# manasakani/DeviceKMC

Hardware: AMD Instinct MI355X
Metric: KMC steps/sec (higher is better)
Workload: dtype f64

## Files before the change

### devicekmc_amd/csrc/common.h

```cpp
#pragma once
#include <hip/hip_runtime.h>
#include <stdint.h>
#include <stdio.h>
#include <string.h>
#include <math.h>
#include "../../include/devicekmc_hip.h"
#include "../../include/devicekmc_hip_debug.h"

enum { DEFECT = 0, OXYGEN_DEFECT = 1, VACANCY = 2, O_EL = 3, Hf_EL = 4, Ni_EL = 5, Ti_EL = 6, Pt_EL = 7, N_EL = 8, NULL_ELEMENT = 9 };
enum { EV_GEN = 0, EV_REC = 1, EV_VDIFF = 2, EV_IDIFF = 3, EV_NULL = 4 };

#define DKMC_KB 8.617333262e-5
#define DKMC_Q 1.60217663e-19
#define DKMC_HBAR 1.054571817e-34
#define DKMC_MAX_LAYERS 5
#define WAVE 64

struct MetalSet { int n; const int *e; };

__device__ __forceinline__ bool is_metal(int el, const MetalSet &ms)
{
    bool r = false;
    for (int t = 0; t < ms.n; ++t) r |= (ms.e[t] == el);
    return r;
// ... 87 lines not shown
template <int NT>
__device__ __forceinline__ double block_sum_all(double v, double *red)
{
    const int lane = threadIdx.x & 63, w = threadIdx.x >> 6;
    v = wave_sum(v);
    __syncthreads();
    if (lane == 0) red[w] = v;
    __syncthreads();
    double s = 0.0;
#pragma unroll
    for (int i = 0; i < NT / 64; ++i) s += red[i];
    return s;
}

__host__ __device__ __forceinline__ unsigned long long dbl_key(double v)
{
    const unsigned long long b = __builtin_bit_cast(unsigned long long, v);
    return (b >> 63) ? ~b : (b | 0x8000000000000000ull);
}
__host__ __device__ __forceinline__ double key_dbl(unsigned long long k)
{
    return __builtin_bit_cast(double, (k >> 63) ? (k & 0x7fffffffffffffffull) : ~k);
}
__device__ __forceinline__ int ld_agent(const int *p) { return __hip_atomic_load(p, __ATOMIC_RELAXED, __HIP_MEMORY_SCOPE_AGENT); }
__device__ __forceinline__ void st_agent(int *p, int v) { __hip_atomic_store(p, v, __ATOMIC_RELAXED, __HIP_MEMORY_SCOPE_AGENT); }
__device__ __forceinline__ int seed_bits(int i, int N, int n_left, int n_right) { return (i < n_left ? 1 : 0) | (i >= N - n_right ? 2 : 0); }
inline void clamp_seeds(int N, int &n_left, int &n_right)
{
    n_left = n_left < 0 ? 0 : (n_left > N ? N : n_left);
    n_right = n_right < 0 ? 0 : (n_right > N ? N : n_right);
}

struct KBlocked {
    int m, R, nb, total, maxwin, maxints;
    long long winsum;
    int *perm;
    int *pcol;
    int4 *blk;
    int form = 1;
    int maxseg = 0;
    long long segsum = 0;
    int4 *seg = nullptr;
    int word_bytes = 4;
};
constexpr int X_POLY_DEFAULT = 8;
struct Engine {
    hipStream_t stream = nullptr;
    int device = 0;
    double cg_tol = 1e-6;
    int current_warm_start = 1;
    int profiling = 0;
    int cb_edge_domain = 0;
    long long tcache_budget = -1;
    double pair_cut = 6.5;
    int pair_form = 0;
    int k_blocked = 1;
    int k_blocked_large = 0;
    int k_window_word_bytes = 4;
    int x_aux = 2;
    int x_slab = 1;
    int k_slab = 1;
    int x_poly = X_POLY_DEFAULT;
    int x_poly_auto = 1;
    int x_poly_rows[2] = {0, 0};
    int x_poly_form = 2;
    int x_poly1_degree = 0;
    int x_poly_form_used = 0, x_poly_products = 0;
    int x_slab_poly = 0;
    int x_aux_warm = 0;
    int x_items_kc = 0;
    int x_apply_form = 0;
    int x_tile_f32 = 1;
    double x_tile_drop = 0.0;
    int x_tile_drop_unit = 0;
    int x_tile_drop_auto = 1;
    long long x_tile_drop_gate = 0;
    double x_tile_drop_used = 0.0;
    int xtl_census_form = 1;
    int x_static_tiles = 2;
    int x_static_gate = 0;
    int x_static_nM = -1;
    int x_static_verify = 0;
    int x_tile_f32_fail_once = 0;
    int x_nmul_form = 1;
    int x_nmul_lane_bytes = 16;
    int x_nmul_window = 2;
    int x_nmul_window_cap = 76 * 1024;
    int x_nmul_window_block = 320;
    int x_block = 16;
    int x_format = 1;
    int current_map = 0;
    int x_iter_hint = 0;
    int event_temperature = 0;
    int event_census = 0;
    int event_census_valid = 0;
    double event_census_info[16] = {0};
    dkmc_stats stats{};
    char err[512] = {0};
    int err_code = 0;
    double E_gen[DKMC_MAX_LAYERS] = {0}, E_rec[DKMC_MAX_LAYERS] = {0}, E_Vdiff[DKMC_MAX_LAYERS] = {0}, E_Odiff[DKMC_MAX_LAYERS] = {0};
    int num_layers = 0;
    static const int NBUF = 184;
    void *buf[NBUF] = {nullptr};
    size_t bufsz[NBUF] = {0};
};

constexpr int X_STATIC_GATE = 32768;
static inline int x_static_rule(int ns, int gate_override) { return ns >= (gate_override > 0 ? gate_override : X_STATIC_GATE) ? 1 : 0; }
Engine &eng();
int dkmc_fail(int code, const char *what, const char *file, int line);
void *scratch(int slot, size_t bytes);
void *scratch_try(int slot, size_t bytes);
static inline int grid_blocks(long long work, int per_block, int cap)
{
    long long b = (work + per_block - 1) / per_block;
    if (b < 1) b = 1;
    if (b > cap) b = cap;
    return (int)b;
}
inline MetalSet load_metals(const int *d_metals, int num_metals) { MetalSet ms; ms.n = num_metals; ms.e = d_metals; return ms; }

#define HIPCHK(x) do { hipError_t e__ = (x); if (e__ != hipSuccess) return dkmc_fail((int)e__, hipGetErrorString(e__), __FILE__, __LINE__); } while (0)
#define KCHK() do { hipError_t e__ = hipGetLastError(); if (e__ != hipSuccess) return dkmc_fail((int)e__, hipGetErrorString(e__), __FILE__, __LINE__); } while (0)

enum {
    S_CG_S = 0, S_CG_R, S_CG_P, S_CG_T, S_CG_PART, S_CG_CTRL, S_CG_RUNS, S_CG_REM, S_CG_NRUNS, S_CG_PS, S_CG_SEGOFF, S_CG_SEGS, S_CG_SEGPART, S_CG_XCHG, S_CG_PARTS,
    S_K_DATA, S_K_RHS,
    S_PW_LIST, S_PW_CNT, S_PW_CELLS, S_PW_PERM, S_PW_LIST2,
    S_EV_PROB, S_EV_ROWSUM, S_EV_G2, S_EV_G3, S_EV_CTRL, S_EV_UNI, S_EV_LOG,
    S_SCAN_TMP, S_SCAN_TMP2, S_SCAN_OFF64, S_SCAN_INTILE,
    S_AT_FLAG, S_AT_SITE, S_AT_OFSITE, S_AT_NEIGH,
    S_X_ROWPTR, S_X_COL, S_X_DATA, S_X_DATA2, S_X_CNT, S_X_SLIST, S_X_SCB, S_X_SFLAG, S_X_RHS, S_X_SRANK,
    S_P_IMACRO, S_HEAT, S_HEAT_A, S_HEAT_B, S_HEAT_Y,
    S_MISC0, S_MISC1, S_MISC2, S_MISC3,
    S_XT_DPOS, S_XT_SNODE_D, S_XT_SNODE_I, S_XT_CMASK, S_XT_ISTILE, S_XT_NSUBC, S_XT_TOFF, S_XT_SOFF, S_XT_TILES, S_XT_NITEMW, S_XT_WRANGE,
    S_XT_ITEMS, S_XT_SPLIT, S_XT_TVAL, S_XT_TVAL32, S_XT_ROWPART, S_XT_COLPART, S_XT_CNT, S_XT_Q,
    S_XT_T_NITEMW, S_XT_T_ITEMS, S_XT_T_SPLIT, S_XT_T_COLPART, S_XT_T_MISC,
    S_XTB_PANELS, S_XTB_QS, S_XTB_ROWPART, S_XTB_COLPART, S_XTB_GRAM, S_XTB_SMALL, S_XTB_XI,
    S_XTB_SLAB_BOX, S_XTB_SLAB_TAB, S_XTB_SLAB_OWNER, S_XTB_SLAB_LISTS, S_XTB_SLAB_SDST, S_XTB_SLAB_FLAG, S_XTB_SLAB_RLISTS, S_XTB_SLAB_GX, S_XTB_SLAB_S1, S_XTB_SLAB_S3, S_XTB_SLAB_R3,
    S_XTB_EMU_Y, S_XTB_EMU_CTRL, S_XTB_YPANEL, S_XTB_PRE_V, S_XTB_PRE_W1, S_XTB_PRE_W2, S_XTB_PRE_Z, S_XTB_PRE_U,
    S_XTB_NPACK_CNT, S_XTB_NPACK_OFF, S_XTB_NPACK_COL, S_XTB_NPACK_W,
    S_XTL_CELLS, S_XTL_TFLAG, S_XTL_TVAL32, S_XTL_TILES, S_XTL_WRANGE, S_XTL_NITEMW, S_XTL_ITEMS, S_XTL_SPLIT,
    S_KS_TAB, S_KS_OWNER, S_KS_LISTS, S_KS_FLAG, S_KS_BOX, S_KS_RLISTS, S_KS_XA, S_KS_XB, S_KS_SEND, S_KS_RECV, S_KS_YBUF, S_KS_EMU,
    S_XTB_TEST_RP, S_XTB_TEST_CI, S_XTB_TEST_VAL, S_XTB_TEST_SC, S_XTB_TEST_NSR, S_XTB_TEST_LIST, S_XTB_TEST_IN, S_XTB_TEST_ADD, S_XTB_TEST_OUT,
    S_XTB_TEST_W1, S_XTB_TEST_W2, S_XTB_TEST_QS, S_XTB_TEST_CTRL, S_XTB_TEST_NPCNT, S_XTB_TEST_NPOFF, S_XTB_TEST_NPCOL, S_XTB_TEST_NPW,
    S_P_CMAP,
    S_XTB_ALG_PANELS, S_XTB_ALG_INTS, S_XTB_ALG_GRAM, S_XTB_ALG_QS, S_XTB_ALG_CTRL,
    S_CL_PARENT, S_CL_SUMS, S_CL_POS, S_CL_TABLE, S_CL_CTRL,
    S_EV_NBAD, S_EV_CENSUS_PART, S_EV_CENSUS_INFO,
    S_GAP_SITE, S_GAP_CTRL, S_GAP_CELLS, S_GAP_SORTED, S_GAP_NODES, S_GAP_EDGES,
    S_PT_HOP, S_PT_PRED, S_PT_ROWS, S_PT_CTRL,
    S_TR_HASH, S_TR_COMP, S_TR_SITE, S_TR_ROWS, S_TR_CTRL,
    S_CUT_SITE, S_CUT_TABLE, S_CUT_ROWS, S_CUT_CTRL,
    S_FL_SITE, S_FL_ROWS, S_FL_CTRL,
    S_NSLOTS
};
static_assert(S_NSLOTS <= Engine::NBUF, "scratch slots");

int comm_attached();
int comm_nranks();
int comm_rank();
int comm_allgather_f64(double *buf, size_t count);
int comm_alltoallv_f64(const double *sendbuf, double *recvbuf, const long long *cnt);
int comm_allreduce_sum_f64(double *buf, size_t count);
int comm_agree(int local_rc, const char *what);
int comm_agree_count();
int comm_peer_ready(size_t count);
double *comm_peer_slots(int parity);
void comm_peer_drop();
int comm_peer_exchange(int parity, size_t count, int *ctrl_done, int *ctrl_aborted, int *ctrl_timeout, int stamp);
int comm_bcast0_f64(double *buf, size_t count);

int ev_census_enqueue(int N, int nn, const int *neigh, const int *element, const double *temperature, const double *ev_prob, double **d_info16);

int dkmc_exclusive_scan_i32(const int *d_in, int *d_out, int n, int *d_total);
int dkmc_exclusive_scan_i32_i64(const int *d_in, long long *d_out, int n, long long *d_total);
```

### devicekmc_amd/csrc/engine.hip

```cpp
#include "common.h"
#include <stdlib.h>

int events_upload_layers();
void xstate_reset(const void *key);

static Engine g_engine;
Engine &eng() { return g_engine; }

int dkmc_fail(int code, const char *what, const char *file, int line)
{
    Engine &e = eng();
    snprintf(e.err, sizeof(e.err), "%s (%s:%d)", what, file, line);
    e.err_code = code ? code : -1;
    fprintf(stderr, "devicekmc_hip: %s\n", e.err);
    return e.err_code;
}

void *scratch(int slot, size_t bytes)
{
    Engine &e = eng();
    if (bytes == 0) bytes = 16;
    if (e.bufsz[slot] < bytes) {
        if (e.buf[slot]) { (void)hipStreamSynchronize(e.stream); (void)hipFree(e.buf[slot]); }
        size_t want = bytes + bytes / 8 + 256;
        hipError_t rc = hipMalloc(&e.buf[slot], want);
        if (rc != hipSuccess) {
            char msg[160]; snprintf(msg, sizeof(msg), "hipMalloc(%zu bytes) failed in scratch(slot %d): %s", want, slot, hipGetErrorString(rc));
            dkmc_fail(2, msg, __FILE__, __LINE__); e.buf[slot] = nullptr; e.bufsz[slot] = 0; return nullptr;
        }
        e.bufsz[slot] = want;
    }
    return e.buf[slot];
}

void *scratch_try(int slot, size_t bytes)
{
    Engine &e = eng();
    if (bytes == 0) bytes = 16;
    if (e.bufsz[slot] < bytes) {
        if (e.buf[slot]) { (void)hipStreamSynchronize(e.stream); (void)hipFree(e.buf[slot]); }
        e.buf[slot] = nullptr; e.bufsz[slot] = 0;
        const size_t want = bytes + bytes / 8 + 256;
        if (hipMalloc(&e.buf[slot], want) != hipSuccess) { (void)hipGetLastError(); e.buf[slot] = nullptr; return nullptr; }
        e.bufsz[slot] = want;
    }
    return e.buf[slot];
}

extern "C" {

const char *dkmc_last_error(void) { return eng().err; }
void dkmc_clear_error(void) { eng().err[0] = 0; eng().err_code = 0; }
const dkmc_stats *dkmc_get_stats(void) { return &eng().stats; }
void dkmc_set_cg_tolerance(double tol) { eng().cg_tol = tol; }
void dkmc_set_current_warm_start(int mode) { eng().current_warm_start = mode; }
int dkmc_get_current_warm_start(void) { return eng().current_warm_start; }
void dkmc_set_profiling(int on) { eng().profiling = on; }
void dkmc_set_x_format(int tiled) { eng().x_format = tiled ? 1 : 0; }
int dkmc_get_x_format(void) { return eng().x_format; }
void dkmc_set_current_map(int on) { eng().current_map = on ? 1 : 0; }
int dkmc_get_current_map(void) { return eng().current_map; }
void dkmc_set_tcache_budget(long long bytes) { eng().tcache_budget = bytes; }
void dkmc_set_pair_cutoff(double x_cut) { eng().pair_cut = x_cut > 0.0 ? x_cut : 0.0; }
void dkmc_set_pair_form(int form) { eng().pair_form = form == 1 ? 1 : 0; }
int dkmc_get_pair_form(void) { return eng().pair_form; }
void dkmc_set_k_slab(int on) { eng().k_slab = on ? 1 : 0; }
int dkmc_get_k_slab(void) { return eng().k_slab; }
void dkmc_set_x_aux_warm(int on) { eng().x_aux_warm = on ? 1 : 0; }
int dkmc_get_x_aux_warm(void) { return eng().x_aux_warm; }
void dkmc_set_x_items(int kc) { eng().x_items_kc = kc > 0 ? (kc < 256 ? kc : 256) : 0; }
void dkmc_set_x_poly(int degree) { eng().x_poly = degree < 0 ? 0 : (degree > 16 ? 16 : degree); eng().x_poly_auto = 0; }
int dkmc_get_x_poly(void) { return eng().x_poly; }
void dkmc_set_x_poly_auto(int on) { Engine &e = eng(); e.x_poly_auto = on ? 1 : 0; if (on && e.x_poly <= 0) e.x_poly = X_POLY_DEFAULT; }
int dkmc_get_x_poly_auto(void) { return eng().x_poly_auto; }
void dkmc_set_x_poly_form(int form) { eng().x_poly_form = form == 1 ? 1 : (form == 2 ? 2 : 0); }
int dkmc_get_x_poly_form(void) { return eng().x_poly_form; }
int dkmc_get_x_poly_form_used(void) { return eng().x_poly_form_used; }
int dkmc_get_x_poly_products(void) { return eng().x_poly_products; }
void dkmc_debug_set_x_poly1_degree(int n) { eng().x_poly1_degree = n < 0 ? 0 : (n > 20 ? 20 : n); }
void dkmc_set_x_poly_auto_rows(int n0, int n1) { Engine &e = eng(); e.x_poly_rows[0] = n0 > 0 ? n0 : 0; e.x_poly_rows[1] = n1 > e.x_poly_rows[0] ? n1 : e.x_poly_rows[0]; }
void dkmc_set_x_apply_form(int form) { eng().x_apply_form = form == 1 ? 1 : 0; }
int dkmc_get_x_apply_form(void) { return eng().x_apply_form; }
void dkmc_set_x_tile_f32(int mode) { eng().x_tile_f32 = mode == 0 ? 0 : 1; }
int dkmc_get_x_tile_f32(void) { return eng().x_tile_f32; }
void dkmc_set_x_tile_drop(double theta) { eng().x_tile_drop = theta > 0.0 ? (theta > 1e-4 ? 1e-4 : theta) : 0.0; }
double dkmc_get_x_tile_drop(void) { return eng().x_tile_drop; }
void dkmc_set_x_tile_drop_unit(int unit) { eng().x_tile_drop_unit = unit == 1 ? 1 : 0; }
int dkmc_get_x_tile_drop_unit(void) { return eng().x_tile_drop_unit; }
void dkmc_set_x_tile_drop_auto(int on) { eng().x_tile_drop_auto = on ? 1 : 0; }
int dkmc_get_x_tile_drop_auto(void) { return eng().x_tile_drop_auto; }
void dkmc_set_x_tile_drop_auto_subblocks(long long gate) { eng().x_tile_drop_gate = gate > 0 ? gate : 0; }
double dkmc_get_x_tile_drop_used(void) { return eng().x_tile_drop_used; }
void dkmc_debug_fail_true_residual_once(void) { eng().x_tile_f32_fail_once = 1; }
void dkmc_set_x_static_tiles(int mode) { eng().x_static_tiles = (mode == 0 || mode == 1) ? mode : 2; }
int dkmc_get_x_static_tiles(void) { return eng().x_static_tiles; }
int dkmc_debug_x_static_verify(int on) { const int was = eng().x_static_verify; eng().x_static_verify = on ? 1 : 0; return was; }
void dkmc_debug_set_x_static_gate(int members) { eng().x_static_gate = members > 0 ? members : 0; }
int dkmc_x_static_rule(int members) { return x_static_rule(members, eng().x_static_gate); }
int dkmc_x_static_strips(int n_metals) { return n_metals > 0 ? n_metals / 256 : 0; }
void dkmc_set_x_nmul_form(int form) { eng().x_nmul_form = form == 0 ? 0 : 1; }
int dkmc_get_x_nmul_form(void) { return eng().x_nmul_form; }
void dkmc_set_x_nmul_lane_bytes(int bytes) { eng().x_nmul_lane_bytes = bytes == 8 ? 8 : 16; }
int dkmc_get_x_nmul_lane_bytes(void) { return eng().x_nmul_lane_bytes; }
void dkmc_set_x_nmul_window(int mode) { eng().x_nmul_window = (mode == 0 || mode == 1) ? mode : 2; }
int dkmc_get_x_nmul_window(void) { return eng().x_nmul_window; }
void dkmc_debug_set_x_nmul_window(int cap_bytes, int block_rows)
{
    Engine &e = eng();
    e.x_nmul_window_cap = cap_bytes < 0 ? 76 * 1024 : (cap_bytes > 76 * 1024 ? 76 * 1024 : cap_bytes);
    e.x_nmul_window_block = (block_rows >= 16 && block_rows <= 1024 && block_rows % 16 == 0) ? block_rows : 320;
}
void dkmc_set_x_slab(int on) { eng().x_slab = on ? 1 : 0; }
int dkmc_get_x_slab(void) { return eng().x_slab; }
void dkmc_set_x_slab_poly(int on) { eng().x_slab_poly = on ? 1 : 0; }
int dkmc_get_x_slab_poly(void) { return eng().x_slab_poly; }
void dkmc_set_x_block(int s) { eng().x_block = s < 1 ? 1 : (s > 16 ? 16 : s); }
int dkmc_get_x_block(void) { return eng().x_block; }
void dkmc_set_x_aux(int mode) { eng().x_aux = mode < 0 ? 0 : (mode > 3 ? 2 : mode); }
int dkmc_get_x_aux(void) { return eng().x_aux; }
void dkmc_set_k_blocked(int on) { eng().k_blocked = on ? 1 : 0; }
int dkmc_get_k_blocked(void) { return eng().k_blocked; }
void dkmc_set_k_blocked_large(int on) { eng().k_blocked_large = on ? 1 : 0; }
int dkmc_get_k_blocked_large(void) { return eng().k_blocked_large; }
void dkmc_set_k_window_word_bytes(int bytes) { eng().k_window_word_bytes = bytes == 2 ? 2 : 4; }
int dkmc_get_k_window_word_bytes(void) { return eng().k_window_word_bytes; }
void dkmc_set_cb_edge_domain(int atoms_only) { eng().cb_edge_domain = atoms_only ? 1 : 0; }

int dkmc_get_gpu_info(char *gpu_string, int capacity, int dev)
{
    hipDeviceProp_t prop;
    HIPCHK(hipSetDevice(dev));
    HIPCHK(hipGetDeviceProperties(&prop, dev));
    snprintf(gpu_string, capacity, "%s", prop.name);
    return 0;
}

int dkmc_set_gpu(int dev) { HIPCHK(hipSetDevice(dev)); eng().device = dev; return 0; }
int dkmc_set_stream(void *s) { eng().stream = (hipStream_t)s; return 0; }
int dkmc_synchronize(void) { HIPCHK(hipStreamSynchronize(eng().stream)); return 0; }

int dkmc_copy_to_const_memory(const double *E_gen, const double *E_rec, const double *E_Vdiff, const double *E_Odiff, int nl)
{
    Engine &e = eng();
    if (nl > DKMC_MAX_LAYERS) return dkmc_fail(3, "more than 5 layers (MAX_NUM_LAYERS, kmc_events.cu:7)", __FILE__, __LINE__);
    e.num_layers = nl;
    for (int i = 0; i < nl; ++i) { e.E_gen[i] = E_gen[i]; e.E_rec[i] = E_rec[i]; e.E_Vdiff[i] = E_Vdiff[i]; e.E_Odiff[i] = E_Odiff[i]; }
    return events_upload_layers();
}

#define ALLOC(field, n, T) HIPCHK(hipMalloc((void **)&buf->field, (size_t)(n) * sizeof(T)))
int dkmc_gpubuf_create(dkmc_gpubuf *buf, int N, int N_atom, int nn, int nmt,
                       const int *h_layer, const double *hx, const double *hy, const double *hz,
                       const int *h_neigh, const int *h_metals, double freq, double sigma, double k, const double *h_lattice)
{
    memset(buf, 0, sizeof(*buf));
    buf->N_ = N; buf->N_atom_ = N_atom; buf->nn_ = nn; buf->num_metal_types_ = nmt;
    ALLOC(site_layer, N, int); ALLOC(site_element, N, int); ALLOC(metal_types, nmt > 0 ? nmt : 1, int);
    ALLOC(site_x, N, double); ALLOC(site_y, N, double); ALLOC(site_z, N, double);
    ALLOC(site_power, N, double); ALLOC(site_CB_edge, N, double);
    ALLOC(site_potential_boundary, N, double); ALLOC(site_potential_charge, N, double);
    ALLOC(site_temperature, N, double); ALLOC(site_charge, N, int);
    ALLOC(neigh_idx, (size_t)N * nn, int);
    ALLOC(T_bg, 1, double); ALLOC(sigma, 1, double); ALLOC(k, 1, double); ALLOC(lattice, 3, double); ALLOC(freq, 1, double);
    ALLOC(atom_element, N, int); ALLOC(atom_x, N, double); ALLOC(atom_y, N, double); ALLOC(atom_z, N, double);
    ALLOC(atom_power, N, double); ALLOC(atom_CB_edge, N, double); ALLOC(atom_charge, N, int);
    ALLOC(atom_virtual_potentials, N_atom + 2, double);
    HIPCHK(hipMemset(buf->atom_virtual_potentials, 0, (size_t)(N_atom + 2) * sizeof(double)));
    HIPCHK(hipMemset(buf->site_power, 0, (size_t)N * sizeof(double)));
    HIPCHK(hipMemcpy(buf->site_layer, h_layer, (size_t)N * sizeof(int), hipMemcpyHostToDevice));
    HIPCHK(hipMemcpy(buf->site_x, hx, (size_t)N * sizeof(double), hipMemcpyHostToDevice));
    HIPCHK(hipMemcpy(buf->site_y, hy, (size_t)N * sizeof(double), hipMemcpyHostToDevice));
    HIPCHK(hipMemcpy(buf->site_z, hz, (size_t)N * sizeof(double), hipMemcpyHostToDevice));
    if (nmt > 0) HIPCHK(hipMemcpy(buf->metal_types, h_metals, (size_t)nmt * sizeof(int), hipMemcpyHostToDevice));
    HIPCHK(hipMemcpy(buf->sigma, &sigma, sizeof(double), hipMemcpyHostToDevice));
    HIPCHK(hipMemcpy(buf->k, &k, sizeof(double), hipMemcpyHostToDevice));
    HIPCHK(hipMemcpy(buf->freq, &freq, sizeof(double), hipMemcpyHostToDevice));
// ... 75 lines not shown
```

### devicekmc_amd/csrc/xt.hip

```cpp
#include "xtiles.h"
#include <hip/hip_ext.h>
int tc_prepare_tiled(const XParams &P, dkmc_gpubuf *buf, int ns, const SEntry *S, const int *aflag, const int *srank, const int *atom_site,
                     int c_lo, int c_hi, int sharded, TCacheView *out);
#include <vector>
#include <algorithm>
#include <stdlib.h>
#include <string.h>

__device__ __forceinline__ double xt_tvalue(const XParams &P, double prefac, const TCacheView &TC,
                                            double x1, double y1, double z1, double cb1, int f1, int slot1, int slotA1, int mr1,
                                            double x2, double y2, double z2, double cb2, int f2, int slot2, int slotA2, int mr2,
                                            bool have_pre = false, double pre = 0.0)
{
    const double d = site_dist(x1, y1, z1, x2, y2, z2, P.laty, P.latz, P.pbc);
    if (d < P.nn_dist) return 0.0;
    const int kind = tunnel_kind<AF_MP_VAL>(f1, f2, cb1, cb2, P.tol);
    if (!kind) return 0.0;
    if (kind == 1 && TC.enabled) {
        const bool v1 = f1 & AF_V;
        double cv;
        if (have_pre && !v1) { if (pre == pre) return -pre; }
        else if (tc_lookup(TC, v1 ? slot1 : slot2, v1 ? slotA1 : slotA2, v1 ? mr2 : mr1, cv)) return -cv;
    }
    return -wkb_T(kind, 1e-10 * d, fabs(cb1 - cb2), prefac, P.V0);
}

__global__ void k_xt_snodes(int ns, int ns_pad, const SEntry *__restrict__ S, const double *__restrict__ ax, const double *__restrict__ ay,
                            const double *__restrict__ az, double *sx, double *sy, double *sz, double *scb, int *sflag, int *srow)
{
    const int s = blockIdx.x * blockDim.x + threadIdx.x;
    if (s >= ns_pad) return;
    if (s < ns) {
        const SEntry e = S[s];
        sx[s] = ax[e.idx]; sy[s] = ay[e.idx]; sz[s] = az[e.idx]; scb[s] = e.cb; sflag[s] = e.flag; srow[s] = e.idx + 2;
    } else { sx[s] = 0; sy[s] = 0; sz[s] = 0; scb[s] = 0; sflag[s] = 0; srow[s] = -1; }
}
__global__ void k_xt_snode_slots(int ns, int ns_pad, const SEntry *__restrict__ S, const int *__restrict__ atom_site, TCacheView TC,
                                 int *sslot, int *sslotA, int *smr)
{
    const int s = blockIdx.x * blockDim.x + threadIdx.x;
    if (s >= ns_pad) return;
    int sl = -1, sa = -1, mr = -1;
    if (s < ns && TC.enabled) {
        const SEntry e = S[s];
        if (e.flag & AF_V) { const int site = atom_site[e.idx]; sl = TC.slot_of_site[site]; if (TC.nL) sa = TC.slotA_of_site[site]; }
        mr = TC.mrank_atom[e.idx];
    }
    sslot[s] = sl; sslotA[s] = sa; smr[s] = mr;
}

__global__ __launch_bounds__(XT_NT) void k_xt_census(XParams P, int ns, int nK, int nW, SNodes S, unsigned *__restrict__ cmask,
                                                     const int *__restrict__ keep_flags, long long n_keep_cells)
{
    const int lane = threadIdx.x & 63;
    const long long ci = (long long)blockIdx.x * (XT_NT / 64) + (threadIdx.x >> 6);
    if (ci >= (long long)nK * nW) return;
    if (keep_flags && ci < n_keep_cells && keep_flags[0] == 0) return;
    const int w = (int)(ci / nK), k = (int)(ci % nK);
    unsigned m = 0;
    if (XT_C * w + XT_C - 1 > XT_R * k) {
        double cx[4], cy[4], cz[4], ccb[4]; int cf[4], csc[4];
#pragma unroll
        for (int j = 0; j < 4; ++j) {
            const int sc = XT_C * w + lane + 64 * j;
            csc[j] = sc; cx[j] = S.x[sc]; cy[j] = S.y[sc]; cz[j] = S.z[sc]; ccb[j] = S.cb[sc]; cf[j] = S.flag[sc];
        }
        for (int r = 0; r < XT_R; ++r) {
            const int s = XT_R * k + r;
            if (s >= ns) break;
            const double rx = S.x[s], ry = S.y[s], rz = S.z[s], rcb = S.cb[s]; const int rf = S.flag[s];
#pragma unroll
            for (int j = 0; j < 4; ++j) {
                const bool pred = csc[j] > s && tunnel_kind<AF_MP_VAL>(rf, cf[j], rcb, ccb[j], P.tol) != 0 &&
                                  !(site_dist(rx, ry, rz, cx[j], cy[j], cz[j], P.laty, P.latz, P.pbc) < P.nn_dist);
                const unsigned long long bal = __ballot(pred);
                if (bal & 0xffffffffull) m |= 1u << (2 * j);
                if (bal >> 32) m |= 1u << (2 * j + 1);
            }
            if (m == 0xffu) break;
        }
    }
    if (lane == 0) cmask[ci] = m;
}
__global__ void k_xt_cell_counts(long long ncell, const unsigned *__restrict__ cmask, int *__restrict__ is_tile, int *__restrict__ nsub)
{
    const long long i = (long long)blockIdx.x * blockDim.x + threadIdx.x;
    if (i < ncell) { const unsigned m = cmask[i]; is_tile[i] = m != 0; nsub[i] = __popc(m); }
}
__global__ void k_xt_tile_list(int nK, long long ncell, const unsigned *__restrict__ cmask, const int *__restrict__ toff, const int *__restrict__ soff,
                               XTile *__restrict__ tiles)
{
    const long long i = (long long)blockIdx.x * blockDim.x + threadIdx.x;
    if (i < ncell && cmask[i]) { XTile t; t.k = (int)(i % nK); t.w = (int)(i / nK); t.mask = cmask[i]; t.soff = soff[i]; tiles[toff[i]] = t; }
}
__global__ void k_xt_wrange(int nK, int nW, const unsigned *__restrict__ cmask, int2 *__restrict__ wrange)
{
    const int i = blockIdx.x * blockDim.x + threadIdx.x;
    if (i < nK) {
        int b = nW, e = 0;
        for (int w = 0; w < nW; ++w) if (cmask[(long long)w * nK + i]) { b = min(b, w); e = w + 1; }
        wrange[i] = make_int2(b, e);
    }
}
#define XT_MAXRANKS 64
#define XT_TAPER 2048
struct XSplit { int n; int taper; int tb[XT_MAXRANKS + 1]; int item_lo[XT_MAXRANKS + 1]; int max_items_per_strip; int nitems;
                int soff[XT_MAXRANKS + 1], w_first[XT_MAXRANKS + 1], w_last[XT_MAXRANKS + 1]; };
__global__ void k_xt_split(int ntiles, long long nsub_total, const XTile *__restrict__ tiles, int n, XSplit *sp)
{
    const int r = threadIdx.x;
    if (r > n) return;
    int t = 0;
    if (r == n) t = ntiles;
    else if (r > 0) {
        const long long want = nsub_total * r / n;
        int lo = 0, hi = ntiles;
        while (lo < hi) { const int mid = (lo + hi) >> 1; if ((long long)tiles[mid].soff < want) lo = mid + 1; else hi = mid; }
        t = lo;
    }
    sp->tb[r] = t;
    if (r == 0) { sp->n = n; sp->max_items_per_strip = 0; sp->taper = (ntiles / n >= 8 * XT_TAPER) ? XT_TAPER : 0; }
}
__device__ __forceinline__ int xt_run_len(int t, int t1, int kc, const XSplit *sp)
{
    int r = 0;
    while (r + 1 < sp->n && t >= sp->tb[r + 1]) ++r;
    const int end = sp->tb[r + 1], d = end - 1 - t;
    const int sh = sp->taper ? d / sp->taper : 5;
    int len = sh >= 5 ? kc : min(kc, 1 << sh);
    return max(1, min(len, min(end, t1) - t));
}
template <int MODE>
__global__ void k_xt_items(int nK, int nW, int kc, int ntiles, const int *__restrict__ toff, const int *__restrict__ ioff, const XTile *__restrict__ tiles,
                           XSplit *sp, int *__restrict__ nitem_w, XItem *__restrict__ items, int rec_shift)
{
    const int w = blockIdx.x * blockDim.x + threadIdx.x;
    if (w == 0 && !MODE) nitem_w[2 * (nW + 2)] = rec_shift;
    if (w >= nW) return;
    const int t0 = toff[(long long)w * nK], t1 = (w + 1 < nW) ? toff[(long long)(w + 1) * nK] : ntiles;
    int o = MODE ? ioff[w] : 0, c = 0;
    const int m = (1 << rec_shift) - 1;
    for (int t = t0; t < t1;) {
        const int len = xt_run_len(t, t1, kc, sp);
        if (MODE) { const XTile f = tiles[t]; XItem it; it.t0 = t; it.t1 = t + len; it.w = w; it.c = rec_shift ? 1 : 0; it.k0 = f.k; it.mask0 = f.mask; it.soff0 = f.soff; it.pad = (o + c) >> rec_shift; items[o + c] = it; }
        t += len; ++c;
        bool cut = t >= t1;
        if (!cut) for (int r = 1; r < sp->n; ++r) cut |= sp->tb[r] == t;
        if (cut) {
            const int cpad = (c + m) & ~m;
            for (; c < cpad; ++c)
                if (MODE) { XItem it; it.t0 = t - 1; it.t1 = t - 1; it.w = w; it.c = 1; it.k0 = 0; it.mask0 = 0; it.soff0 = 0; it.pad = (o + c) >> rec_shift; items[o + c] = it; }
        }
    }
    if (!MODE) { nitem_w[w] = c; atomicMax(&sp->max_items_per_strip, c); }
}
__global__ void k_xt_rank_items(const int *__restrict__ nitems_dev, int ntiles, long long nsub_total, const XItem *__restrict__ items,
                                const XTile *__restrict__ tiles, XSplit *sp)
{
    const int r = threadIdx.x;
    const int nitems = *nitems_dev;
    if (r == 0) sp->nitems = nitems;
    if (r > sp->n) return;
    const int tb = sp->tb[r];
    int lo = 0, hi = nitems;
    while (lo < hi) { const int mid = (lo + hi) >> 1; if (items[mid].t0 < tb) lo = mid + 1; else hi = mid; }
    if (r == sp->n) lo = nitems;
    sp->item_lo[r] = lo;
    sp->soff[r] = tb < ntiles ? tiles[tb].soff : (int)nsub_total;
    sp->w_first[r] = tb < ntiles ? tiles[tb].w : 0;
    sp->w_last[r] = tb > 0 ? tiles[tb - 1].w : 0;
}

template <int TR>
__global__ __launch_bounds__(XT_NT) void k_xt_fill(XParams P, int ns, const XTile *__restrict__ tiles, int sub_base, SNodes S, TCacheView TC,
                                                   double *__restrict__ tval, unsigned long long *__restrict__ nnz_upper, float *__restrict__ tval32, int t_split)
{
    __shared__ double rx[XT_R], ry[XT_R], rz[XT_R], rcb[XT_R];
    __shared__ int rf[XT_R], rslot[XT_R], rslotA[XT_R], rmr[XT_R];
    __shared__ double lt[TR ? XT_C / XT_SBW : 1][TR ? XT_R / 2 : 1][TR ? XT_SBW + 1 : 1];
    const XTile td = tiles[blockIdx.x];
    const int tid = threadIdx.x;
    if (tid < XT_R) {
        const int s = XT_R * td.k + tid;
        rx[tid] = S.x[s]; ry[tid] = S.y[s]; rz[tid] = S.z[s]; rcb[tid] = S.cb[s]; rf[tid] = S.flag[s]; rslot[tid] = S.slot[s]; rslotA[tid] = S.slotA[s]; rmr[tid] = S.mr[s];
// ... 667 lines not shown

template <int OP>
static int xt_tile_sums(const double *vS, double *out, int vpos)
{
    Engine &e = eng(); hipStream_t st = e.stream; const XTState &X = g_xt;
    if (X.item_n > 0)
        hipLaunchKernelGGL((k_xt_tiles_only<OP>), dim3((X.item_n + 3) / 4), dim3(XT_NT), 0, st, X.item_n, (const XItem *)g_xb.items + X.item_lo,
                           (const XTile *)g_xb.tiles, (int)X.sub_base, (const double *)g_xb.tval, vS, X.nW, X.ns_pad, g_xb.rowpart, g_xb.colpart, vpos);
    hipLaunchKernelGGL((k_xt_rows<1>), dim3(std::max(X.nK, 1)), dim3(XT_NT), 0, st, X.ns, X.nK, X.nW, X.ns_pad, (const int2 *)g_xb.wrange,
                       (const int *)g_xb.nitem_w, (const double *)g_xb.rowpart, (const double *)g_xb.colpart, (const int *)nullptr,
                       (const double *)nullptr, (const double *)nullptr, (double *)nullptr, (double *)nullptr, (const XCtrl *)nullptr, out,
                       0, (const int *)nullptr, 0, (const double *)nullptr, X.w_lo, X.w_hi);
    KCHK();
    if (comm_attached()) {
        int rc = comm_allreduce_sum_f64(out, (size_t)X.ns); if (rc) return rc;
        rc = comm_bcast0_f64(out, (size_t)X.ns); if (rc) return rc;
    }
    return 0;
}

int xt_tile_sums_mv(const double *vS, double *out) { return xt_tile_sums<0>(vS, out, 1); }

static int xt_build_items(int nK, int nW, int kc, int ntiles, long long nsub_total, const int *toff, const XTile *tiles, int nranks, int me,
                          int slot_nitemw, int slot_items, int slot_split, XShare *out, int rec_shift = 0)
{
    Engine &e = eng(); hipStream_t st = e.stream;
    if (nranks > XT_MAXRANKS) return dkmc_fail(46, "update_power: more ranks than XT_MAXRANKS", __FILE__, __LINE__);
    int *nitem_w = (int *)scratch(slot_nitemw, (size_t)(nW + 4) * 4 * 3);
    XSplit *sp = (XSplit *)scratch(slot_split, sizeof(XSplit));
    if (!nitem_w || !sp) return e.err_code;
    int *ioff = nitem_w + nW + 2;
    XSplit h{};
    out->nitem_w = nitem_w; out->items = nullptr; out->nitems = 0; out->maxchunk = 1; out->rec_shift = rec_shift;
    out->item_lo = 0; out->item_n = 0; out->tile_lo = 0; out->tile_n = 0; out->sub_base = 0; out->sub_n = 0; out->w_lo = 0; out->w_hi = 0;
    if (ntiles <= 0) { HIPCHK(hipMemsetAsync(nitem_w, 0, (size_t)(nW + 4) * 4 * 3, st)); return 0; }
    hipLaunchKernelGGL(k_xt_split, dim3(1), dim3(XT_MAXRANKS + 1), 0, st, ntiles, nsub_total, tiles, nranks, sp);
    hipLaunchKernelGGL((k_xt_items<0>), dim3((nW + 255) / 256), dim3(256), 0, st, nK, nW, kc, ntiles, toff, (const int *)nullptr, tiles, sp, nitem_w, (XItem *)nullptr, rec_shift);
    int rc = dkmc_exclusive_scan_i32(nitem_w, ioff, nW, ioff + nW); if (rc) return rc;
    XItem *items = (XItem *)scratch(slot_items, (size_t)(ntiles + 4 * (size_t)(nW + nranks) + 4) * sizeof(XItem));
    if (!items) return e.err_code;
    hipLaunchKernelGGL((k_xt_items<1>), dim3((nW + 255) / 256), dim3(256), 0, st, nK, nW, kc, ntiles, toff, (const int *)ioff, tiles, sp, nitem_w, items, rec_shift);
    hipLaunchKernelGGL(k_xt_rank_items, dim3(1), dim3(XT_MAXRANKS + 1), 0, st, (const int *)(ioff + nW), ntiles, nsub_total, (const XItem *)items, tiles, sp);
    HIPCHK(hipMemcpyAsync(&h, sp, sizeof(XSplit), hipMemcpyDeviceToHost, st));
    HIPCHK(hipStreamSynchronize(st));
    const int nitems = h.nitems;
    out->items = items; out->nitems = nitems; out->maxchunk = std::max(1, h.max_items_per_strip);
    out->item_lo = h.item_lo[me]; out->item_n = h.item_lo[me + 1] - h.item_lo[me];
    out->tile_lo = h.tb[me]; out->tile_n = h.tb[me + 1] - h.tb[me];
    out->sub_base = h.soff[me]; out->sub_n = h.soff[me + 1] - h.soff[me];
    out->w_lo = h.w_first[me]; out->w_hi = out->tile_n > 0 ? h.w_last[me + 1] + 1 : out->w_lo;
    return 0;
}

#include "xt_live.h"
#include "xt_static.h"

static SideStream g_side;

int xt_assemble_and_solve(dkmc_gpubuf *buf, const XParams &P, int ns, const SEntry *S, const int *aneigh, const int *ancnt, const int *aflag,
                          const int *srank, const int *atom_site, double *rhs, double *y, int *iters_out, double *rr_out, double *yaux, int yaux_valid, int warm)
{
    TCacheView TC{};
    Engine &e = eng(); hipStream_t st = e.stream;
    XTState &X = g_xt; X.valid = false;
    g_xlive = XLive{};
    const int Na = P.Na, Nsub = Na + 1;
    X.Nsub = Nsub; X.ns = ns;
    const int ns_pad = ((ns + XT_C - 1) / XT_C) * XT_C + XT_C;
    X.ns_pad = ns_pad;
    const int nK = (ns + XT_R - 1) / XT_R, nW = (ns + XT_C - 1) / XT_C;
    X.nK = nK; X.nW = nW;
    const long long ncell = (long long)nK * nW;
    if (ncell > 0x7ffffff0ll) return dkmc_fail(47, "update_power: too many tile cells", __FILE__, __LINE__);

    const int nbr = (Nsub + 255) / 256, m = Nsub;
    const bool sharded = comm_attached() != 0;
    const int nr = sharded ? comm_nranks() : 1, me = sharded ? comm_rank() : 0;
    int rc = 0, ntiles = 0;
    long long xs_nnz = 0;
    int *cnt = nullptr, *nsrank = nullptr, *col = nullptr, *si = nullptr, *srow = nullptr, *nitem_w = nullptr;
    xrp_t *rp = nullptr, *dpos = nullptr;
    double *val = nullptr, *sd = nullptr, *tval = nullptr, *rowpart = nullptr, *colpart = nullptr, *sc = nullptr, *r = nullptr, *p = nullptr, *t = nullptr,
           *q = nullptr, *vS = nullptr, *part = nullptr, *qS = nullptr, *sS = nullptr, *xS = nullptr, *part_pt = nullptr, *part_rr = nullptr;
    XTile *tiles = nullptr; int2 *wrange = nullptr; XItem *items = nullptr; unsigned long long *d_cnt = nullptr; XCtrl *ctrl = nullptr;
    float *tval32 = nullptr;
    SNodes SN{};
    double *xbuf = nullptr;
    XStatic &K = g_xs;
    const bool k_had = K.valid;
    K.valid = false; K.pending = false; K.reused = false; K.verify_nnz = -1;
    const int nM_first = (!sharded && e.x_format != 0) ? e.x_static_nM : -1;
    const int w_static = nM_first >= 0 ? xs_w_static(nM_first) : 0;
    for (int c = 0; c < 8; ++c) K.info[c] = 0;
    for (int c = 0; c < 4; ++c) K.verify[c] = 0;
    K.info[0] = nM_first >= 0 ? 1 : 0; K.info[1] = w_static; K.info[6] = XS_NA; K.info[7] = -1;
    int t_static = 0, xs_reason = XS_NA; long long sub_static = 0;
    bool k_cand = false;
    auto assemble = [&]() -> int {
        if (g_fault_phase == 1) { g_fault_phase = 0; return dkmc_fail(90, "injected fault (assembly of X)", __FILE__, __LINE__); }
        if (sharded) { xbuf = (double *)scratch(S_CG_XCHG, ((size_t)ns * (e.x_block > 1 ? 16 : 1) + 2) * (e.x_block > 1 ? comm_nranks() : 1) * 8); if (!xbuf) return e.err_code; if (ns > 0) { rc = side_stream_init(g_side); if (rc) return rc; } }
        cnt = (int *)scratch(S_X_CNT, (size_t)(Nsub + 4) * 4);
        rp = (xrp_t *)scratch(S_X_ROWPTR, (size_t)(Nsub + 4) * sizeof(xrp_t));
        dpos = (xrp_t *)scratch(S_XT_DPOS, (size_t)(Nsub + 4) * sizeof(xrp_t));
        nsrank = (int *)scratch(S_X_SCB, (size_t)(Nsub + 4) * 4);
        if (!cnt || !rp || !dpos || !nsrank) return e.err_code;
        hipLaunchKernelGGL((k_xpat_plain<0>), dim3(nbr), dim3(256), 0, st, P, (const int *)nullptr, aneigh, ancnt, cnt, (const xrp_t *)nullptr, (int *)nullptr);
        rc = dkmc_exclusive_scan_i32_i64(cnt, rp, Nsub, rp + Nsub); if (rc) return rc;
        HIPCHK(hipMemcpyAsync(&xs_nnz, rp + Nsub, sizeof(long long), hipMemcpyDeviceToHost, st));
        HIPCHK(hipStreamSynchronize(st));
        if (xs_nnz <= 0) return dkmc_fail(10, "update_power: empty X", __FILE__, __LINE__);
        X.xs_nnz = xs_nnz;
        col = (int *)scratch(S_X_COL, (size_t)xs_nnz * 4);
        val = (double *)scratch(S_X_DATA, (size_t)xs_nnz * 8);
        if (!col || !val) return e.err_code;
        hipLaunchKernelGGL((k_xpat_plain<1>), dim3(nbr), dim3(256), 0, st, P, (const int *)nullptr, aneigh, ancnt, cnt, (const xrp_t *)rp, col);
        hipLaunchKernelGGL((k_xval<16>), dim3((Nsub + 15) / 16), dim3(256), 0, st, P, Nsub, (const SEntry *)nullptr, 0, (const int *)nullptr, (const xrp_t *)rp,
                           (const int *)col, (const double *)buf->atom_x, (const double *)buf->atom_y, (const double *)buf->atom_z, aflag,
                           (const double *)buf->atom_CB_edge, val, TCacheView{}, atom_site, dpos);
        hipLaunchKernelGGL(k_xt_node_srank, dim3(nbr), dim3(256), 0, st, Nsub, srank, nsrank);
        KCHK();
        g_xb.rp = rp; g_xb.dpos = dpos; g_xb.ci = col; g_xb.val = val; g_xb.nsrank = nsrank;
        g_xb.ax = buf->atom_x; g_xb.ay = buf->atom_y; g_xb.az = buf->atom_z;

        sd = (double *)scratch(S_XT_SNODE_D, (size_t)ns_pad * 4 * 8);
        si = (int *)scratch(S_XT_SNODE_I, (size_t)ns_pad * 5 * 4);
        if (!sd || !si) return e.err_code;
        SN.x = sd; SN.y = sd + ns_pad; SN.z = sd + 2 * (size_t)ns_pad; SN.cb = sd + 3 * (size_t)ns_pad;
        SN.flag = si; SN.slot = si + ns_pad; SN.mr = si + 2 * (size_t)ns_pad; SN.slotA = si + 4 * (size_t)ns_pad;
        srow = si + 3 * (size_t)ns_pad;
        hipLaunchKernelGGL(k_xt_snodes, dim3((ns_pad + 255) / 256), dim3(256), 0, st, ns, ns_pad, S, (const double *)buf->atom_x, (const double *)buf->atom_y,
                           (const double *)buf->atom_z, sd, sd + ns_pad, sd + 2 * (size_t)ns_pad, sd + 3 * (size_t)ns_pad, si, srow);
        g_xb.S = SN; g_xb.srow = srow;
        if (w_static > 0) {
            const double par[6] = {P.tol, P.nn_dist, P.m_e, P.V0, P.laty, P.latz};
            if (!k_had || K.key != (const void *)buf->site_x) xs_reason = XS_FIRST;
            else if (K.nM != nM_first || K.w_static != w_static) xs_reason = XS_METALS;
            else if (memcmp(par, K.par, sizeof(par)) != 0 || K.pbc != P.pbc) xs_reason = XS_PARAMS;
            else {
                k_cand = true; xs_reason = XS_KEPT;
                HIPCHK(hipMemsetAsync(K.flags, 0, 4 * sizeof(int), st));
                hipLaunchKernelGGL(k_xs_cmp_metals, dim3((nM_first + 255) / 256), dim3(256), 0, st, nM_first, SN, (const double *)K.snap_d, (const int *)K.snap_f, K.flags);
            }
        }

        X.ntiles = 0; X.nitems = 0; X.nsub_total = 0; X.t_upper = 0; X.kc = 1;
        unsigned *cmask = nullptr; int *is_tile = nullptr, *nsubc = nullptr, *toff = nullptr, *soff = nullptr;
        if (ncell > 0) {
            cmask = (unsigned *)scratch(S_XT_CMASK, (size_t)(ncell + 4) * 4);
            is_tile = (int *)scratch(S_XT_ISTILE, (size_t)(ncell + 4) * 4);
            nsubc = (int *)scratch(S_XT_NSUBC, (size_t)(ncell + 4) * 4);
            toff = (int *)scratch(S_XT_TOFF, (size_t)(ncell + 4) * 4);
            soff = (int *)scratch(S_XT_SOFF, (size_t)(ncell + 4) * 4);
            if (!cmask || !is_tile || !nsubc || !toff || !soff) return e.err_code;
            const long long n_keep = k_cand ? (long long)w_static * nK : 0;
            if (k_cand) {
                HIPCHK(hipMemsetAsync(cmask, 0, (size_t)n_keep * 4, st));
                if (K.t_static > 0) hipLaunchKernelGGL(k_xs_scatter_masks, dim3((K.t_static + 255) / 256), dim3(256), 0, st, K.t_static, (const XTile *)K.tiles, nK, (const int *)K.flags, cmask);
            }
            hipLaunchKernelGGL(k_xt_census, dim3((unsigned)((ncell + 3) / 4)), dim3(XT_NT), 0, st, P, ns, nK, nW, SN, cmask, k_cand ? (const int *)K.flags : (const int *)nullptr, n_keep);
            hipLaunchKernelGGL(k_xt_cell_counts, dim3((unsigned)((ncell + 255) / 256)), dim3(256), 0, st, ncell, (const unsigned *)cmask, is_tile, nsubc);
            rc = dkmc_exclusive_scan_i32(is_tile, toff, (int)ncell, toff + ncell); if (rc) return rc;
            rc = dkmc_exclusive_scan_i32(nsubc, soff, (int)ncell, soff + ncell); if (rc) return rc;
            int h2[2] = {0, 0}, hs[2] = {0, 0}, hf = 0;
            HIPCHK(hipMemcpyAsync(&h2[0], toff + ncell, sizeof(int), hipMemcpyDeviceToHost, st));
            HIPCHK(hipMemcpyAsync(&h2[1], soff + ncell, sizeof(int), hipMemcpyDeviceToHost, st));
            if (w_static > 0) {
                HIPCHK(hipMemcpyAsync(&hs[0], toff + (long long)w_static * nK, sizeof(int), hipMemcpyDeviceToHost, st));
                HIPCHK(hipMemcpyAsync(&hs[1], soff + (long long)w_static * nK, sizeof(int), hipMemcpyDeviceToHost, st));
                if (k_cand) HIPCHK(hipMemcpyAsync(&hf, K.flags, sizeof(int), hipMemcpyDeviceToHost, st));
            }
            HIPCHK(hipStreamSynchronize(st));
            X.ntiles = h2[0]; X.nsub_total = h2[1];
            t_static = hs[0]; sub_static = hs[1];
            if (k_cand && hf) { k_cand = false; xs_reason = XS_METALS; }
            if (k_cand && (t_static != K.t_static || sub_static != K.sub_static)) { k_cand = false; xs_reason = XS_PREFIX; }
            if (h2[1] < 0) return dkmc_fail(47, "update_power: more than 2^31 sub-blocks", __FILE__, __LINE__);
        }
        ntiles = X.ntiles;
        X.kc = std::max(1, std::min(XT_MAXKC, ntiles / nr / 4096));
        if (e.x_block > 1 && ntiles <= 2048 * nr) X.kc = std::max(1, std::min(XT_MAXKC, (ntiles + 1024 * nr - 1) / (1024 * nr)));
        tiles = (XTile *)scratch(S_XT_TILES, (size_t)(ntiles + 1) * sizeof(XTile));
        wrange = (int2 *)scratch(S_XT_WRANGE, (size_t)(nK + 4) * sizeof(int2));
        if (!tiles || !wrange) return e.err_code;
        if (ncell > 0) {
            hipLaunchKernelGGL(k_xt_tile_list, dim3((unsigned)((ncell + 255) / 256)), dim3(256), 0, st, nK, ncell, (const unsigned *)cmask, (const int *)toff, (const int *)soff, tiles);
            hipLaunchKernelGGL(k_xt_wrange, dim3((nK + 255) / 256), dim3(256), 0, st, nK, nW, (const unsigned *)cmask, wrange);
        }
        int h_prefix_differs = 0;
        if (k_cand && t_static > 0) {
            hipLaunchKernelGGL(k_xs_cmp_tiles, dim3((t_static + 255) / 256), dim3(256), 0, st, t_static, (const XTile *)tiles, (const XTile *)K.tiles, K.flags);
            HIPCHK(hipMemcpyAsync(&h_prefix_differs, K.flags + 1, sizeof(int), hipMemcpyDeviceToHost, st));
        }
        XShare sh{};
        if (e.x_items_kc > 0) X.kc = e.x_items_kc;
        rc = xt_build_items(nK, nW, X.kc, ntiles, X.nsub_total, toff, tiles, nr, me, S_XT_NITEMW, S_XT_ITEMS, S_XT_SPLIT, &sh, 2); if (rc) return rc;
        if ((sh.item_lo | sh.item_n) & 3) return dkmc_fail(48, "update_power: run list not padded to groups of four", __FILE__, __LINE__);
        X.nitems = sh.nitems; X.maxchunk = sh.maxchunk; X.rec_shift = sh.rec_shift;
        items = sh.items; nitem_w = sh.nitem_w;
        KCHK();
        if (k_cand && t_static > 0) { HIPCHK(hipStreamSynchronize(st)); if (h_prefix_differs) { k_cand = false; xs_reason = XS_PREFIX; } }
        g_xb.tiles = tiles; g_xb.items = items; g_xb.wrange = wrange; g_xb.nitem_w = nitem_w; g_xb.cmask = cmask; g_xb.toff = toff;

        X.item_lo = sh.item_lo; X.item_n = sh.item_n; X.tile_lo = sh.tile_lo; X.tile_n = sh.tile_n; X.sub_base = sh.sub_base; X.sub_n = sh.sub_n;
        X.w_lo = sh.w_lo; X.w_hi = sh.w_hi;
        e.stats.comm_ranks = sharded ? comm_nranks() : 0;
        e.stats.comm_count_per_rank = sharded ? ns + 2 : 0;
        e.stats.comm_local_segments = X.item_n;

        rc = tc_prepare_tiled(P, buf, ns, S, aflag, srank, atom_site, sharded ? XT_C * X.w_lo : 0, sharded ? XT_C * X.w_hi : 0x7fffffff, sharded ? 1 : 0, &TC);
        if (rc) return rc;
        hipLaunchKernelGGL(k_xt_snode_slots, dim3((ns_pad + 255) / 256), dim3(256), 0, st, ns, ns_pad, S, atom_site, TC, si + ns_pad, si + 4 * (size_t)ns_pad, si + 2 * (size_t)ns_pad);

        if (k_cand && (e.buf[S_XT_TVAL] != K.tval || e.bufsz[S_XT_TVAL] != K.tval_cap)) { k_cand = false; xs_reason = XS_STORE; }
        if (k_cand) {
            bool kept = true;
            tval = (double *)xs_scratch_keep(S_XT_TVAL, (size_t)(X.sub_n + 4) * XT_SUB * 8, (size_t)sub_static * XT_SUB * 8, false, &kept);
            if (!kept) { k_cand = false; xs_reason = XS_STORE; }
        } else
        tval = (double *)scratch(S_XT_TVAL, (size_t)(X.sub_n + 4) * XT_SUB * 8);
        rowpart = (double *)scratch(S_XT_ROWPART, (size_t)(ncell + 1) * XT_R * 8);
        colpart = (double *)scratch(S_XT_COLPART, (size_t)(X.nitems + 1) * XT_C * 8);
        d_cnt = (unsigned long long *)scratch(S_XT_CNT, 16);
        if (!tval || !rowpart || !colpart || !d_cnt) return e.err_code;
        tval32 = nullptr; e.stats.x_tile_stream = 0; e.stats.x_tile_f64_rounds = 0; e.stats.x_tile_f32_bytes = 0;
        if (e.x_tile_f32 != 0 && !sharded && e.x_block > 1 && e.x_poly > 0 && e.cg_tol >= 1e-8 && X.tile_n > 0) {
            const size_t b32 = (size_t)(X.sub_n + 4) * XT_SUB * 4;
            if (k_cand && K.img && e.buf[S_XT_TVAL32] == K.tval32 && e.bufsz[S_XT_TVAL32] == K.tval32_cap) {
                bool kept = true;
                tval32 = (float *)xs_scratch_keep(S_XT_TVAL32, b32, (size_t)sub_static * XT_SUB * 4, true, &kept);
                if (!kept) { k_cand = false; xs_reason = XS_IMAGE; }
            } else {
                if (k_cand) { k_cand = false; xs_reason = K.img ? XS_STORE : XS_IMAGE; }
                tval32 = (float *)scratch_try(S_XT_TVAL32, b32);
            }
            if (tval32) e.stats.x_tile_f32_bytes = (long long)b32; else e.stats.x_tile_stream = -1;
        }
        HIPCHK(hipMemsetAsync(rowpart, 0, (size_t)(ncell + 1) * XT_R * 8, st));
        HIPCHK(hipMemsetAsync(colpart, 0, (size_t)(X.nitems + 1) * XT_C * 8, st));
        HIPCHK(hipMemsetAsync(d_cnt, 0, 16, st));
        if (k_cand && (tval32 != nullptr) != K.img) { k_cand = false; xs_reason = XS_IMAGE; }
        if (w_static > 0 && !k_cand) { rc = xs_reserve(nM_first, t_static); if (rc) return rc; }
        const int t_fill0 = k_cand ? t_static : 0;
        if (nM_first < 0) {
            if (X.tile_n > 0)
                hipLaunchKernelGGL((k_xt_fill<0>), dim3(X.tile_n), dim3(XT_NT), 0, st, P, ns, (const XTile *)tiles + X.tile_lo, (int)X.sub_base, SN, TC, tval, d_cnt, tval32, 0);
        } else {
            if (t_fill0 == 0 && t_static > 0)
                hipLaunchKernelGGL((k_xt_fill<0>), dim3(t_static), dim3(XT_NT), 0, st, P, ns, (const XTile *)tiles, (int)X.sub_base, SN, TC, tval, d_cnt, tval32, t_static);
            if (X.tile_n - t_static > 0)
                hipLaunchKernelGGL((k_xt_fill<1>), dim3(X.tile_n - t_static), dim3(XT_NT), 0, st, P, ns, (const XTile *)tiles + t_static, (int)X.sub_base, SN, TC, tval, d_cnt, tval32, 0);
        }
        KCHK();
        K.info[2] = k_cand ? t_static : 0; K.info[3] = X.tile_n - t_fill0; K.info[4] = k_cand ? sub_static : 0; K.info[5] = X.sub_n - (k_cand ? sub_static : 0); K.info[6] = xs_reason;
        if (w_static > 0) {
            if (!k_cand) {
                if (t_static > 0) HIPCHK(hipMemcpyAsync(K.tiles, tiles, (size_t)t_static * sizeof(XTile), hipMemcpyDeviceToDevice, st));
                hipLaunchKernelGGL(k_xs_snapshot, dim3((nM_first + 255) / 256), dim3(256), 0, st, nM_first, SN, K.snap_d, K.snap_f);
                KCHK();
                const double par[6] = {P.tol, P.nn_dist, P.m_e, P.V0, P.laty, P.latz};
                memcpy(K.par, par, sizeof(par)); K.pbc = P.pbc;
                K.key = (const void *)buf->site_x; K.nM = nM_first; K.w_static = w_static; K.t_static = t_static; K.sub_static = sub_static;
            }
            K.tval = e.buf[S_XT_TVAL]; K.tval_cap = e.bufsz[S_XT_TVAL]; K.img = tval32 != nullptr;
            K.tval32 = K.img ? e.buf[S_XT_TVAL32] : nullptr; K.tval32_cap = K.img ? e.bufsz[S_XT_TVAL32] : 0;
            K.pending = true; K.reused = k_cand;
        }
        if (e.x_static_verify && nM_first >= 0 && ncell > 0) {
            rc = xs_verify(P, ns, nK, nW, ncell, SN, TC, cmask, tiles, ntiles, X.nsub_total, tval, tval32); if (rc) return rc;
        }
        g_xb.tval32 = tval32;
        g_xb.tval = tval; g_xb.rowpart = rowpart; g_xb.colpart = colpart;
        X.valid = true;

        sc = (double *)scratch(S_CG_S, (size_t)m * 8); r = (double *)scratch(S_CG_R, (size_t)m * 8);
        p = (double *)scratch(S_CG_P, (size_t)m * 8); t = (double *)scratch(S_CG_T, (size_t)m * 8);
        q = (double *)scratch(S_XT_Q, (size_t)m * 8);
        vS = (double *)scratch(S_CG_PS, (size_t)ns_pad * 3 * 8);
        part = (double *)scratch(S_CG_PART, (size_t)3 * 8192 * 8);
        ctrl = (XCtrl *)scratch(S_CG_CTRL, sizeof(XCtrl));
        if (!sc || !r || !p || !t || !q || !vS || !part || !ctrl) return e.err_code;
        qS = vS; sS = vS + ns_pad; xS = vS + 2 * (size_t)ns_pad;
        HIPCHK(hipMemsetAsync(vS, 0, (size_t)ns_pad * 3 * 8, st));
        part_pt = part; part_rr = part + 4096;
        return 0;
    };
    rc = assemble();
    if (sharded) rc = comm_agree(rc, "assembly of X");
    if (rc) return rc;

    const double tol2 = e.cg_tol * e.cg_tol;

    if (ns > 0) {
        hipLaunchKernelGGL(k_xt_fill_f64, dim3((ns + 255) / 256), dim3(256), 0, st, qS, (long long)ns, 1.0);
        rc = xt_tile_sums<0>(qS, xS, 1); if (rc) return rc;
    }
    hipLaunchKernelGGL(k_xt_scale_init, dim3(nbr), dim3(256), 0, st, m, (const xrp_t *)dpos, val, (const int *)nsrank, (const double *)xS, sc, rhs, y, q, sS, qS);
    KCHK();

    const int ntb = (X.item_n + 3) / 4;
    const int nsb = (std::max(m - 2, 1) + XT_NT / 8 * XT_RPG_FUSED - 1) / (XT_NT / 8 * XT_RPG_FUSED);
    const int nsb1 = (std::max(m - 2, 1) + XT_NT / 8 - 1) / (XT_NT / 8);
    const int n2b = grid_blocks(std::max(std::max(nK, (m + 4095) / 4096), 1), 1, 1024);
    const int gv = grid_blocks(m, XT_NT * 4, 256);
    const int np_pt = n2b;
    const bool nt_loads = (size_t)X.sub_n * XT_SUB * 8 > ((size_t)200 << 20);

    const bool split = sharded && ns > 0;
    const bool seq_neigh = !split && (size_t)X.sub_n * XT_SUB * 8 > ((size_t)2 << 30);
    e.stats.xt_split_launch = (split || seq_neigh) ? 1 : 0;
    int cur_it = -1, local_fail = 0;
    auto matvec = [&](hipEvent_t e0, hipEvent_t e1, hipEvent_t e2, hipEvent_t e3, hipEvent_t ec) -> int {
#define XT_APPLY_ARGS(NI, NTB, NSB) NI, (const XItem *)items + X.item_lo, (const XTile *)tiles, (int)X.sub_base, (const double *)tval, (const double *)qS, nW, ns_pad, \
                      rowpart, colpart, (const XCtrl *)ctrl, NTB, NSB, m, (const xrp_t *)rp, (const int *)col, (const double *)val, (const double *)q, \
                      (const double *)sc, (const int *)nsrank, t
        if (split) {
            SideStream &S = g_side; const int sl = (int)(S.seq++ % SideStream::RING);
            auto local = [&]() -> int {
            if (g_fault_phase == 2 && cur_it >= g_fault_iter) { g_fault_phase = 0; return dkmc_fail(91, "injected fault (CG iteration)", __FILE__, __LINE__); }
            if (ntb > 0) {
                if (nt_loads) hipExtLaunchKernelGGL((k_xt_apply<1>), dim3(ntb), dim3(XT_NT), 0, st, e0, e1, 0, XT_APPLY_ARGS(X.item_n, ntb, 0), 2);
                else hipExtLaunchKernelGGL((k_xt_apply<0>), dim3(ntb), dim3(XT_NT), 0, st, e0, e1, 0, XT_APPLY_ARGS(X.item_n, ntb, 0), 2);
            } else if (e0) { HIPCHK(hipEventRecord(e0, st)); HIPCHK(hipEventRecord(e1, st)); }
            HIPCHK(hipEventRecord(S.a[sl], st));
            HIPCHK(hipStreamWaitEvent(S.st, S.a[sl], 0));
            hipLaunchKernelGGL(k_xt_neigh, dim3(nsb1 + 2), dim3(XT_NT), 0, S.st, nsb1, m, (const xrp_t *)rp, (const int *)col, (const double *)val, (const double *)q,
                               (const double *)sc, (const int *)nsrank, (const XCtrl *)ctrl, t);
            HIPCHK(hipEventRecord(S.b[sl], S.st));
            hipLaunchKernelGGL((k_xt_rows<1>), dim3(std::max(nK, 1)), dim3(XT_NT), 0, st, ns, nK, nW, ns_pad, (const int2 *)wrange, (const int *)nitem_w, (const double *)rowpart,
                               (const double *)colpart, (const int *)srow, (const double *)sS, (const double *)p, t, part_pt, (const XCtrl *)ctrl, xbuf,
                               m, (const int *)nsrank, comm_rank() == 0 ? 1 : 0, (const double *)r, X.w_lo, X.w_hi);
            KCHK();
            return 0;
            };
            if (int lrc = local()) {
                if (!local_fail) local_fail = lrc;
                (void)hipGetLastError();
                hipLaunchKernelGGL(k_xt_abort_word, dim3(1), dim3(1), 0, st, ctrl, xbuf, ns);
            }
            if (int rcx = comm_allreduce_sum_f64(xbuf, (size_t)ns + 2)) return rcx;
            if (ec) HIPCHK(hipEventRecord(ec, st));
            HIPCHK(hipStreamWaitEvent(st, S.b[sl], 0));
            hipExtLaunchKernelGGL(k_xt_rows_apply, dim3(n2b), dim3(XT_NT), 0, st, e2, e3, 0, ns, nK, (const double *)xbuf, (const int *)srow, (const double *)sS,
                                  (const double *)p, t, part_pt, ctrl, m, (const int *)nsrank, (const double *)r);
            return 0;
        }
        if (seq_neigh) {
            if (ntb > 0) hipExtLaunchKernelGGL((k_xt_apply<1>), dim3(ntb), dim3(XT_NT), 0, st, e0, e1, 0, XT_APPLY_ARGS(X.item_n, ntb, 0), 2);
            else if (e0) { HIPCHK(hipEventRecord(e0, st)); HIPCHK(hipEventRecord(e1, st)); }
            hipLaunchKernelGGL(k_xt_neigh, dim3(nsb1 + 2), dim3(XT_NT), 0, st, nsb1, m, (const xrp_t *)rp, (const int *)col, (const double *)val, (const double *)q,
                               (const double *)sc, (const int *)nsrank, (const XCtrl *)ctrl, t);
        } else if (nt_loads) hipExtLaunchKernelGGL((k_xt_apply<1>), dim3(ntb + nsb + 2), dim3(XT_NT), 0, st, e0, e1, 0, XT_APPLY_ARGS(X.item_n, ntb, nsb), 0);
        else hipExtLaunchKernelGGL((k_xt_apply<0>), dim3(ntb + nsb + 2), dim3(XT_NT), 0, st, e0, e1, 0, XT_APPLY_ARGS(X.item_n, ntb, nsb), 0);
#undef XT_APPLY_ARGS
        hipExtLaunchKernelGGL((k_xt_rows<0>), dim3(n2b), dim3(XT_NT), 0, st, e2, e3, 0, ns, nK, nW, ns_pad, (const int2 *)wrange, (const int *)nitem_w,
                              (const double *)rowpart, (const double *)colpart, (const int *)srow, (const double *)sS, (const double *)p, t,
                              part_pt, (const XCtrl *)ctrl, (double *)nullptr, m, (const int *)nsrank, 0, (const double *)r, 0, nW);
        return 0;
    };

    XCtrl h{};
    bool solved = false;
    e.stats.xb_width = 1; e.stats.xb_fallback = 0; e.stats.xb_poly_used = 0;
    if (e.x_block > 1 && ns > 0) {
        XtbArgs B{};
        B.m = m; B.ns = ns; B.ns_pad = ns_pad; B.nK = nK; B.nW = nW; B.s = e.x_block;
        B.items = (const XItem *)items + X.item_lo; B.item_n = X.item_n; B.tiles = tiles; B.sub_base = (int)X.sub_base; B.tval = tval; B.tval32 = tval32;
        B.wrange = wrange; B.nitem_w = nitem_w; B.nrecords = X.nitems >> X.rec_shift;
        B.srow = srow; B.sS = sS; B.nsrank = nsrank; B.rp = rp; B.ci = col; B.val = val; B.sc = sc; B.ax = buf->atom_x; B.ay = buf->atom_y; B.az = buf->atom_z; B.b = rhs; B.y = y;
        B.yaux = yaux; B.yaux_valid = yaux_valid;
        B.ctrl = ctrl; B.tol2 = tol2; B.nt_loads = nt_loads; B.sharded = sharded; B.w_lo = X.w_lo; B.w_hi = X.w_hi;
        B.warm = warm != 0; B.stored_subblocks = X.nsub_total;
        int bi = 0; double brr = 0.0;
        rc = xtb_cg(B, &bi, &brr);
        e.stats.xb_width = e.x_block;
        if (rc == 0) { solved = true; h.iters = bi; h.rr[bi & 1] = brr; if (sharded && !(e.x_slab && comm_nranks() > 1)) e.stats.comm_count_per_rank = (long long)ns * (4 * ((e.x_block + 3) / 4)) + 2; }
        else if (rc != DKMC_XTB_BREAKDOWN) return rc;
        else {
            e.stats.xb_fallback = 1;
            hipLaunchKernelGGL(k_xt_requeue, dim3(nbr), dim3(256), 0, st, m, (const double *)y, (const double *)sc, (const int *)nsrank, q, qS);
        }
    }
    const bool prof = e.profiling != 0;
    if (!solved) {
    HIPCHK(hipMemsetAsync(ctrl, 0, sizeof(XCtrl), st));
    if (sharded && ns > 0) hipLaunchKernelGGL(k_xt_set_sharded, dim3(1), dim3(1), 0, st, ctrl);
    HIPCHK(hipMemsetAsync(p, 0, (size_t)m * 8, st));
    rc = matvec(nullptr, nullptr, nullptr, nullptr, nullptr); if (rc) return rc;
    hipLaunchKernelGGL(k_xt_resid_init, dim3(gv), dim3(XT_NT), 0, st, m, (const double *)t, (const double *)rhs, r, p, (const double *)sc, q, (const int *)nsrank, qS, part_rr);
    hipLaunchKernelGGL(k_xt_check0, dim3(1), dim3(XT_NT), 0, st, (const double *)part_rr, gv, ctrl, tol2);
    KCHK();

    EventSampler &pf = g_loop_events;
    if (prof) if (int prc = pf.begin(EventSampler::LONG | EventSampler::SHORT | (sharded && ns > 0 ? EventSampler::COMM : 0))) return prc;

    const int loop_rc = cg_poll_loop(ctrl, h, LaunchPlan::hinted_minus8(e.x_iter_hint), st, "CG: no convergence after 200000 iterations", prof ? &pf : nullptr,
                                     [&](int it, const hipEvent_t *ev) -> int {
            cur_it = it;
            if (int mrc = matvec(ev[0], ev[1], ev[2], ev[3], ev[4])) return mrc;
            hipLaunchKernelGGL(k_xt_step, dim3(gv), dim3(XT_NT), 0, st, m, it, (const double *)part_pt, np_pt, (const double *)(part_rr + 512 * (it & 1)), gv,
                               part_rr + 512 * ((it + 1) & 1), p, (const double *)t, y, r, (const double *)sc, q, (const int *)nsrank, qS, ctrl, tol2);
            return 0;
        });
    if (loop_rc) { HIPCHK(hipStreamSynchronize(st)); return loop_rc; }
    if (local_fail) return local_fail;
    if (h.aborted) return dkmc_fail(46, "a peer rank aborted the sharded current solve", __FILE__, __LINE__);
    }
    hipLaunchKernelGGL(k_xt_vec_mul, dim3(nbr), dim3(256), 0, st, m, y, (const double *)sc);
    KCHK();
    if (sharded && !solved) { rc = comm_bcast0_f64(y, (size_t)m); if (rc) return rc; }
    unsigned long long h_cnt[2] = {0, 0};
    HIPCHK(hipMemcpyAsync(h_cnt, d_cnt, sizeof(h_cnt), hipMemcpyDeviceToHost, st));
    HIPCHK(hipStreamSynchronize(st));
    X.t_upper = h_cnt[0] + (K.pending && K.reused ? K.nnz_static : h_cnt[1]);
    if (K.pending && !e.err_code) {
        if (!K.reused) K.nnz_static = h_cnt[1];
        K.valid = true;
    }
    K.pending = false;
    if (K.verify_nnz >= 0) {
        const long long d = (long long)X.t_upper - K.verify_nnz;
        K.verify[3] = d < 0 ? -d : d;
        K.info[7] = K.verify[0] + K.verify[1] + K.verify[2] + K.verify[3];
    }
    e.x_iter_hint = h.iters;
    if (iters_out) *iters_out = h.iters;
    if (rr_out) *rr_out = h.rr[h.iters & 1];
    long long t_upper = (long long)X.t_upper;
    if (sharded) {
        double *cntbuf = (double *)scratch(S_XT_CNT, 16);
        double hv = (double)t_upper;
        HIPCHK(hipMemcpy(cntbuf, &hv, 8, hipMemcpyHostToDevice));
        if (int rcx = comm_allreduce_sum_f64(cntbuf, 1)) return rcx;
        HIPCHK(hipStreamSynchronize(st));
        HIPCHK(hipMemcpy(&hv, cntbuf, 8, hipMemcpyDeviceToHost));
        t_upper = (long long)(hv + 0.5);
    }
    e.stats.X_nnz = xs_nnz + 2 * t_upper;
    e.stats.spmv_tiles = ntiles; e.stats.spmv_tile_entries = t_upper;
    e.stats.xt_subblocks = X.nsub_total; e.stats.xt_local_subblocks = X.sub_n; e.stats.xt_items = X.nitems; e.stats.xt_kc = X.kc; e.stats.xt_records = X.nitems >> X.rec_shift;
    if (solved && e.x_tile_drop_used > 0.0 && g_xlive.state == 1) {
        const XLive &lv = g_xlive;
        e.stats.xt_local_subblocks = lv.info[e.x_tile_drop_unit == 1 ? 5 : 4]; e.stats.spmv_tiles = (int)lv.info[2]; e.stats.xt_items = lv.nitems; e.stats.xt_records = lv.nrecords;
    }
    e.stats.xt_sparse_nnz = xs_nnz; e.stats.xt_ns = ns;
    e.stats.spmv_segments = 0; e.stats.spmv_segment_entries = 0;
    e.stats.spmv_long_rows = ns; e.stats.spmv_short_rows = m - ns; e.stats.spmv_long_nnz = 2 * t_upper; e.stats.spmv_short_nnz = xs_nnz;
    if (prof && !solved) g_loop_events.to_stats(e.stats, true);
    return e.err_code;
}

// ... 146 lines not shown
{
    const int s = blockIdx.x * blockDim.x + threadIdx.x;
    if (s < ns) v[s] = 0.5 + (double)(((unsigned)s * 2654435761u) >> 16) / 65536.0;
}
__global__ void k_xt_test_accumulate(int ns, double *__restrict__ acc, const double *__restrict__ x)
{
    const int s = blockIdx.x * blockDim.x + threadIdx.x;
    if (s < ns) acc[s] += x[s];
}
extern "C" int dkmc_xt_check_shares(int nranks, double *max_abs_diff, double *max_abs, long long *subblocks_sum, long long *items_sum, int *items_total)
{
    Engine &e = eng(); hipStream_t st = e.stream; const XTState &X = g_xt;
    if (!X.valid || comm_attached() || X.tile_n != X.ntiles) return dkmc_fail(13, "xt_check_shares: needs the X of a single-GPU solve", __FILE__, __LINE__);
    if (nranks < 1 || nranks > XT_MAXRANKS) return dkmc_fail(13, "xt_check_shares: bad arguments", __FILE__, __LINE__);
    const int nK = X.nK, nW = X.nW, ns = X.ns, ns_pad = X.ns_pad, ntiles = X.ntiles;
    if (max_abs_diff) *max_abs_diff = 0.0;
    if (max_abs) *max_abs = 0.0;
    if (subblocks_sum) *subblocks_sum = 0;
    if (items_sum) *items_sum = 0;
    if (items_total) *items_total = 0;
    if (ns <= 0 || ntiles <= 0) return 0;
    double *buf = (double *)scratch(S_XT_T_MISC, (size_t)4 * ns_pad * 8);
    if (!buf) return e.err_code;
    double *v = buf, *full = buf + ns_pad, *acc = buf + 2 * (size_t)ns_pad, *tmp = buf + 3 * (size_t)ns_pad;
    const int gb = (ns + 255) / 256;
    HIPCHK(hipMemsetAsync(buf, 0, (size_t)4 * ns_pad * 8, st));
    hipLaunchKernelGGL(k_xt_test_vector, dim3(gb), dim3(256), 0, st, ns, v);
    int rc = xt_tile_sums<0>(v, full, 0); if (rc) return rc;
    const size_t rowpart_bytes = (size_t)((long long)nK * nW + 1) * XT_R * 8;
    const int kc = std::max(1, std::min(XT_MAXKC, ntiles / nranks / 4096));
    long long sb_sum = 0, it_sum = 0;
    for (int r = 0; r < nranks; ++r) {
        XShare sh{};
        rc = xt_build_items(nK, nW, kc, ntiles, X.nsub_total, (const int *)g_xb.toff, (const XTile *)g_xb.tiles, nranks, r,
                            S_XT_T_NITEMW, S_XT_T_ITEMS, S_XT_T_SPLIT, &sh, 2);
        if (rc) return rc;
        if ((sh.item_lo | sh.item_n) & 3) return dkmc_fail(48, "xt_check_shares: run list not padded to groups of four", __FILE__, __LINE__);
        if (items_total) *items_total = sh.nitems;
        sb_sum += sh.sub_n; it_sum += sh.item_n;
        double *colpart = (double *)scratch(S_XT_T_COLPART, (size_t)(sh.nitems + 1) * XT_C * 8);
        if (!colpart) return e.err_code;
        HIPCHK(hipMemsetAsync(colpart, 0, (size_t)(sh.nitems + 1) * XT_C * 8, st));
        HIPCHK(hipMemsetAsync(g_xb.rowpart, 0, rowpart_bytes, st));
        if (sh.item_n > 0)
            hipLaunchKernelGGL((k_xt_tiles_only<0>), dim3((sh.item_n + 3) / 4), dim3(XT_NT), 0, st, sh.item_n, (const XItem *)sh.items + sh.item_lo,
                               (const XTile *)g_xb.tiles, 0, (const double *)g_xb.tval, (const double *)v, nW, ns_pad, g_xb.rowpart, colpart, 0);
        hipLaunchKernelGGL((k_xt_rows<1>), dim3(std::max(nK, 1)), dim3(XT_NT), 0, st, ns, nK, nW, ns_pad, (const int2 *)g_xb.wrange,
                           (const int *)sh.nitem_w, (const double *)g_xb.rowpart, (const double *)colpart, (const int *)nullptr,
                           (const double *)nullptr, (const double *)nullptr, (double *)nullptr, (double *)nullptr, (const XCtrl *)nullptr, tmp,
                           0, (const int *)nullptr, 0, (const double *)nullptr, sh.w_lo, sh.w_hi);
        hipLaunchKernelGGL(k_xt_test_accumulate, dim3(gb), dim3(256), 0, st, ns, acc, (const double *)tmp);
        KCHK();
    }
    HIPCHK(hipMemsetAsync(g_xb.rowpart, 0, rowpart_bytes, st));
    std::vector<double> hf(ns), ha(ns);
    HIPCHK(hipMemcpyAsync(hf.data(), full, (size_t)ns * 8, hipMemcpyDeviceToHost, st));
    HIPCHK(hipMemcpyAsync(ha.data(), acc, (size_t)ns * 8, hipMemcpyDeviceToHost, st));
    HIPCHK(hipStreamSynchronize(st));
    double md = 0.0, ma = 0.0;
    for (int i = 0; i < ns; ++i) { md = std::max(md, fabs(hf[i] - ha[i])); ma = std::max(ma, fabs(hf[i])); }
    if (max_abs_diff) *max_abs_diff = md;
    if (max_abs) *max_abs = ma;
    if (subblocks_sum) *subblocks_sum = sb_sum;
    if (items_sum) *items_sum = it_sum;
    return e.err_code;
}


extern "C" int dkmc_xtb_emulate_slabs(int nranks, int width, double tol, int time_rank, int sweep_cap, double *rel_diff, int *iters_slab, int *iters_ref,
                                      double *times_us , long long *xdoubles , int *rows_min_max )
{
    Engine &e = eng(); hipStream_t st = e.stream; const XTState &X = g_xt;
    if (!X.valid || comm_attached() || X.tile_n != X.ntiles || X.ns <= 0 || !g_xb.ay) return dkmc_fail(13, "xtb_emulate_slabs: needs the X of a single-GPU solve", __FILE__, __LINE__);
    if (nranks < 1 || nranks > 32) return dkmc_fail(13, "xtb_emulate_slabs: 1 ... 32 ranks", __FILE__, __LINE__);
    const int m = X.Nsub, ns = X.ns, s = std::max(2, std::min(width, 16));
    double *sc = (double *)e.buf[S_CG_S], *sS = (double *)e.buf[S_CG_PS], *rhs = (double *)e.buf[S_X_RHS];
    double *yb = (double *)scratch(S_XTB_EMU_Y, (size_t)(m + 8) * 8 * 2);
    XCtrl *ctrl = (XCtrl *)scratch(S_XTB_EMU_CTRL, 256);
    if (!sc || !sS || !rhs || !yb || !ctrl) return e.err_code ? e.err_code : dkmc_fail(13, "xtb_emulate_slabs: no solver state", __FILE__, __LINE__);
    sS += X.ns_pad;
    XtbArgs B{};
    B.m = m; B.ns = ns; B.ns_pad = X.ns_pad; B.nK = X.nK; B.nW = X.nW; B.s = s;
    B.items = (const XItem *)g_xb.items + X.item_lo; B.item_n = X.item_n; B.tiles = g_xb.tiles; B.sub_base = (int)X.sub_base; B.tval = g_xb.tval;
    B.wrange = g_xb.wrange; B.nitem_w = g_xb.nitem_w; B.nrecords = X.nitems >> X.rec_shift;
    B.srow = g_xb.srow; B.sS = sS; B.nsrank = g_xb.nsrank; B.rp = g_xb.rp; B.ci = g_xb.ci; B.val = g_xb.val; B.sc = sc;
    B.ax = g_xb.ax; B.ay = g_xb.ay; B.az = g_xb.az; B.b = rhs; B.ctrl = ctrl; B.tol2 = tol * tol;
    B.nt_loads = (size_t)X.sub_n * XT_SUB * 8 > ((size_t)200 << 20); B.sharded = false; B.w_lo = X.w_lo; B.w_hi = X.w_hi;
    const int hint = e.x_iter_hint;
    double *yref = yb, *yslab = yb + m + 8;
    HIPCHK(hipMemsetAsync(yb, 0, (size_t)(m + 8) * 8 * 2, st));
    B.y = yref;
    int it_ref = 0, it_slab = 0; double rr = 0.0;
    int rc = 0;
    if (sweep_cap <= 0) { const int pd0 = e.x_poly; if (!e.x_slab_poly) e.x_poly = 0; rc = xtb_cg(B, &it_ref, &rr); e.x_poly = pd0; if (rc && rc != DKMC_XTB_BREAKDOWN) return rc; }
    const int ntiles = X.ntiles;
    int kc = std::max(1, std::min(XT_MAXKC, ntiles / nranks / 4096));
    if (ntiles <= 2048 * nranks) kc = std::max(1, std::min(XT_MAXKC, (ntiles + 1024 * nranks - 1) / (1024 * nranks)));
    std::vector<XShare> sh((size_t)nranks);
    for (int r = 0; r < nranks; ++r) {
        rc = xt_build_items(X.nK, X.nW, kc, ntiles, X.nsub_total, (const int *)g_xb.toff, (const XTile *)g_xb.tiles, nranks, r, S_XT_T_NITEMW, S_XT_T_ITEMS, S_XT_T_SPLIT, &sh[r], 2);
        if (rc) return rc;
        if ((sh[r].item_lo | sh[r].item_n) & 3) return dkmc_fail(48, "xtb_emulate_slabs: run list not padded to groups of four", __FILE__, __LINE__);
    }
    B.y = yslab;
    rc = xtb_cg_slab_emulate(B, nranks, sh.data(), time_rank, sweep_cap, &it_slab, &rr, times_us, xdoubles);
    e.x_iter_hint = hint;
    if (rc && rc != DKMC_XTB_BREAKDOWN) return rc;
    std::vector<double> h0((size_t)m), h1((size_t)m);
    HIPCHK(hipMemcpyAsync(h0.data(), yref, (size_t)m * 8, hipMemcpyDeviceToHost, st));
    HIPCHK(hipMemcpyAsync(h1.data(), yslab, (size_t)m * 8, hipMemcpyDeviceToHost, st));
    HIPCHK(hipStreamSynchronize(st));
    double md = 0.0, ma = 0.0;
    for (int i = 0; i < m; ++i) { md = std::max(md, fabs(h0[i] - h1[i])); ma = std::max(ma, fabs(h0[i])); }
    if (rel_diff) *rel_diff = sweep_cap > 0 ? -1.0 : (ma > 0.0 ? md / ma : md);
    if (iters_slab) *iters_slab = it_slab;
    if (iters_ref) *iters_ref = it_ref;
    if (rows_min_max) {
        std::vector<int> tab((size_t)nranks);
        HIPCHK(hipMemcpy(tab.data(), (int *)e.buf[S_XTB_SLAB_TAB] + 4096 + 32 + 2, (size_t)nranks * 4, hipMemcpyDeviceToHost));
        rows_min_max[0] = *std::min_element(tab.begin(), tab.end()); rows_min_max[1] = *std::max_element(tab.begin(), tab.end());
    }
    return e.err_code;
}

extern "C" int dkmc_xt_get_tiles(long long *ntiles, long long *nsub, int *tiles4, double *tval)
{
    Engine &e = eng(); const XTState &X = g_xt;
    if (!X.valid || comm_attached() || X.tile_n != X.ntiles) return dkmc_fail(13, "xt_get_tiles: needs the X of a single-GPU solve", __FILE__, __LINE__);
    HIPCHK(hipStreamSynchronize(e.stream));
    if (ntiles) *ntiles = X.ntiles;
    if (nsub) *nsub = X.nsub_total;
    static_assert(sizeof(XTile) == 16, "XTile is four ints");
    if (tiles4 && X.ntiles) HIPCHK(hipMemcpy(tiles4, g_xb.tiles, (size_t)X.ntiles * sizeof(XTile), hipMemcpyDeviceToHost));
    if (tval && X.nsub_total) HIPCHK(hipMemcpy(tval, g_xb.tval, (size_t)X.nsub_total * XT_SUB * 8, hipMemcpyDeviceToHost));
    return 0;
}
const xrp_t *xt_xs_rp() { return g_xb.rp; }
const int *xt_xs_col() { return g_xb.ci; }
const double *xt_xs_val() { return g_xb.val; }
bool xt_valid() { return g_xt.valid; }

int xt_export_csr(int *rows_out, long long *nnz_out, int *h_rp, int *h_col, double *h_data)
{
    Engine &e = eng(); const XTState &X = g_xt;
    if (!X.valid) return dkmc_fail(13, "get_last_X: no assembled X", __FILE__, __LINE__);
    if (comm_attached()) return dkmc_fail(13, "get_last_X: not available on a sharded X", __FILE__, __LINE__);
    HIPCHK(hipStreamSynchronize(e.stream));
    const long long nnz = X.xs_nnz + 2 * (long long)X.t_upper;
    if (rows_out) *rows_out = X.Nsub;
    if (nnz_out) *nnz_out = nnz;
    if (!h_rp && !h_col && !h_data) return 0;
    if (nnz > 2147483647LL || X.nsub_total > (1ll << 18)) return dkmc_fail(12, "get_last_X: X is too large for the int32 CSR copy of this call", __FILE__, __LINE__);
    std::vector<xrp_t> rp((size_t)X.Nsub + 1); std::vector<int> ci((size_t)X.xs_nnz); std::vector<double> va((size_t)X.xs_nnz);
    HIPCHK(hipMemcpy(rp.data(), g_xb.rp, rp.size() * sizeof(xrp_t), hipMemcpyDeviceToHost));
    HIPCHK(hipMemcpy(ci.data(), g_xb.ci, ci.size() * 4, hipMemcpyDeviceToHost));
    HIPCHK(hipMemcpy(va.data(), g_xb.val, va.size() * 8, hipMemcpyDeviceToHost));
    std::vector<XTile> tl((size_t)X.ntiles); std::vector<double> tv((size_t)X.nsub_total * XT_SUB); std::vector<int> srow((size_t)X.ns_pad);
    if (X.ntiles) HIPCHK(hipMemcpy(tl.data(), g_xb.tiles, tl.size() * sizeof(XTile), hipMemcpyDeviceToHost));
    if (X.nsub_total) HIPCHK(hipMemcpy(tv.data(), g_xb.tval, tv.size() * 8, hipMemcpyDeviceToHost));
    HIPCHK(hipMemcpy(srow.data(), g_xb.srow, srow.size() * 4, hipMemcpyDeviceToHost));
    std::vector<std::vector<std::pair<int, double>>> rowsv((size_t)X.Nsub);
    for (int i = 0; i < X.Nsub; ++i) for (xrp_t p = rp[i]; p < rp[i + 1]; ++p) rowsv[i].push_back({ci[p], va[p]});
    for (const XTile &t : tl) {
        int sl = 0;
        for (int q = 0; q < 8; ++q) {
            if (!((t.mask >> q) & 1u)) continue;
            const double *sb = tv.data() + ((size_t)t.soff + sl) * XT_SUB; ++sl;
// ... 19 lines not shown
```

### devicekmc_amd/csrc/xt_live.h

```cpp
#pragma once

XLive g_xlive;

constexpr double XTL_DROP_AUTO_THETA = 1e-10;
constexpr long long XTL_DROP_GATE = 246272;
double xtl_drop_rule(long long stored_subblocks, long long gate_override)
{
    const long long gate = gate_override > 0 ? gate_override : XTL_DROP_GATE;
    return stored_subblocks > 0 && stored_subblocks >= gate ? XTL_DROP_AUTO_THETA : 0.0;
}
extern "C" double dkmc_xtl_drop_rule(long long stored_subblocks) { return xtl_drop_rule(stored_subblocks, eng().x_tile_drop_gate); }

__global__ __launch_bounds__(XT_NT) void k_xtl_census(int nK, const XTile *__restrict__ tiles, int sub_base, const double *__restrict__ tval,
                                                      const double *__restrict__ sS, double theta, int unit, unsigned *__restrict__ lcmask,
                                                      int *__restrict__ tflag, unsigned long long *__restrict__ cnt)
{
    __shared__ double rs[XT_R], mx[XT_C / XT_SBW];
    const XTile td = tiles[blockIdx.x];
    const int tid = threadIdx.x, q = tid >> 5, c = tid & 31;
    if (tid < XT_R) rs[tid] = sS[XT_R * td.k + tid];
    __syncthreads();
    double m = 0.0;
    if ((td.mask >> q) & 1u) {
        const int sl = __popc(td.mask & ((1u << q) - 1u));
// ... 74 lines not shown
        if (re) atomicAdd(cnt + 3, (unsigned long long)re);
    }
}
__global__ __launch_bounds__(XT_NT) void k_xtl_compact(int nK, const XTile *__restrict__ tiles, int sub_base, const unsigned *__restrict__ lcmask,
                                                       const int *__restrict__ lsoff, const float4 *__restrict__ src32, float4 *__restrict__ dst32)
{
    const XTile td = tiles[blockIdx.x];
    const size_t ci = (size_t)td.w * nK + td.k;
    const unsigned lm = lcmask[ci] & td.mask;
    if (!lm) return;
    const float4 *s = src32 + (size_t)(td.soff - sub_base) * (XT_SUB / 4) + threadIdx.x;
    float4 *d = dst32 + (size_t)lsoff[ci] * (XT_SUB / 4) + threadIdx.x;
    int dl = 0;
#pragma unroll
    for (int q = 0; q < XT_C / XT_SBW; ++q)
        if ((lm >> q) & 1u) { d[(size_t)dl * (XT_SUB / 4)] = s[(size_t)__popc(td.mask & ((1u << q) - 1u)) * (XT_SUB / 4)]; ++dl; }
}
__global__ __launch_bounds__(XT_NT) void k_xtl_zero_dead(long long n, int per, int nW, const XTile *__restrict__ tiles, const int *__restrict__ tflag,
                                                         double *__restrict__ rowpartB)
{
    const long long i = (long long)blockIdx.x * blockDim.x + threadIdx.x;
    if (i >= n) return;
    const int t = (int)(i / per);
    if (tflag[t]) return;
    const XTile td = tiles[t];
    rowpartB[((size_t)td.k * nW + td.w) * per + (size_t)(i % per)] = 0.0;
}

static hipEvent_t g_xl_ev[3]; static bool g_xl_ev_ready = false;

static long long g_xtl_reread = 0;
static int xt_live_census(double theta, int unit, const double *sS, unsigned **lcmask_out, int **tflag_out, unsigned long long *h4)
{
    Engine &e = eng(); hipStream_t st = e.stream; const XTState &X = g_xt;
    const long long ncell = (long long)X.nK * X.nW;
    unsigned *lcmask = (unsigned *)scratch(S_XTL_CELLS, (size_t)(ncell + 4) * 4 * 3);
    int *tflag = (int *)scratch(S_XTL_TFLAG, (size_t)(X.ntiles + 8) * 4 + 32);
    if (!lcmask || !tflag) return e.err_code;
    unsigned long long *cnt = reinterpret_cast<unsigned long long *>(tflag + ((X.ntiles + 7) & ~7));
    HIPCHK(hipMemsetAsync(lcmask, 0, (size_t)(ncell + 4) * 4, st));
    HIPCHK(hipMemsetAsync(cnt, 0, 32, st));
    if (e.xtl_census_form == 1 && g_xb.tval32 && theta >= 1e-290)
        hipLaunchKernelGGL(k_xtl_census_img, dim3(X.ntiles), dim3(XT_NT), 0, st, X.nK, (const XTile *)g_xb.tiles, (int)X.sub_base, (const double *)g_xb.tval,
                           reinterpret_cast<const float4 *>(g_xb.tval32), sS, theta, unit, lcmask, tflag, cnt);
    else
        hipLaunchKernelGGL(k_xtl_census, dim3(X.ntiles), dim3(XT_NT), 0, st, X.nK, (const XTile *)g_xb.tiles, (int)X.sub_base, (const double *)g_xb.tval, sS, theta,
                           unit, lcmask, tflag, cnt);
    KCHK();
    HIPCHK(hipMemcpyAsync(h4, cnt, 32, hipMemcpyDeviceToHost, st));
    HIPCHK(hipStreamSynchronize(st));
    g_xtl_reread = (long long)h4[3];
    *lcmask_out = lcmask; *tflag_out = tflag;
    return 0;
}
extern "C" int dkmc_debug_xtl_census_form(int form) { const int was = eng().xtl_census_form; eng().xtl_census_form = form == 1 ? 1 : 0; return was; }
extern "C" long long dkmc_debug_xtl_census_reread(void) { return g_xtl_reread; }

int xt_live_build(double theta, int unit, const double *sS, XLive *lv)
{
    Engine &e = eng(); hipStream_t st = e.stream; const XTState &X = g_xt;
    *lv = XLive{};
    if (!(theta > 0.0) || !X.valid || comm_attached() || X.tile_n != X.ntiles || X.ntiles <= 0 || !g_xb.tval32 || !sS) return 0;
    const bool prof = e.profiling != 0;
    if (prof && !g_xl_ev_ready) { for (auto &ev : g_xl_ev) HIPCHK(hipEventCreate(&ev)); g_xl_ev_ready = true; }
    if (prof) HIPCHK(hipEventRecord(g_xl_ev[0], st));
    const int nK = X.nK, nW = X.nW;
    const long long ncell = (long long)nK * nW;
    unsigned *lcmask = nullptr; int *tflag = nullptr; unsigned long long h3[4] = {0, 0, 0, 0};
    if (int rc = xt_live_census(theta, unit, sS, &lcmask, &tflag, h3)) return rc;
    lv->tflag = tflag;
    lv->info[1] = X.ntiles; lv->info[2] = (long long)h3[0]; lv->info[3] = X.nsub_total; lv->info[4] = (long long)h3[1]; lv->info[5] = (long long)h3[2];
    const int nlive = (int)h3[0]; const long long nsub_live = (long long)h3[unit == 1 ? 2 : 1];
    if ((X.nsub_total - nsub_live) * 64 < X.nsub_total) { lv->state = -2; return 0; }
    int *ltoff = (int *)lcmask + (ncell + 4), *lsoff = ltoff + (ncell + 4);
    hipLaunchKernelGGL(k_xt_cell_counts, dim3((unsigned)((ncell + 255) / 256)), dim3(256), 0, st, ncell, (const unsigned *)lcmask, ltoff, lsoff);
    if (int rc = dkmc_exclusive_scan_i32(ltoff, ltoff, (int)ncell, ltoff + ncell)) return rc;
    if (int rc = dkmc_exclusive_scan_i32(lsoff, lsoff, (int)ncell, lsoff + ncell)) return rc;
    if (prof) HIPCHK(hipEventRecord(g_xl_ev[1], st));
    const size_t bytes = (size_t)(nsub_live + 4) * XT_SUB * 4;
    float *c32 = (float *)scratch_try(S_XTL_TVAL32, bytes);
    if (!c32) { lv->state = -1; return 0; }
    XTile *ltiles = (XTile *)scratch(S_XTL_TILES, (size_t)(nlive + 1) * sizeof(XTile));
    int2 *lwrange = (int2 *)scratch(S_XTL_WRANGE, (size_t)(nK + 4) * sizeof(int2));
    if (!ltiles || !lwrange) return e.err_code;
    hipLaunchKernelGGL(k_xtl_compact, dim3(X.ntiles), dim3(XT_NT), 0, st, nK, (const XTile *)g_xb.tiles, (int)X.sub_base, (const unsigned *)lcmask, (const int *)lsoff,
                       reinterpret_cast<const float4 *>(g_xb.tval32), reinterpret_cast<float4 *>(c32));
    hipLaunchKernelGGL(k_xt_tile_list, dim3((unsigned)((ncell + 255) / 256)), dim3(256), 0, st, nK, ncell, (const unsigned *)lcmask, (const int *)ltoff, (const int *)lsoff, ltiles);
    hipLaunchKernelGGL(k_xt_wrange, dim3((nK + 255) / 256), dim3(256), 0, st, nK, nW, (const unsigned *)lcmask, lwrange);
    KCHK();
    XShare sh{};
    if (int rc = xt_build_items(nK, nW, X.kc, nlive, nsub_live, ltoff, ltiles, 1, 0, S_XTL_NITEMW, S_XTL_ITEMS, S_XTL_SPLIT, &sh, 2)) return rc;
    if ((sh.item_lo | sh.item_n) & 3) return dkmc_fail(48, "live view: run list not padded to groups of four", __FILE__, __LINE__);
    if (prof) {
        HIPCHK(hipEventRecord(g_xl_ev[2], st));
        HIPCHK(hipEventSynchronize(g_xl_ev[2]));
        float ms = 0.f;
        HIPCHK(hipEventElapsedTime(&ms, g_xl_ev[0], g_xl_ev[1])); lv->ms[0] = ms;
        HIPCHK(hipEventElapsedTime(&ms, g_xl_ev[1], g_xl_ev[2])); lv->ms[1] = ms;
    }
    lv->tiles = ltiles; lv->items = sh.items ? sh.items + sh.item_lo : nullptr; lv->item_n = sh.item_n; lv->wrange = lwrange; lv->nitem_w = sh.nitem_w;
    lv->nrecords = sh.nitems >> sh.rec_shift; lv->nitems = sh.nitems; lv->tval32 = c32;
    lv->info[6] = (long long)bytes;
    lv->state = 1;
    return 0;
}
void xt_live_zero_dead(const XLive &lv, double *rowpartB, int so)
{
    const XTState &X = g_xt;
    if (lv.info[2] >= X.ntiles) return;
    const int per = XT_R * so;
    const long long n = (long long)X.ntiles * per;
    hipLaunchKernelGGL(k_xtl_zero_dead, dim3((unsigned)((n + XT_NT - 1) / XT_NT)), dim3(XT_NT), 0, eng().stream, n, per, X.nW, (const XTile *)g_xb.tiles, lv.tflag, rowpartB);
}

extern "C" int dkmc_get_x_tile_live_info(long long *info8, double *ms2)
{
    if (info8) { for (int c = 0; c < 8; ++c) info8[c] = g_xlive.info[c]; info8[0] = g_xlive.state; }
    if (ms2 && eng().profiling) { ms2[0] = g_xlive.ms[0]; ms2[1] = g_xlive.ms[1]; }
    return 0;
}
static const double *xt_live_sS()
{
    const double *vS = (const double *)eng().buf[S_CG_PS];
    return vS ? vS + g_xt.ns_pad : nullptr;
}
extern "C" int dkmc_xt_get_live(double theta, int *live_per_tile, double *sS_out)
{
    Engine &e = eng(); const XTState &X = g_xt;
    const double *sS = xt_live_sS();
    if (!X.valid || comm_attached() || X.tile_n != X.ntiles || X.ntiles <= 0 || !sS) return dkmc_fail(13, "xt_get_live: needs the X of a single-GPU solve", __FILE__, __LINE__);
    unsigned *lcmask = nullptr; int *tflag = nullptr; unsigned long long h3[4];
    if (int rc = xt_live_census(theta, 0, sS, &lcmask, &tflag, h3)) return rc;
    if (live_per_tile) HIPCHK(hipMemcpy(live_per_tile, tflag, (size_t)X.ntiles * 4, hipMemcpyDeviceToHost));
    if (sS_out) HIPCHK(hipMemcpy(sS_out, sS, (size_t)X.ns * 8, hipMemcpyDeviceToHost));
    return e.err_code;
}
__global__ void k_xtl_tile_masks(int ntiles, int nK, const XTile *__restrict__ tiles, const unsigned *__restrict__ lcmask, int *__restrict__ out)
{
    const int t = blockIdx.x * blockDim.x + threadIdx.x;
    if (t < ntiles) out[t] = (int)lcmask[(size_t)tiles[t].w * nK + tiles[t].k];
}
extern "C" int dkmc_xt_get_live_masks(double theta, int *mask_per_tile)
{
    Engine &e = eng(); const XTState &X = g_xt;
    const double *sS = xt_live_sS();
    if (!X.valid || comm_attached() || X.tile_n != X.ntiles || X.ntiles <= 0 || !sS) return dkmc_fail(13, "xt_get_live_masks: needs the X of a single-GPU solve", __FILE__, __LINE__);
    unsigned *lcmask = nullptr; int *tflag = nullptr; unsigned long long h3[4];
    if (int rc = xt_live_census(theta, 1, sS, &lcmask, &tflag, h3)) return rc;
    if (mask_per_tile) {
        hipLaunchKernelGGL(k_xtl_tile_masks, dim3((X.ntiles + 255) / 256), dim3(256), 0, e.stream, X.ntiles, X.nK, (const XTile *)g_xb.tiles, (const unsigned *)lcmask, tflag);
        KCHK();
        HIPCHK(hipMemcpyAsync(mask_per_tile, tflag, (size_t)X.ntiles * 4, hipMemcpyDeviceToHost, e.stream));
        HIPCHK(hipStreamSynchronize(e.stream));
    }
    return e.err_code;
}
int xt_live_for_test(XLive *lv)
{
    const double *sS = xt_live_sS();
    if (int rc = xt_live_build(eng().x_tile_drop, eng().x_tile_drop_unit, sS, lv)) return rc;
    if (lv->state != 1) return dkmc_fail(13, "no live image at the current threshold and unit (dkmc_set_x_tile_drop; dkmc_get_x_tile_live_info)", __FILE__, __LINE__);
    return 0;
}
```

### devicekmc_amd/csrc/xtb.hip

```cpp
#include "xtiles.h"
#include "slab.h"
#include <hip/hip_ext.h>
#include <algorithm>
#include <functional>
#include <type_traits>
#include <vector>

#define XB_SP 16
#define XB_MAXPOLY 16
#define XB_MAXPOLY1 20
#define XB_DSPLIT 8
#define XB_NG 6
typedef double dbl4 __attribute__((ext_vector_type(4)));
#define XB_MFMA(a, b, c) __builtin_amdgcn_mfma_f64_16x16x4f64((a), (b), (c), 0, 0, 0)
#define XB_MFMA4(a, b, c) __builtin_amdgcn_mfma_f64_4x4x4f64((a), (b), (c), 0, 0, 0)

__device__ __forceinline__ double xtb_aux(int row, int col)
{
    unsigned long long h = (unsigned long long)row * 0x9E3779B97F4A7C15ull + (unsigned long long)col * 0xC2B2AE3D27D4EB4Full + 12345ull;
    h ^= h >> 29; h *= 0xBF58476D1CE4E5B9ull; h ^= h >> 32;
    return (double)(h >> 11) * (1.0 / 4503599627370496.0) - 1.0;
}
struct XbAux { double lo[3], hi[3]; int k[16][3]; unsigned long long mm[6]; int hs, pad_; };
__device__ __forceinline__ double xtb_rhs(const double *__restrict__ b, int row, int v, int s, const XbAux *__restrict__ aux = nullptr,
// ... 383 lines not shown
        xrp_t p = a + g;
        if (dlist) {
            const int n = row == 0 ? nd0 : nd1, l0 = row == 0 ? 0 : nd0;
            const int ia = l0 + (int)((long long)n * part / XB_DSPLIT), ib = l0 + (int)((long long)n * (part + 1) / XB_DSPLIT);
            int i = ia + g;
            for (; i + 48 < ib; i += 64) {
                const int q0 = dlist[i], q1 = dlist[i + 16], q2 = dlist[i + 32], q3 = dlist[i + 48];
                const int c0 = ci[q0], c1 = ci[q1], c2 = ci[q2], c3 = ci[q3];
                s0 += val[q0] * (sc[c0] * P[(size_t)c0 * XB_SP + v]); s1 += val[q1] * (sc[c1] * P[(size_t)c1 * XB_SP + v]);
                s2 += val[q2] * (sc[c2] * P[(size_t)c2 * XB_SP + v]); s3 += val[q3] * (sc[c3] * P[(size_t)c3 * XB_SP + v]);
            }
            for (; i < ib; i += 16) { const int q0 = dlist[i], c0 = ci[q0]; s0 += val[q0] * (sc[c0] * P[(size_t)c0 * XB_SP + v]); }
            p = b;
        }
        for (; p + 48 < b; p += 64) {
            const int c0 = ci[p], c1 = ci[p + 16], c2 = ci[p + 32], c3 = ci[p + 48];
            const double a0 = val[p], a1 = val[p + 16], a2 = val[p + 32], a3 = val[p + 48];
            s0 += a0 * (sc[c0] * P[(size_t)c0 * XB_SP + v]); s1 += a1 * (sc[c1] * P[(size_t)c1 * XB_SP + v]);
            s2 += a2 * (sc[c2] * P[(size_t)c2 * XB_SP + v]); s3 += a3 * (sc[c3] * P[(size_t)c3 * XB_SP + v]);
        }
        for (; p < b; p += 16) { const int c0 = ci[p]; s0 += val[p] * (sc[c0] * P[(size_t)c0 * XB_SP + v]); }
        red[g][v] = (s0 + s1) + (s2 + s3);
        __syncthreads();
        if (g == 0) {
            double s = 0.0;
#pragma unroll
            for (int u = 0; u < 16; ++u) s += red[u][v];
            drvpart[(row * XB_DSPLIT + part) * XB_SP + v] = s;
        }
        return;
    }
    const int li = xtb_xcd_block((int)gridDim.x - 2 * XB_DSPLIT, (int)blockIdx.x - 2 * XB_DSPLIT) * 16 + g;
    const int row = rowlist ? (li < nlist ? rowlist[li] : m) : 2 + li;
    const bool ok = row < m;
    const xrp_t p0 = ok ? rp[row] : 0, p1 = ok ? rp[row + 1] : 0;
    const int nsr = ok ? nsrank[row] : 0;
    const double scr = ok ? sc[row] : 0.0;
    XnSums s = {0.0, 0.0, 0.0, 0.0};
    for (xrp_t base = p0; base < p1; base += 64) {
        int cm[4]; double wm[4];
#pragma unroll
        for (int b = 0; b < 4; ++b) { const xrp_t pe = base + 16 * b + v; cm[b] = pe < p1 ? ci[pe] : -1; wm[b] = pe < p1 ? val[pe] : 0.0; }
#pragma unroll
        for (int b = 0; b < 4; ++b) wm[b] = cm[b] >= 0 ? wm[b] * sc[cm[b]] : 0.0;
#pragma unroll
        for (int b = 0; b < 4; ++b) {
            if (base + 16 * b >= p1) break;
            s = xn_batch16(P, v, xn_entry(cm[b], wm[b]), s);
        }
    }
    const double sum = (s.s0 + s.s1) + (s.s2 + s.s3);
    if (ok) T[(size_t)row * XB_SP + v] = nsr < 0 ? scr * sum : sum;
}

__device__ __forceinline__ double xtb_list_sum(const double *__restrict__ p, size_t stride, int first, int n, int step)
{
    double a0 = 0.0, a1 = 0.0, a2 = 0.0, a3 = 0.0;
    for (int c = first; c < n; c += 16 * step) {
        double x[16];
#pragma unroll
        for (int u = 0; u < 16; ++u) { const int cu = c + u * step; x[u] = cu < n ? p[(size_t)cu * stride] : 0.0; }
#pragma unroll
        for (int u = 0; u < 16; u += 4) { a0 += x[u]; a1 += x[u + 1]; a2 += x[u + 2]; a3 += x[u + 3]; }
    }
    return (a0 + a1) + (a2 + a3);
}
__device__ __forceinline__ void xtb_list_sum2(const double *__restrict__ p, size_t stride, size_t off, int first, int n, int v, double &sa, double &sb)
{
    const bool odd = (v & 1) != 0;
    const dbl2 *__restrict__ q = reinterpret_cast<const dbl2 *>(odd ? p - 1 + off : p);
    const size_t st2 = stride >> 1;
    double a0 = 0.0, a1 = 0.0, a2 = 0.0, a3 = 0.0, b0 = 0.0, b1 = 0.0, b2 = 0.0, b3 = 0.0;
    for (int c = first; c < n; c += 16) {
        dbl2 x[16];
#pragma unroll
        for (int u = 0; u < 16; ++u) { const int cu = c + u; x[u] = cu < n ? __builtin_nontemporal_load(q + (size_t)cu * st2) : (dbl2)(0.0); }
#pragma unroll
        for (int u = 0; u < 16; u += 4) { a0 += x[u].x; a1 += x[u + 1].x; a2 += x[u + 2].x; a3 += x[u + 3].x; b0 += x[u].y; b1 += x[u + 1].y; b2 += x[u + 2].y; b3 += x[u + 3].y; }
    }
    const double sx = (a0 + a1) + (a2 + a3), sy = (b0 + b1) + (b2 + b3);
    const double got = xor_lane<1>(odd ? sx : sy);
    sa = odd ? got : sx; sb = odd ? sy : got;
}
__global__ __launch_bounds__(XT_NT) void k_xtb_fold_local(int ns, int nK, int nW, int so, const int2 *__restrict__ wrange, const int *__restrict__ nitem_w,
                                                          const double *__restrict__ rowpartB, const double *__restrict__ colpartB, double *__restrict__ xbuf,
                                                          const XCtrl *ctrl, int flag_rank0, int w_lo, int w_hi, const long long *__restrict__ sdst = nullptr)
{
    if (ctrl->done) return;
    const int v = threadIdx.x & 15, r4 = threadIdx.x >> 4;
    const int rec_shift = nitem_w[2 * (nW + 2)];
    for (int k = blockIdx.x; k < nK; k += gridDim.x) {
        int2 wr = wrange[k];
        wr.x = max(wr.x, w_lo); wr.y = min(wr.y, w_hi);
        const int wk = k / (XT_C / XT_R);
        const bool mine = wk >= w_lo && wk < w_hi;
        const int nc = mine ? nitem_w[wk] >> rec_shift : 0, cbase = nitem_w[nW + 2 + wk] >> rec_shift;
        double tA = 0.0, tB = 0.0;
        if (v < so) {
            const double *rpp = rowpartB + ((size_t)k * nW * XT_R + r4) * so + v;
            const double *cpp = colpartB + ((size_t)cbase * XT_C + (XT_R * (k % (XT_C / XT_R)) + r4)) * so + v;
            const size_t rs = (size_t)XT_R * so, cs = (size_t)XT_C * so;
            double cA, cB, rA_, rB_;
            xtb_list_sum2(cpp, cs, (size_t)16 * so, 0, nc, v, cA, cB);
            xtb_list_sum2(rpp, rs, (size_t)16 * so, wr.x, wr.y, v, rA_, rB_);
            tA = cA + rA_; tB = cB + rB_;
            const int sA = XT_R * k + r4, sB = sA + 16;
            if (sA < ns) xbuf[(sdst ? (size_t)sdst[sA] : (size_t)sA * so) + v] = tA;
            if (sB < ns) xbuf[(sdst ? (size_t)sdst[sB] : (size_t)sB * so) + v] = tB;
        }
    }
    if (!sdst && blockIdx.x == 0 && threadIdx.x == 0) {
        xbuf[(size_t)ns * so] = (flag_rank0 && ctrl->done_local) ? 1.0 : 0.0;
        xbuf[(size_t)ns * so + 1] = ctrl->abort_local ? 1.0 : 0.0;
    }
}
__global__ void k_xtb_abort_word(XCtrl *ctrl, double *xbuf, size_t slot) { ctrl->abort_local = 1; xbuf[slot] = 1.0; }
__global__ void k_xtb_set_sharded(XCtrl *ctrl) { ctrl->sharded = 1; }

template <int INIT, int SH = 0, int NF = 0>
__global__ __launch_bounds__(XT_NT) void k_xtb_rows(int ns, int nK, int nW, int m, int s, int so, const int2 *__restrict__ wrange, const int *__restrict__ nitem_w,
                                                    const double *__restrict__ rowpartB, const double *__restrict__ colpartB,
                                                    const int *__restrict__ srow, const double *__restrict__ sS, const int *__restrict__ nsrank,
                                                    const double *__restrict__ sc, const double *__restrict__ drvpart, double *__restrict__ T,
                                                    const double *__restrict__ P, double *__restrict__ R, const double *__restrict__ b,
                                                    double *__restrict__ gpart, XCtrl *ctrl, const double *__restrict__ xbuf, int it, int nr,
                                                    const XbAux *__restrict__ aux, const double *__restrict__ ax, const double *__restrict__ ay, const double *__restrict__ az)
{
    const size_t xslot = (size_t)ns * so + 2;
    __shared__ double lg[4][XB_NG / 2][4][64];
    __shared__ int sdone;
    if (threadIdx.x == 0) {
        sdone = ctrl->done;
        if (SH && !sdone) {
            bool ab = false;
            for (int r = 0; r < nr; ++r) ab |= xbuf[r * xslot + (size_t)ns * so + 1] != 0.0;
            if (xbuf[(size_t)ns * so] != 0.0 || ab) {
                sdone = 1;
                if (blockIdx.x == 0) { ctrl->done = it + 1 > 0 ? it + 1 : 1; if (ab) ctrl->aborted = 1; }
            }
        }
    }
    __syncthreads();
    if (sdone) return;
    const int v = threadIdx.x & 15, r4 = threadIdx.x >> 4;
    const int wv = threadIdx.x >> 6, lane = threadIdx.x & 63;
    const int rec_shift = nitem_w[2 * (nW + 2)];
    dbl4 G[XB_NG];
#pragma unroll
    for (int g = 0; g < XB_NG; ++g) G[g] = (dbl4)(0.0);
    for (int k = blockIdx.x; k < nK; k += gridDim.x) {
        const int2 wr = wrange[k];
        const int wk = k / (XT_C / XT_R);
        const int nc = nitem_w[wk] >> rec_shift, cbase = nitem_w[nW + 2 + wk] >> rec_shift;
        double tA = 0.0, tB = 0.0;
        const int sA = XT_R * k + r4, sB = sA + 16;
        if (SH) {
            if (v < so) {
                for (int r = 0; r < nr; ++r) {
                    if (sA < ns) tA += xbuf[r * xslot + (size_t)sA * so + v];
                    if (sB < ns) tB += xbuf[r * xslot + (size_t)sB * so + v];
                }
            }
        } else if (!NF && v < so) {
            const double *rpp = rowpartB + ((size_t)k * nW * XT_R + r4) * so + v;
            const double *cpp = colpartB + ((size_t)cbase * XT_C + (XT_R * (k % (XT_C / XT_R)) + r4)) * so + v;
            const size_t rs = (size_t)XT_R * so, cs = (size_t)XT_C * so;
            double cA, cB, rA_, rB_;
            xtb_list_sum2(cpp, cs, (size_t)16 * so, 0, nc, v, cA, cB);
            xtb_list_sum2(rpp, rs, (size_t)16 * so, wr.x, wr.y, v, rA_, rB_);
            tA = cA + rA_; tB = cB + rB_;
        }
        double pA = 0.0, pB = 0.0, rA = 0.0, rB = 0.0;
        if (sA < ns) {
            const int row = srow[sA]; const size_t o = (size_t)row * XB_SP + v;
            if (NF) tA = T[o]; else { tA = sS[sA] * (T[o] + tA); T[o] = tA; }
            if (INIT) { rA = tA - xtb_rhs(b, row, v, s, aux, ax, ay, az, sc); R[o] = rA; } else { pA = P[o]; rA = R[o]; }
        } else tA = 0.0;
        if (sB < ns) {
            const int row = srow[sB]; const size_t o = (size_t)row * XB_SP + v;
            if (NF) tB = T[o]; else { tB = sS[sB] * (T[o] + tB); T[o] = tB; }
            if (INIT) { rB = tB - xtb_rhs(b, row, v, s, aux, ax, ay, az, sc); R[o] = rB; } else { pB = P[o]; rB = R[o]; }
        } else tB = 0.0;
        if (!INIT) {
            G[0] = XB_MFMA(pA, tA, G[0]); G[1] = XB_MFMA(pA, rA, G[1]); G[2] = XB_MFMA(tA, rA, G[2]); G[3] = XB_MFMA(tA, tA, G[3]); G[5] = XB_MFMA(pA, pA, G[5]);
            G[0] = XB_MFMA(pB, tB, G[0]); G[1] = XB_MFMA(pB, rB, G[1]); G[2] = XB_MFMA(tB, rB, G[2]); G[3] = XB_MFMA(tB, tB, G[3]); G[5] = XB_MFMA(pB, pB, G[5]);
        }
        G[4] = XB_MFMA(rA, rA, G[4]); G[4] = XB_MFMA(rB, rB, G[4]);
    }
    {
        const int chunk = ((m + (int)gridDim.x - 1) / (int)gridDim.x + 3) & ~3;
        const int i0 = blockIdx.x * chunk, i1 = min(m, i0 + chunk);
        for (int r0 = i0 + 4 * wv; r0 < i1; r0 += 64) {
            double tv[4], pv[4], rv[4]; int sr[4];
#pragma unroll
            for (int u = 0; u < 4; ++u) {
                const int row = r0 + 16 * u + (lane >> 4);
                const bool in = row < i1;
                const size_t o = (size_t)(in ? row : i0) * XB_SP + v;
                sr[u] = in ? nsrank[row] : 0;
                tv[u] = T[o];
                if (!INIT) { pv[u] = P[o]; rv[u] = R[o]; }
            }
#pragma unroll
            for (int u = 0; u < 4; ++u) {
                const int row = r0 + 16 * u + (lane >> 4);
                if (r0 + 16 * u >= i1) break;
                const bool use = row < i1 && sr[u] < 0;
                const size_t o = (size_t)row * XB_SP + v;
                double t_ = use ? tv[u] : 0.0, p_ = 0.0, r_ = 0.0;
                if (!NF && use && row < 2) {
                    double sd = 0.0;
#pragma unroll
                    for (int w = 0; w < XB_DSPLIT; ++w) sd += drvpart[(row * XB_DSPLIT + w) * XB_SP + v];
                    t_ = sc[row] * sd; T[o] = t_;
                }
                if (INIT) { if (use) { r_ = t_ - xtb_rhs(b, row, v, s, aux, ax, ay, az, sc); R[o] = r_; } }
                else if (use) { p_ = pv[u]; r_ = rv[u]; }
                if (!INIT) { G[0] = XB_MFMA(p_, t_, G[0]); G[1] = XB_MFMA(p_, r_, G[1]); G[2] = XB_MFMA(t_, r_, G[2]); G[3] = XB_MFMA(t_, t_, G[3]); G[5] = XB_MFMA(p_, p_, G[5]); }
                G[4] = XB_MFMA(r_, r_, G[4]);
            }
        }
    }
#pragma unroll
    for (int h = 0; h < 2; ++h) {
        __syncthreads();
#pragma unroll
        for (int g = 0; g < XB_NG / 2; ++g)
#pragma unroll
            for (int u = 0; u < 4; ++u) lg[wv][g][u][lane] = G[h * (XB_NG / 2) + g][u];
        __syncthreads();
        for (int e = threadIdx.x; e < (XB_NG / 2) * 256; e += XT_NT) {
            const int g = e >> 8, u = (e >> 6) & 3, l = e & 63;
            gpart[(size_t)blockIdx.x * (XB_NG * 256) + h * (XB_NG / 2) * 256 + e] = (lg[0][g][u][l] + lg[1][g][u][l]) + (lg[2][g][u][l] + lg[3][g][u][l]);
        }
    }
}
__global__ __launch_bounds__(XT_NT) void k_xtb_fold_rows(int ns, int nK, int nW, int so, const int2 *__restrict__ wrange, const int *__restrict__ nitem_w,
                                                         const double *__restrict__ rowpartB, const double *__restrict__ colpartB, const int *__restrict__ srow,
                                                         const double *__restrict__ sS, const double *__restrict__ sc, const double *__restrict__ drvpart,
                                                         double *__restrict__ T, const XCtrl *ctrl)
{
    if (ctrl->done) return;
    const int v = threadIdx.x & 15, r4 = threadIdx.x >> 4;
    const int rec_shift = nitem_w[2 * (nW + 2)];
    if (blockIdx.x == 0 && threadIdx.x < 32) {
        const int row = threadIdx.x >> 4;
        double sd = 0.0;
#pragma unroll
        for (int w = 0; w < XB_DSPLIT; ++w) sd += drvpart[(row * XB_DSPLIT + w) * XB_SP + v];
        T[(size_t)row * XB_SP + v] = sc[row] * sd;
    }
    for (int k = blockIdx.x; k < nK; k += gridDim.x) {
        const int2 wr = wrange[k];
        const int wk = k / (XT_C / XT_R);
        const int nc = nitem_w[wk] >> rec_shift, cbase = nitem_w[nW + 2 + wk] >> rec_shift;
        double tA = 0.0, tB = 0.0;
        const int sA = XT_R * k + r4, sB = sA + 16;
        if (v < so) {
            const double *rpp = rowpartB + ((size_t)k * nW * XT_R + r4) * so + v;
            const double *cpp = colpartB + ((size_t)cbase * XT_C + (XT_R * (k % (XT_C / XT_R)) + r4)) * so + v;
            const size_t rs = (size_t)XT_R * so, cs = (size_t)XT_C * so;
            double cA, cB, rA_, rB_;
            xtb_list_sum2(cpp, cs, (size_t)16 * so, 0, nc, v, cA, cB);
            xtb_list_sum2(rpp, rs, (size_t)16 * so, wr.x, wr.y, v, rA_, rB_);
            tA = cA + rA_; tB = cB + rB_;
        }
        if (sA < ns) { const size_t o = (size_t)srow[sA] * XB_SP + v; T[o] = sS[sA] * (T[o] + tA); }
        if (sB < ns) { const size_t o = (size_t)srow[sB] * XB_SP + v; T[o] = sS[sB] * (T[o] + tB); }
    }
}
__global__ __launch_bounds__(XT_NT) void k_xtb_gred(int npart, const double *__restrict__ gpart, double *__restrict__ gfin, const XCtrl *ctrl)
{
    __shared__ double red[16][17];
    if (ctrl->done) return;
    const int el = threadIdx.x & 15, q = threadIdx.x >> 4;
    const int e = 16 * (int)blockIdx.x + el;
    red[q][el] = xtb_list_sum(gpart + e, (size_t)XB_NG * 256, q, npart, 16);
    __syncthreads();
    if (q == 0) {
        double a = 0.0;
#pragma unroll
        for (int u = 0; u < 16; ++u) a += red[u][el];
        gfin[e] = a;
    }
}

#define XB_M(name) double (*name)[17]
#define XB_WSYNC() do { __builtin_amdgcn_fence(__ATOMIC_RELEASE, "wavefront"); __builtin_amdgcn_wave_barrier(); __builtin_amdgcn_fence(__ATOMIC_ACQUIRE, "wavefront"); } while (0)
__device__ __forceinline__ void xtb_mm(XB_M(C), XB_M(A), XB_M(B), bool ta, double alpha, XB_M(D), double delta)
{
    const int j = threadIdx.x & 15, i0 = threadIdx.x >> 4;
    double bcol[16], acc[4];
#pragma unroll
    for (int k = 0; k < 16; ++k) bcol[k] = B[k][j];
#pragma unroll
    for (int u = 0; u < 4; ++u) {
        const int i = i0 + 4 * u;
        double a0 = 0.0, a1 = 0.0;
#pragma unroll
        for (int k = 0; k < 16; k += 2) { a0 += (ta ? A[k][i] : A[i][k]) * bcol[k]; a1 += (ta ? A[k + 1][i] : A[i][k + 1]) * bcol[k + 1]; }
        acc[u] = alpha * (a0 + a1) + (D ? delta * D[i][j] : 0.0);
    }
    XB_WSYNC();
#pragma unroll
    for (int u = 0; u < 4; ++u) C[i0 + 4 * u][j] = acc[u];
    XB_WSYNC();
}
__device__ __forceinline__ void xtb_symmetrise(XB_M(A), int s)
{
    double acc[4];
#pragma unroll
    for (int u = 0; u < 4; ++u) { const int e = (int)threadIdx.x + 64 * u, i = e >> 4, j = e & 15; acc[u] = (i < s && j < s) ? 0.5 * (A[i][j] + A[j][i]) : 0.0; }
    XB_WSYNC();
#pragma unroll
    for (int u = 0; u < 4; ++u) { const int e = (int)threadIdx.x + 64 * u; A[e >> 4][e & 15] = acc[u]; }
    XB_WSYNC();
}
__device__ __forceinline__ bool xtb_chol(XB_M(A), int s)
{
    bool ok = true;
    if ((int)threadIdx.x >= s && threadIdx.x < 16) A[threadIdx.x][threadIdx.x] = 1.0;
    XB_WSYNC();
    for (int k = 0; k < s; ++k) {
        const double d = A[k][k];
        if (!(d > 0.0)) ok = false;
        const double ld = sqrt(d > 0.0 ? d : 1.0);
        XB_WSYNC();
        if ((int)threadIdx.x == k) A[k][k] = ld;
        else if ((int)threadIdx.x > k && (int)threadIdx.x < s) A[threadIdx.x][k] = A[threadIdx.x][k] / ld;
        XB_WSYNC();
        const int j = threadIdx.x & 15, i0 = threadIdx.x >> 4;
        const double ljk = A[j][k];
#pragma unroll
        for (int u = 0; u < 4; ++u) {
            const int i = i0 + 4 * u;
            if (i > k && j > k && j <= i && i < s) A[i][j] -= A[i][k] * ljk;
        }
        XB_WSYNC();
    }
    return ok;
}
__device__ __forceinline__ void xtb_chol_solve(XB_M(X), XB_M(L), XB_M(B), int s)
{
    const int j = threadIdx.x & 15;
    double x[16];
    if (threadIdx.x < 16) {
#pragma unroll
// ... 422 lines not shown
template <class Body>
static int xtb_reenter(int rc, double rr0, int *iters_out, double *rr_out, Body body)
{
    for (int round = 1; rc == DKMC_XTB_AGAIN && round < 6; ++round) {
        int it2 = 0; double rr1 = 0.0;
        rc = body(&it2, &rr1);
        if (iters_out) *iters_out += it2;
        if (rc == DKMC_XTB_AGAIN && !(rr1 < 0.25 * rr0)) rc = 0;
        rr0 = rr1;
    }
    if (rc == DKMC_XTB_AGAIN) rc = 0;
    if (rr_out) *rr_out = rr0;
    return rc;
}
int xtb_cg(const XtbArgs &A, int *iters_out, double *rr_out)
{
    bool peer_used = false;
    double rr0 = 0.0;
    if (A.sharded && eng().x_slab && comm_nranks() > 1 && comm_nranks() <= XS_MAXR && A.ay && A.az) {
        const int nr = comm_nranks(), me = comm_rank();
        const int rc = xtb_cg_slab(A, nr, me, nullptr, -1, iters_out, &rr0);
        return xtb_reenter(rc, rr0, iters_out, rr_out, [&](int *it, double *rr) { return xtb_cg_slab(A, nr, me, nullptr, -1, it, rr); });
    }
    XbNPack npk{};
    const bool packed = !A.sharded && A.m > 2 && A.ns > 0 && eng().x_poly > 0 && eng().x_nmul_form == 1;
    if (packed) { if (int rcp = xtb_npack(A, A.m, nullptr, scratch, 0, &npk)) return rcp; }
    const XbNPack *np = packed ? &npk : nullptr;
    Engine &e = eng();
    const bool f32 = e.x_tile_f32 != 0 && A.tval32 != nullptr && !A.sharded && A.m > 2 && A.ns > 0 && e.x_poly > 0 && A.tol2 >= 1e-16;
    if (f32) e.stats.x_tile_stream = 1; else if (e.stats.x_tile_stream == 1) e.stats.x_tile_stream = 0;
    e.stats.x_tile_f64_rounds = f32 ? 0 : 1;
    XLive *lv = nullptr;
    const double theta = e.x_tile_drop > 0.0 ? e.x_tile_drop : (e.x_tile_drop_auto && A.warm ? xtl_drop_rule(A.stored_subblocks, e.x_tile_drop_gate) : 0.0);
    e.x_tile_drop_used = 0.0;
    if (f32 && theta > 0.0 && A.item_n > 0 && A.tiles == g_xb.tiles && A.tval32 == g_xb.tval32) {
        if (int rcl = xt_live_build(theta, e.x_tile_drop_unit, A.sS, &g_xlive)) return rcl;
        if (g_xlive.state == 1) { lv = &g_xlive; e.x_tile_drop_used = theta; }
    }
    int rc = xtb_cg_body(A, iters_out, &rr0, &peer_used, np, f32, lv);
    rc = xtb_reenter(rc, rr0, iters_out, rr_out, [&](int *it, double *rr) { ++e.stats.x_tile_f64_rounds; return xtb_cg_body(A, it, rr, &peer_used, np, false, nullptr); });
    if (rc != 0 && rc != DKMC_XTB_BREAKDOWN && peer_used) comm_peer_drop();
    return rc;
}
static int xtb_cg_body(const XtbArgs &A, int *iters_out, double *rr_out, bool *peer_used, const XbNPack *np, bool f32, XLive *lv)
{
    Engine &e = eng(); hipStream_t st = e.stream;
    const int m = A.m, s = A.s, so = 4 * ((s + 3) / 4);
    const size_t pan = (size_t)m * XB_SP;
    const long long ncell = (long long)A.nK * A.nW;
    const int ng = std::max(128, std::min(A.nK, 4096));
    double *panels = (double *)scratch(S_XTB_PANELS, (pan * 3 + m + 16) * 8);
    double *QS = (double *)scratch(S_XTB_QS, (size_t)A.ns_pad * XB_SP * 8);
    double *rowpartB = (double *)scratch(S_XTB_ROWPART, (size_t)(ncell + 1) * XT_R * so * 8);
    const int nrec = std::max(A.nrecords, lv ? lv->nrecords : 0);
    double *colpartB = (double *)scratch(S_XTB_COLPART, (size_t)(nrec + 1) * XT_C * so * 8);
    double *gpart = (double *)scratch(S_XTB_GRAM, (size_t)ng * XB_NG * 256 * 8);
    double *small = (double *)scratch(S_XTB_SMALL, (size_t)(4 * 256 + 2 * XB_DSPLIT * XB_SP + XB_NG * 256) * 8);
    if (!panels || !QS || !rowpartB || !colpartB || !gpart || !small) return e.err_code;
    double *R = panels, *P = panels + pan, *T = panels + 2 * pan, *y0 = panels + 3 * pan;
    double *mats = small, *drvpart = small + 4 * 256, *gfin = drvpart + 2 * XB_DSPLIT * XB_SP;
    const int pd = xtb_poly_degree(e, A);
    e.stats.xb_poly_used = pd;
    const bool one = pd > 0 && xtb_poly_one(e);
    const int pn = one ? xtb_poly1_degree(e, pd) : pd;
    e.x_poly_form_used = one ? 1 : 0; e.x_poly_products = one ? pn : 2 * pd;
    double *Vp = nullptr, *W1 = nullptr, *W2 = nullptr, *Zp = nullptr, *bz = nullptr, *Up = nullptr;
    if (pd > 0) {
        Vp = (double *)scratch(S_XTB_PRE_V, (pan + m + 16) * 8); W1 = (double *)scratch(S_XTB_PRE_W1, pan * 8); W2 = (double *)scratch(S_XTB_PRE_W2, pan * 8);
        Zp = (double *)scratch(S_XTB_PRE_Z, pan * 8);
        if (!Vp || !W1 || !W2 || !Zp) return e.err_code;
        bz = Vp + pan;
        HIPCHK(hipMemsetAsync(bz, 0, (size_t)(m + 16) * 8, st));
        if (one) {
            Up = (double *)scratch(S_XTB_PRE_U, pan * 8);
            if (!Up) return e.err_code;
            HIPCHK(hipMemsetAsync(Vp, 0, pan * 8, st));
            HIPCHK(hipMemsetAsync(Up, 0, pan * 8, st));
        }
    }
    double pc[XB_MAXPOLY1 + 1] = {1.0}, qmin = 1.0;
    if (one) xtb_poly1_coeffs(pn, pc, &qmin); else xtb_poly_coeffs(pd, pc);
    const double tol2_loop = one ? A.tol2 * qmin : (pd > 0 ? A.tol2 / 2.25 : A.tol2);
    HIPCHK(hipMemsetAsync(QS, 0, (size_t)A.ns_pad * XB_SP * 8, st));
    HIPCHK(hipMemsetAsync(rowpartB, 0, (size_t)(ncell + 1) * XT_R * so * 8, st));
    HIPCHK(hipMemsetAsync(colpartB, 0, (size_t)(nrec + 1) * XT_C * so * 8, st));
    HIPCHK(hipMemsetAsync(A.ctrl, 0, sizeof(XCtrl), st));
    const bool sharded = A.sharded;
    const int nr = sharded ? comm_nranks() : 1, me = sharded ? comm_rank() : 0;
    double *xbuf = nullptr;
    const size_t xcount = (size_t)A.ns * so + 2;
    const bool peer = sharded && comm_peer_ready(xcount);
    *peer_used = peer;
    int xpar = 0;
    if (sharded) {
        if (!peer) { xbuf = (double *)scratch(S_CG_XCHG, xcount * nr * 8); if (!xbuf) return e.err_code; }
        hipLaunchKernelGGL(k_xtb_set_sharded, dim3(1), dim3(1), 0, st, A.ctrl);
    }
    const bool keep_aux = A.yaux != nullptr && pd == 0;
    double *Ypanel = keep_aux ? (double *)scratch(S_XTB_YPANEL, pan * 8) : nullptr;
    if (keep_aux && !Ypanel) return e.err_code;
    XbAux *aux = nullptr; int hs = 1;
    if (int rc = xtb_aux_setup(A, &aux, &hs)) return rc;
    int local_fail = 0;
    hipLaunchKernelGGL(k_xtb_init, dim3((unsigned)((pan + 255) / 256)), dim3(256), 0, st, m, (const double *)A.y, A.sc, A.nsrank, y0, P, QS,
                       (const double *)((keep_aux && A.yaux_valid) ? A.yaux : nullptr), hs, s, Ypanel);
    struct XbView { const XItem *items; int item_n; const XTile *tiles; const int2 *wrange; const int *nitem_w; };
    const XbView full{A.items, A.item_n, A.tiles, A.wrange, A.nitem_w};
    const XbView live = lv ? XbView{lv->items, lv->item_n, lv->tiles, lv->wrange, lv->nitem_w} : full;
    const XbView *vw = &full;
    const int ntb = (A.item_n + 3) / 4;
    const int nnb = 2 * XB_DSPLIT + (std::max(m - 2, 1) + 15) / 16;
    const int gs = grid_blocks((m + 15) / 16, 4, 2048);
    const bool prof = e.profiling != 0;
    if (prof) if (int prc = g_loop_events.begin(EventSampler::LONG | EventSampler::SHORT)) return prc;
    const bool side = sharded && m > 20000 && ntb > 0 && side_stream_init(g_xb_side) == 0;
    const float *t32 = nullptr;
    auto product = [&](hipEvent_t e0, hipEvent_t e1) {
        int sl = 0;
        if (side) {
            SideStream &S = g_xb_side; sl = (int)(S.seq++ % SideStream::RING);
            (void)hipEventRecord(S.a[sl], st);
            (void)hipStreamWaitEvent(S.st, S.a[sl], 0);
            hipLaunchKernelGGL(k_xtb_neigh, dim3(nnb), dim3(XT_NT), 0, S.st, m, A.rp, A.ci, A.val, (const double *)P, A.sc, A.nsrank, (const XCtrl *)A.ctrl, T, drvpart);
            (void)hipEventRecord(S.b[sl], S.st);
        }
        if (vw->item_n > 0) xtb_apply({vw->item_n, vw->items, vw->tiles, A.sub_base, A.tval, QS, A.nW, rowpartB, colpartB, A.ctrl, t32}, A.nt_loads, so, 0, st, e0, e1);
        if (side) (void)hipStreamWaitEvent(st, g_xb_side.b[sl], 0);
        else hipLaunchKernelGGL(k_xtb_neigh, dim3(nnb), dim3(XT_NT), 0, st, m, A.rp, A.ci, A.val, (const double *)P, A.sc, A.nsrank, (const XCtrl *)A.ctrl, T, drvpart);
    };
    const XbNRank nk{m, nullptr, np, QS, A.ctrl};
    auto applyL = [&](double *src, double *dst, bool qs) {
        xtb_applyL(st, A, pn, pc, src, dst, W1, W2, qs, [](int, double *) { return 0; }, [&](bool, auto f) { f(nk, [](double *p) { return p; }); return 0; });
    };
    auto fold_rows = [&](double *Tt) {
        hipLaunchKernelGGL(k_xtb_fold_rows, dim3(std::max(ng, 1)), dim3(XT_NT), 0, st, A.ns, A.nK, A.nW, so, vw->wrange, vw->nitem_w, (const double *)rowpartB, (const double *)colpartB,
                           A.srow, A.sS, A.sc, (const double *)drvpart, Tt, (const XCtrl *)A.ctrl);
    };
    auto product_pre = [&](hipEvent_t e0, hipEvent_t e1) {
        applyL(P, Vp, true);
        double *Pk = P, *Tk = T; P = Vp; T = Zp;
        t32 = f32 ? A.tval32 : nullptr;
        if (lv) { vw = &live; t32 = lv->tval32; }
        product(e0, e1);
        t32 = nullptr;
        P = Pk; T = Tk;
        fold_rows(Zp);
        vw = &full;
        applyL(Zp, T, false);
    };
    auto product_one = [&](hipEvent_t e0, hipEvent_t e1) {
        t32 = f32 ? A.tval32 : nullptr;
        if (lv) { vw = &live; t32 = lv->tval32; }
        product(e0, e1);
        t32 = nullptr;
        fold_rows(T);
        vw = &full;
        applyL(T, Up, false);
    };
    auto gram_one = [&](hipEvent_t e2, hipEvent_t e3) {
        hipExtLaunchKernelGGL(k_xtb_gram1, dim3(ng), dim3(XT_NT), 0, st, e2, e3, 0, m, (const double *)P, (const double *)Vp, (const double *)T, (const double *)Up,
                              (const double *)R, (const double *)Zp, gpart, (const XCtrl *)A.ctrl);
    };
    auto step = [&](int it) {
        if (one) hipLaunchKernelGGL(k_xtb_step1, dim3(gs), dim3(XT_NT), 0, st, m, it, (const double *)mats, y0, R, Zp, P, Vp, (const double *)T, (const double *)Up, A.sc,
                                    A.nsrank, QS, (const XCtrl *)A.ctrl);
        else hipLaunchKernelGGL(k_xtb_step, dim3(gs), dim3(XT_NT), 0, st, m, it, (const double *)mats, y0, R, P, (const double *)T, A.sc, A.nsrank, QS, (const XCtrl *)A.ctrl,
                                (const int *)nullptr, Ypanel);
    };
    const double *bsel = A.b;
#define XB_ROWS_ARGS(IT_) A.ns, A.nK, A.nW, m, s, so, (lv && !init ? live : full).wrange, (lv && !init ? live : full).nitem_w, (const double *)rowpartB, (const double *)colpartB, A.srow, A.sS, A.nsrank, A.sc, \
                     (const double *)drvpart, T, (const double *)P, R, bsel, gpart, A.ctrl, (const double *)xbuf, IT_, nr, (const XbAux *)aux, A.ax, A.ay, A.az
    auto rows = [&](bool init, int itn, hipEvent_t e2, hipEvent_t e3) -> int {
        if (sharded) {
            if (peer) { xbuf = comm_peer_slots(xpar); }
            hipLaunchKernelGGL(k_xtb_fold_local, dim3(std::max(A.nK, 1)), dim3(XT_NT), 0, st, A.ns, A.nK, A.nW, so, A.wrange, A.nitem_w, (const double *)rowpartB,
                               (const double *)colpartB, xbuf + me * xcount, (const XCtrl *)A.ctrl, 1, A.w_lo, A.w_hi);
            if (hipGetLastError() != hipSuccess || local_fail) {
                if (!local_fail) local_fail = dkmc_fail(92, "block-CG: launch failed between two collectives", __FILE__, __LINE__);
                hipLaunchKernelGGL(k_xtb_abort_word, dim3(1), dim3(1), 0, st, A.ctrl, xbuf + me * xcount, (size_t)A.ns * so + 1);
            }
            if (peer) {
                if (int rcx = comm_peer_exchange(xpar, xcount, &A.ctrl->done, &A.ctrl->aborted, &A.ctrl->xchg_timeout, itn + 2)) return rcx;
                xpar ^= 1;
            } else if (int rcx = comm_allgather_f64(xbuf, xcount)) return rcx;
            xtb_rows_launch<1, 0>(init, ng, st, e2, e3, XB_ROWS_ARGS(itn));
        } else if (pd > 0) xtb_rows_launch<0, 1>(init, ng, st, e2, e3, XB_ROWS_ARGS(itn));
        else xtb_rows_launch<0, 0>(init, ng, st, e2, e3, XB_ROWS_ARGS(itn));
        return 0;
    };
    product(nullptr, nullptr);
    if (one) {
        fold_rows(T);
        if (lv) xt_live_zero_dead(*lv, rowpartB, so);
        if (int rcx = rows(true, -1, nullptr, nullptr)) return rcx;
        applyL(R, Zp, false);
        gram_one(nullptr, nullptr);
    } else if (pd > 0) {
        fold_rows(T);
        if (lv) xt_live_zero_dead(*lv, rowpartB, so);
        hipLaunchKernelGGL(k_xtb_pre_resid, dim3((unsigned)((pan + 255) / 256)), dim3(256), 0, st, m, (const double *)T, A.b, Zp);
        applyL(Zp, T, false);
        bsel = bz;
        HIPCHK(hipMemsetAsync(y0, 0, (size_t)m * 8, st));
    }
    if (!one) if (int rcx = rows(true, -1, nullptr, nullptr)) return rcx;
    hipLaunchKernelGGL(k_xtb_gred, dim3(XB_NG * 16), dim3(XT_NT), 0, st, ng, (const double *)gpart, gfin, (const XCtrl *)A.ctrl);
    hipLaunchKernelGGL(k_xtb_small, dim3(1), dim3(256), 0, st, -1, s, (const double *)gfin, mats, A.ctrl, tol2_loop);
    hipLaunchKernelGGL(k_xtb_zero, dim3((unsigned)((pan + 255) / 256)), dim3(256), 0, st, (long long)pan, P);
    step(-1);
    KCHK();
    XCtrl h{};
    if (int rcx = cg_poll_loop(A.ctrl, h, LaunchPlan::hinted_three_quarters(e.x_iter_hint), st, XTB_NO_CONVERGENCE, prof && ntb > 0 && live.item_n > 0 ? &g_loop_events : nullptr,
                               [&](int it, const hipEvent_t *ev) -> int {
            if (sharded && g_xtb_fault_iter >= 0 && it >= g_xtb_fault_iter) { g_xtb_fault_iter = -1; local_fail = dkmc_fail(91, "injected fault (block-CG iteration)", __FILE__, __LINE__); }
            if (one) { product_one(ev[0], ev[1]); gram_one(ev[2], ev[3]); }
            else {
                if (pd > 0) product_pre(ev[0], ev[1]);
                else product(ev[0], ev[1]);
                if (int rcx = rows(false, it, ev[2], ev[3])) return rcx;
            }
            hipLaunchKernelGGL(k_xtb_gred, dim3(XB_NG * 16), dim3(XT_NT), 0, st, ng, (const double *)gpart, gfin, (const XCtrl *)A.ctrl);
            hipLaunchKernelGGL(k_xtb_small, dim3(1), dim3(256), 0, st, it, s, (const double *)gfin, mats, A.ctrl, tol2_loop);
            step(it);
            return 0;
        })) return rcx;
#undef XB_ROWS_ARGS
    if (lv) lv->info[7] = h.iters;
    if (local_fail) return local_fail;
    if (h.xchg_timeout) return dkmc_fail(48, "block-CG: the peer-write exchange timed out waiting for a peer's slot", __FILE__, __LINE__);
    if (h.aborted) return dkmc_fail(46, "a peer rank aborted the sharded current solve", __FILE__, __LINE__);
    if (e.err_code) return e.err_code;
    bool again = false;
    if (pd > 0) {
        HIPCHK(hipMemsetAsync(A.ctrl, 0, sizeof(XCtrl), st));
        if (one) HIPCHK(hipMemcpyAsync(A.y, y0, (size_t)m * 8, hipMemcpyDeviceToDevice, st));
        else {
            hipLaunchKernelGGL(k_xtb_pre_col0, dim3((unsigned)((pan + 255) / 256)), dim3(256), 0, st, m, (const double *)y0, Zp);
            applyL(Zp, Vp, false);
            hipLaunchKernelGGL(k_xtb_pre_add, dim3((m + 255) / 256), dim3(256), 0, st, m, (const double *)Vp, A.y);
        }
        if (!h.pad[0]) {
            hipLaunchKernelGGL(k_xtb_pre_col0, dim3((unsigned)((pan + 255) / 256)), dim3(256), 0, st, m, (const double *)A.y, P);
            hipLaunchKernelGGL(k_xtb_qs_from, dim3((unsigned)((pan + 255) / 256)), dim3(256), 0, st, m, (const double *)P, A.sc, A.nsrank, QS, (const XCtrl *)A.ctrl);
            product(nullptr, nullptr);
            fold_rows(T);
            const int nrp = std::min(XB_RR_MAXPART, (m + 1023) / 1024);
            hipLaunchKernelGGL(k_xtb_pre_rr_part, dim3(nrp), dim3(256), 0, st, m, (const double *)T, A.b, gpart);
            hipLaunchKernelGGL(k_xtb_pre_rr, dim3(1), dim3(256), 0, st, nrp, (const double *)gpart, bz + m);
            double rr_true = 0.0;
            HIPCHK(hipMemcpyAsync(&rr_true, bz + m, 8, hipMemcpyDeviceToHost, st));
            HIPCHK(hipStreamSynchronize(st));
            h.rr[h.iters & 1] = rr_true;
            again = rr_true > A.tol2;
            if (e.x_tile_f32_fail_once) { e.x_tile_f32_fail_once = 0; again = true; }
        }
    } else
    HIPCHK(hipMemcpyAsync(A.y, y0, (size_t)m * 8, hipMemcpyDeviceToDevice, st));
    if (keep_aux) hipLaunchKernelGGL(k_xtb_yaux_out, dim3((unsigned)((pan + 255) / 256)), dim3(256), 0, st, m, (const int *)nullptr, (const double *)Ypanel, A.sc, A.yaux);
    return xtb_finish(h, true, again, prof, iters_out, rr_out);
}

#include "xtb_slab.inc"
int xtb_cg_slab_emulate(const XtbArgs &A, int nr, const XShare *shares, int time_rank, int sweep_cap, int *iters_out, double *rr_out, double *times_us, long long *xdoubles)
{
    g_slab_sweep_cap = sweep_cap;
    double rr0 = 0.0;
    int rc = xtb_cg_slab(A, nr, 0, shares, time_rank, iters_out, &rr0);
    const double nmul_us = g_slab_last.nmul_us;
    if (sweep_cap > 0) { if (rc == DKMC_XTB_AGAIN) rc = 0; if (rr_out) *rr_out = rr0; }
    else rc = xtb_reenter(rc, rr0, iters_out, rr_out, [&](int *it, double *rr) { return xtb_cg_slab(A, nr, 0, shares, -1, it, rr); });
    g_slab_last.nmul_us = nmul_us;
    g_slab_sweep_cap = 0;
    if (times_us) for (int c = 0; c < 8; ++c) times_us[c] = g_slab_times.us[c];
    if (xdoubles) for (int c = 0; c < 3; ++c) xdoubles[c] = g_slab_xbytes[c];
    return rc;
}
extern "C" int dkmc_xtb_slab_last(int *exchanges_per_sweep, long long *halo_doubles_per_exchange, double *nmul_us)
{
    if (exchanges_per_sweep) *exchanges_per_sweep = g_slab_last.exchanges;
    if (halo_doubles_per_exchange) *halo_doubles_per_exchange = g_slab_last.halo_doubles;
    if (nmul_us) *nmul_us = g_slab_last.nmul_us;
    return 0;
}

__global__ void k_xtb_test_panel(int ns, double *__restrict__ QS)
{
    const int i = blockIdx.x * blockDim.x + threadIdx.x;
    if (i >= ns * XB_SP) return;
    const int r = i >> 4, v = i & 15;
    QS[xtb_qs_pos(r, v)] = 0.25 + (double)((((unsigned)r * 2654435761u) ^ ((unsigned)v * 40503u)) >> 20) / 4096.0 + 0.125 * v;
}
__global__ void k_xtb_test_column(int ns, int v, const double *__restrict__ QS, double *__restrict__ vS)
{
    const int r = blockIdx.x * blockDim.x + threadIdx.x;
    if (r < ns) vS[r] = QS[xtb_qs_pos(r, v)];
}
__global__ void k_xtb_test_compare(int ns, int v, const int *__restrict__ srow, const double *__restrict__ T, const double *__restrict__ ref, double *__restrict__ out)
{
    const int r = blockIdx.x * blockDim.x + threadIdx.x;
    if (r >= ns) return;
    const double a = T[(size_t)srow[r] * XB_SP + v], b = ref[r];
    atomicMax(reinterpret_cast<unsigned long long *>(out), (unsigned long long)__double_as_longlong(fabs(a - b)));
    atomicMax(reinterpret_cast<unsigned long long *>(out + 1), (unsigned long long)__double_as_longlong(fabs(b)));
}
int xt_tile_sums_mv(const double *vS, double *out);
extern "C" int dkmc_xtb_check_product(int width, double *max_abs_diff, double *max_abs)
{
    Engine &e = eng(); hipStream_t st = e.stream; const XTState &X = g_xt;
    if (!X.valid || comm_attached() || X.tile_n != X.ntiles || X.ns <= 0) return dkmc_fail(13, "xtb_check_product: needs the X of a single-GPU solve", __FILE__, __LINE__);
    const int m = X.Nsub, ns = X.ns, s = std::max(2, std::min(width, 16)), so = 4 * ((s + 3) / 4);
    const size_t pan = (size_t)m * XB_SP;
    const long long ncell = (long long)X.nK * X.nW;
    const int nrec = X.nitems >> X.rec_shift, ng = 64;
    double *panels = (double *)scratch(S_XTB_PANELS, (pan * 3 + m + 16) * 8);
    double *QS = (double *)scratch(S_XTB_QS, (size_t)X.ns_pad * XB_SP * 8);
    double *rowpartB = (double *)scratch(S_XTB_ROWPART, (size_t)(ncell + 1) * XT_R * so * 8);
    double *colpartB = (double *)scratch(S_XTB_COLPART, (size_t)(nrec + 1) * XT_C * so * 8);
    double *gpart = (double *)scratch(S_XTB_GRAM, (size_t)4096 * XB_NG * 256 * 8);
    double *small = (double *)scratch(S_XTB_SMALL, (size_t)(4 * 256 + 2 * XB_DSPLIT * XB_SP + XB_NG * 256) * 8);
    double *tmp = (double *)scratch(S_XT_T_MISC, (size_t)4 * X.ns_pad * 8);
    XCtrl *ctrl = (XCtrl *)scratch(S_MISC2, 256);
    double *sS = (double *)e.buf[S_CG_PS], *sc = (double *)e.buf[S_CG_S], *rhs = (double *)e.buf[S_X_RHS];
    if (!panels || !QS || !rowpartB || !colpartB || !gpart || !small || !tmp || !ctrl || !sS || !sc || !rhs) return e.err_code ? e.err_code : dkmc_fail(13, "xtb_check_product: no solver state", __FILE__, __LINE__);
    sS += X.ns_pad;
    double *T = panels + 2 * pan, *R = panels, *P = panels + pan, *drvpart = small + 4 * 256;
    double *vS = tmp, *ref = tmp + X.ns_pad, *res = tmp + 2 * (size_t)X.ns_pad;
    HIPCHK(hipMemsetAsync(tmp, 0, (size_t)4 * X.ns_pad * 8, st));
    HIPCHK(hipMemsetAsync(QS, 0, (size_t)X.ns_pad * XB_SP * 8, st));
// ... 327 lines not shown
```

### devicekmc_amd/csrc/xtiles.h

```cpp
#pragma once
#include "xshared.h"
#include "cg_host.h"

#define XT_R 32
#define XT_C 256
#define XT_SBW 32
#define XT_SUB (XT_R * XT_SBW)
#define XT_NT 256
#define XT_MAXKC 32

typedef double dbl2 __attribute__((ext_vector_type(2)));
__host__ __device__ static inline int xt_tval32_pos(int r, int c) { return (((r >> 3) * 64 + (r & 3) * 16 + (c >> 1)) << 2) + (((r >> 2) & 1) << 1) + (c & 1); }

struct __attribute__((aligned(16))) XTile { int k, w; unsigned mask; int soff; };
struct __attribute__((aligned(32))) XItem { int t0, t1, w, c, k0; unsigned mask0; int soff0, pad; };
struct XCtrl { double rr[2]; int done_local, sharded; int done; int iters; int abort_local, aborted; int pad[2]; int xchg_timeout, pad2; };

struct SNodes {
    const double *x, *y, *z, *cb;
    const int *flag, *slot, *mr;
    const int *slotA;
};

struct XTState {
    int Nsub = 0, ns = 0, ns_pad = 0, nK = 0, nW = 0, ntiles = 0, nitems = 0, kc = 1, maxchunk = 1, rec_shift = 0;
    long long nsub_total = 0, xs_nnz = 0;
    unsigned long long t_upper = 0;
    int item_lo = 0, item_n = 0, tile_lo = 0, tile_n = 0, w_lo = 0, w_hi = 0; long long sub_base = 0, sub_n = 0;
    bool valid = false;
};

struct XTBuffers {
    SNodes S; int *srow; XTile *tiles; XItem *items; int2 *wrange; int *nitem_w; double *tval, *rowpart, *colpart;
    float *tval32;
    xrp_t *rp, *dpos; int *ci; double *val; int *nsrank;
    unsigned *cmask; int *toff;
    const double *ax, *ay, *az;
};

extern XTState g_xt;
extern XTBuffers g_xb;

struct XLive {
    int state = 0;
    const XTile *tiles = nullptr; const XItem *items = nullptr; int item_n = 0; const int2 *wrange = nullptr; const int *nitem_w = nullptr; int nrecords = 0;
    int nitems = 0;
    const float *tval32 = nullptr;
    const int *tflag = nullptr;
    long long info[8] = {0, 0, 0, 0, 0, 0, 0, 0}; double ms[2] = {0.0, 0.0};
};
extern XLive g_xlive;
int xt_live_build(double theta, int unit, const double *sS, XLive *lv);
double xtl_drop_rule(long long stored_subblocks, long long gate_override);
void xt_live_zero_dead(const XLive &lv, double *rowpartB, int so);
int xt_live_for_test(XLive *lv);

#define DKMC_XTB_AGAIN 1001
#define DKMC_XTB_BREAKDOWN 1000
struct XtbArgs {
    int m, ns, ns_pad, nK, nW;
    int s;
    const XItem *items; int item_n;
    const XTile *tiles; int sub_base; const double *tval;
    const float *tval32;
    const int2 *wrange; const int *nitem_w; int nrecords;
    const int *srow; const double *sS; const int *nsrank;
    const xrp_t *rp; const int *ci; const double *val;
    const double *sc;
    const double *ax, *ay, *az;
    const double *b;
    double *y;
    double *yaux; int yaux_valid;
    XCtrl *ctrl; double tol2; bool nt_loads;
    bool sharded; int w_lo, w_hi;
    bool warm;
    long long stored_subblocks;
};
int xtb_cg(const XtbArgs &A, int *iters_out, double *rr_out);
struct XShare { int nitems, maxchunk, item_lo, item_n, tile_lo, tile_n, w_lo, w_hi; long long sub_base, sub_n; XItem *items; int *nitem_w; int rec_shift; };
int xtb_cg_slab_emulate(const XtbArgs &A, int nr, const XShare *shares, int time_rank, int sweep_cap, int *iters_out, double *rr_out, double *times_us, long long *xdoubles);
__global__ void k_xt_vec_mul(int m, double *__restrict__ y, const double *__restrict__ s);
```

### devicekmc_amd/lib.py

```python
import ctypes as C
import os

_HERE = os.path.dirname(os.path.abspath(__file__))
LIB_PATH = os.path.join(_HERE, "libdevicekmc_hip.so")

c_int_p = C.POINTER(C.c_int)
c_dbl_p = C.POINTER(C.c_double)
vp = C.c_void_p


class dkmc_gpubuf(C.Structure):
    _PTRS = ["site_charge", "site_power", "site_potential_boundary", "site_potential_charge", "site_temperature",
             "site_CB_edge", "T_bg", "atom_power", "atom_CB_edge", "atom_virtual_potentials", "atom_charge",
             "site_element", "atom_element", "site_x", "site_y", "site_z", "atom_x", "atom_y", "atom_z",
             "metal_types", "sigma", "k", "lattice", "freq", "neigh_idx", "site_layer",
             "Device_row_ptr_d", "Device_col_indices_d", "contact_left_row_ptr", "contact_left_col_indices",
             "contact_right_row_ptr", "contact_right_col_indices"]
    _INTS = ["Device_nnz", "contact_left_nnz", "contact_right_nnz", "num_metal_types_", "N_", "nn_", "N_atom_"]
    _fields_ = [(n, vp) for n in _PTRS] + [(n, C.c_int) for n in _INTS]


class dkmc_stats(C.Structure):
    _fields_ = [("cg_iters_K", C.c_int), ("cg_iters_CB", C.c_int), ("cg_iters_X", C.c_int),
                ("cg_rr_K", C.c_double), ("cg_rr_CB", C.c_double), ("cg_rr_X", C.c_double),
                ("n_events", C.c_int), ("n_charged", C.c_int), ("N_atom", C.c_int),
                ("X_nnz", C.c_longlong), ("psum_last", C.c_double),
                ("spmv_long_ms", C.c_double), ("spmv_short_ms", C.c_double),
                ("spmv_long_launches", C.c_int), ("spmv_short_launches", C.c_int),
                ("spmv_long_nnz", C.c_longlong), ("spmv_short_nnz", C.c_longlong),
                ("spmv_long_rows", C.c_int), ("spmv_short_rows", C.c_int),
                ("spmv_segments", C.c_int), ("spmv_pad", C.c_int), ("spmv_segment_entries", C.c_longlong),
                ("comm_ranks", C.c_int), ("comm_local_segments", C.c_int), ("comm_count_per_rank", C.c_longlong),
                ("comm_ms", C.c_double), ("comm_launches", C.c_int), ("comm_pad", C.c_int),
                ("spmv_tiles", C.c_int), ("spmv_pad2", C.c_int), ("spmv_tile_entries", C.c_longlong),
                ("xt_subblocks", C.c_longlong), ("xt_local_subblocks", C.c_longlong), ("xt_items", C.c_int), ("xt_kc", C.c_int),
                ("xt_sparse_nnz", C.c_longlong), ("xt_ns", C.c_int), ("xt_split_launch", C.c_int),
                ("kcg_ms", C.c_double), ("kcg_iters_timed", C.c_int), ("kcg_blocked", C.c_int), ("pair_ms", C.c_double), ("pair_evaluated", C.c_longlong), ("pair_tested", C.c_longlong), ("xt_records", C.c_longlong), ("tcache_bytes", C.c_longlong), ("kcg_bytes", C.c_longlong), ("xb_aux", C.c_int), ("xb_poly_used", C.c_int), ("xb_width", C.c_int), ("xb_fallback", C.c_int), ("x_tile_stream", C.c_int), ("x_tile_f64_rounds", C.c_int), ("x_tile_f32_bytes", C.c_longlong)]


class dkmc_xtb_ctrl(C.Structure):
    _fields_ = [("rr", C.c_double * 2), ("done_local", C.c_int), ("sharded", C.c_int), ("done", C.c_int), ("iters", C.c_int),
                ("abort_local", C.c_int), ("aborted", C.c_int), ("pad", C.c_int * 2), ("xchg_timeout", C.c_int), ("pad2", C.c_int)]


ALLGATHER_FN = C.CFUNCTYPE(C.c_int, C.c_void_p, C.c_size_t, C.c_int, C.c_int, C.c_void_p)


_I, _D = C.c_int, C.c_double
SYMBOLS = {
    "dkmc_last_error": (C.c_char_p, []),
    "dkmc_clear_error": (None, []),
    "dkmc_get_stats": (C.POINTER(dkmc_stats), []),
    "dkmc_get_gpu_info": (_I, [C.c_char_p, _I, _I]),
    "dkmc_set_gpu": (_I, [_I]),
    "dkmc_set_stream": (_I, [vp]),
    "dkmc_synchronize": (_I, []),
    "dkmc_set_cg_tolerance": (None, [_D]),
    "dkmc_set_cb_edge_domain": (None, [_I]),
    "dkmc_set_x_block": (None, [_I]),
    "dkmc_get_x_block": (_I, []),
    "dkmc_set_k_slab": (None, [_I]),
    "dkmc_get_k_slab": (_I, []),
    "dkmc_xt_tile_census": (_I, [C.POINTER(C.c_longlong)]),
    "dkmc_set_x_items": (None, [_I]),
    "dkmc_set_x_poly": (None, [_I]),
    "dkmc_get_x_poly": (_I, []),
    "dkmc_set_x_poly_auto": (None, [_I]),
    "dkmc_get_x_poly_auto": (_I, []),
    "dkmc_set_x_poly_auto_rows": (None, [_I, _I]),
    "dkmc_set_x_poly_form": (None, [_I]),
    "dkmc_get_x_poly_form": (_I, []),
    "dkmc_get_x_poly_form_used": (_I, []),
    "dkmc_get_x_poly_products": (_I, []),
    "dkmc_debug_set_x_poly1_degree": (None, [_I]),
    "dkmc_set_x_tile_f32": (None, [_I]),
    "dkmc_get_x_tile_f32": (_I, []),
    "dkmc_set_x_tile_drop": (None, [_D]),
    "dkmc_get_x_tile_drop": (_D, []),
    "dkmc_set_x_tile_drop_unit": (None, [_I]),
    "dkmc_get_x_tile_drop_unit": (_I, []),
    "dkmc_set_x_tile_drop_auto": (None, [_I]),
    "dkmc_get_x_tile_drop_auto": (_I, []),
    "dkmc_get_x_tile_drop_used": (_D, []),
    "dkmc_get_x_tile_live_info": (_I, [C.POINTER(C.c_longlong), c_dbl_p]),
    "dkmc_xt_get_live": (_I, [_D, vp, vp]),
    "dkmc_xt_get_live_masks": (_I, [_D, vp]),
    "dkmc_debug_fail_true_residual_once": (None, []),
    "dkmc_set_x_static_tiles": (None, [_I]),
    "dkmc_get_x_static_tiles": (_I, []),
    "dkmc_get_x_static_info": (_I, [C.POINTER(C.c_longlong)]),
    "dkmc_debug_x_static_verify": (_I, [_I]),
    "dkmc_debug_get_x_static_verify": (_I, [C.POINTER(C.c_longlong)]),
    "dkmc_x_static_strips": (_I, [_I]),
    "dkmc_x_static_rule": (_I, [_I]),
    "dkmc_debug_set_x_static_gate": (None, [_I]),
    "dkmc_xt_get_srow": (_I, [c_int_p, vp]),
    "dkmc_xt_get_diag": (_I, [vp]),
    "dkmc_set_x_nmul_form": (None, [_I]),
    "dkmc_get_x_nmul_form": (_I, []),
    "dkmc_set_x_nmul_lane_bytes": (None, [_I]),
    "dkmc_get_x_nmul_lane_bytes": (_I, []),
    "dkmc_set_x_nmul_window": (None, [_I]),
    "dkmc_get_x_nmul_window": (_I, []),
    "dkmc_debug_set_x_nmul_window": (None, [_I, _I]),
    "dkmc_set_x_apply_form": (None, [_I]),
    "dkmc_get_x_apply_form": (_I, []),
    "dkmc_set_x_slab": (None, [_I]),
    "dkmc_get_x_slab": (_I, []),
    "dkmc_set_x_slab_poly": (None, [_I]),
    "dkmc_get_x_slab_poly": (_I, []),
    "dkmc_set_x_aux_warm": (None, [_I]),
    "dkmc_get_x_aux_warm": (_I, []),
    "dkmc_set_x_aux": (None, [_I]),
    "dkmc_get_x_aux": (_I, []),
    "dkmc_set_k_blocked": (None, [_I]),
    "dkmc_get_k_blocked": (_I, []),
    "dkmc_set_k_blocked_large": (None, [_I]),
    "dkmc_get_k_blocked_large": (_I, []),
    "dkmc_set_k_window_word_bytes": (None, [_I]),
    "dkmc_get_k_window_word_bytes": (_I, []),
    "dkmc_kcg_form_info": (_I, [C.POINTER(dkmc_gpubuf), C.POINTER(C.c_longlong)]),
    "dkmc_kcg_form_words": (_I, [C.POINTER(dkmc_gpubuf), C.POINTER(C.c_longlong)]),
    "dkmc_debug_kbw_halfword_pos": (_I, [_I, _I]),
    "dkmc_debug_kbw_segment_cap": (None, [_I]),
    "dkmc_set_pair_cutoff": (None, [_D]),
    "dkmc_reset_pair_sum_cache": (None, []),
    "dkmc_set_pair_form": (None, [_I]),
    "dkmc_get_pair_form": (_I, []),
    "dkmc_get_pair_sum_info": (_I, [C.POINTER(C.c_longlong), C.POINTER(_D)]),
    "dkmc_set_tcache_budget": (None, [C.c_longlong]),
    "dkmc_set_current_warm_start": (None, [_I]),
    "dkmc_get_current_warm_start": (_I, []),
    "dkmc_get_current_warm_vector": (_I, [C.POINTER(dkmc_gpubuf), vp, _I, c_int_p]),
    "dkmc_set_current_warm_vector": (_I, [C.POINTER(dkmc_gpubuf), vp, _I]),
    "dkmc_get_current_warm_aux": (_I, [C.POINTER(dkmc_gpubuf), vp, C.c_longlong, C.POINTER(C.c_longlong)]),
    "dkmc_set_current_warm_aux": (_I, [C.POINTER(dkmc_gpubuf), vp, C.c_longlong]),
    "dkmc_set_profiling": (None, [_I]),
    "dkmc_set_x_format": (None, [_I]),
    "dkmc_get_x_format": (_I, []),
    "dkmc_gpubuf_create": (_I, [C.POINTER(dkmc_gpubuf), _I, _I, _I, _I, vp, vp, vp, vp, vp, vp, _D, _D, _D, vp]),
    "dkmc_gpubuf_free": (_I, [C.POINTER(dkmc_gpubuf)]),
    "dkmc_gpubuf_sync_host_to_gpu": (_I, [C.POINTER(dkmc_gpubuf), vp, vp, vp, vp, vp, vp, vp, vp, _D]),
    "dkmc_gpubuf_sync_gpu_to_host": (_I, [C.POINTER(dkmc_gpubuf), vp, vp, vp, vp, vp, vp, vp, vp, vp]),
    "dkmc_copy_power_from_gpu": (_I, [C.POINTER(dkmc_gpubuf), vp]),
    "dkmc_copy_charge_to_gpu": (_I, [C.POINTER(dkmc_gpubuf), vp]),
    "dkmc_copy_Tbg_to_gpu": (_I, [C.POINTER(dkmc_gpubuf), _D]),
    "dkmc_copy_to_const_memory": (_I, [vp, vp, vp, vp, _I]),
    "dkmc_build_neighbor_index": (_I, [_I, vp, vp, vp, vp, _I, _D, c_int_p, vp]),
    "dkmc_initialize_sparsity": (_I, [C.POINTER(dkmc_gpubuf), _I, _D, _I]),
    "dkmc_free_sparsity": (_I, [C.POINTER(dkmc_gpubuf)]),
    "dkmc_update_charge_gpu": (_I, [vp, vp, vp, _I, _I, vp, _I]),
    "dkmc_update_CB_edge_gpu_sparse": (_I, [C.POINTER(dkmc_gpubuf), _I, _I, _I, _D, _I, _D, _D, _D, _I]),
    "dkmc_background_potential_gpu_sparse": (_I, [C.POINTER(dkmc_gpubuf), _I, _I, _I, _D, _I, _D, _D, _D, _I, _I]),
    "dkmc_poisson_gridless_gpu": (_I, [_I, _I, _I, vp, vp, vp, vp, vp, vp, vp, vp]),
    "dkmc_solve_sparse_CG_Jacobi": (_I, [vp, vp, vp, _I, _I, vp, vp, c_int_p, c_dbl_p]),
    "dkmc_solve_sparse_CG_splitmatrix": (_I, [vp, _I, vp, vp, vp, _I, _I, vp, _I, vp, vp, _D, c_int_p, c_dbl_p]),
    "dkmc_execute_kmc_step_gpu": (_I, [_I, _I, vp, vp, vp, _I, vp, vp, vp, vp, vp, vp, vp, vp, vp, vp, vp, vp,
                                       vp, _I, _I, c_int_p, c_int_p, vp, c_dbl_p]),
    "dkmc_build_event_list": (_I, [_I, _I, vp, vp, vp, _I, vp, vp, vp, vp, vp, vp, vp, vp, vp, vp, vp, vp, vp]),
    "dkmc_set_event_temperature": (None, [_I]),
    "dkmc_get_event_temperature": (_I, []),
    "dkmc_build_event_list_T": (_I, [_I, _I, vp, vp, vp, _I, vp, vp, vp, vp, vp, vp, vp, vp, vp, vp, vp, vp, vp, vp, vp]),
    "dkmc_event_rate_census": (_I, [_I, _I, vp, vp, vp, vp, c_dbl_p]),
    "dkmc_set_event_census": (None, [_I]),
    "dkmc_get_event_census_on": (_I, []),
    "dkmc_get_event_census": (_I, [c_dbl_p]),
    "dkmc_debug_get_event_times": (_I, [c_dbl_p]),
    "dkmc_debug_event_loop": (_I, [_I, _I, vp, vp, vp, vp, vp, vp, _I, _I, c_int_p, c_int_p, vp, c_dbl_p]),
    "dkmc_update_power_gpu_sparse": (_I, [C.POINTER(dkmc_gpubuf), _I, _I, _I, _D, _I, _D, _D, _D, _D, _D, _D, _D, _D, _I,
                                          c_dbl_p, _I, _I, _D]),
# ... 120 lines not shown
```

### include/devicekmc_hip_debug.h

```cpp
#ifndef DEVICEKMC_HIP_DEBUG_H
#define DEVICEKMC_HIP_DEBUG_H
#include "devicekmc_hip.h"
#ifdef __cplusplus
extern "C" {
#endif

int dkmc_xt_time_share(int nranks, int rank, int reps, double *apply_us, double *side_us , int *items_out, long long *subblocks_out);
int dkmc_xt_check_shares(int nranks, double *max_abs_diff, double *max_abs, long long *subblocks_sum, long long *items_sum, int *items_total);
int dkmc_xtb_check_product(int width, double *max_abs_diff, double *max_abs);
int dkmc_xtb_poly_coeffs(int degree, double *pc);
int dkmc_xtb_poly_rule(int m);
void dkmc_set_x_poly_auto_rows(int n0, int n1);
int dkmc_xtb_test_nstep(int m, const long long *rp, const int *ci, const double *val, const double *sc, const double *in, const double *add,
                        double ca, double cb, int form, const int *rowlist, int nlist, const int *nsrank, int ns, double *out, double *qs);
int dkmc_xtb_check_poly(int degree, int form, const double *in, double *out, double *qs);
void dkmc_debug_set_x_nmul_window(int cap_bytes, int block_rows);
int dkmc_xtb_time_poly(int degree, int reps, double *us);
typedef struct dkmc_xtb_ctrl { double rr[2]; int done_local, sharded; int done; int iters; int abort_local, aborted; int pad[2]; int xchg_timeout, pad2; } dkmc_xtb_ctrl;
int dkmc_xtb_test_gram(int m, const double *P, const double *T, const double *R, const int *nsrank, int ns, int ng, int done_word, double *gfin,
                       dkmc_xtb_ctrl *ctrl_out);
int dkmc_xtb_test_small(int it, int s, int nrg, const double *gblocks, double tol2, const dkmc_xtb_ctrl *ctrl_in, double *mats, dkmc_xtb_ctrl *ctrl_out);
int dkmc_xtb_test_step(int m, int it, const double *mats, int done_word, double *y0, double *R, double *P, const double *T, const double *sc,
                       const int *nsrank, int ns, const int *rowlist, int nlist, double *Ypanel, double *qs);
int dkmc_xtb_poly1_coeffs(int n, double *pc, double *qmin);
void dkmc_debug_set_x_poly1_degree(int n);
int dkmc_xtb_test_gram1(int m, const double *const *panels, int ng, int done_word, double *gfin);
int dkmc_xtb_test_step1(int m, int it, const double *mats, int done_word, double *y0, double *const *panels, const double *sc, const int *nsrank, int ns,
                        double *qs);
int dkmc_xtb_time_apply(int width, int variant, int reps, double *us);
int dkmc_xt_tile_census(long long *hist);
void dkmc_set_x_items(int kc);
void dkmc_debug_fail_true_residual_once(void);
int dkmc_xtb_tile_product(int width, int stored_bytes, double *out);
int dkmc_xt_get_tiles(long long *ntiles, long long *nsub, int *tiles4, double *tval);
int dkmc_xtb_time_apply_stored(int width, int stored_bytes, int reps, double *us);
int dkmc_get_x_tile_live_info(long long *info8, double *ms2);
int dkmc_debug_xtl_census_form(int form);
long long dkmc_debug_xtl_census_reread(void);
double dkmc_xtl_drop_rule(long long stored_subblocks);
void dkmc_set_x_tile_drop_auto_subblocks(long long gate);
int dkmc_xt_get_live(double theta, int *live_per_tile, double *sS_out);
int dkmc_xt_get_live_masks(double theta, int *mask_per_tile);
int dkmc_debug_x_static_verify(int on);
int dkmc_debug_get_x_static_verify(long long *v4);
int dkmc_x_static_strips(int n_metals);
int dkmc_x_static_rule(int members);
void dkmc_debug_set_x_static_gate(int members);
int dkmc_xt_get_srow(int *ns_out, int *srow_out);
int dkmc_xt_get_diag(double *d_out);
void dkmc_set_x_apply_form(int form);
int dkmc_get_x_apply_form(void);
void dkmc_debug_inject_fault(int phase, int iteration);
int dkmc_debug_step_stop_word(int m, int it, int done_word, int *updated, int *done_after);

int dkmc_xtb_emulate_slabs(int nranks, int width, double tol, int time_rank, int sweep_cap, double *rel_diff, int *iters_slab, int *iters_ref,
                           double *times_us, long long *xdoubles, int *rows_min_max);

int dkmc_xtb_slab_last(int *exchanges_per_sweep, long long *halo_doubles_per_exchange, double *nmul_us);

int dkmc_kcg_emulate_slabs(dkmc_gpubuf *buf, int N, int N_left, int N_right, double Vd, double high_G, double low_G, int num_metals, int nranks, int time_rank,
                           int iter_cap, double *max_abs_diff, int *iters_slab, int *iters_ref, double *times_us, long long *halo_rows);

int dkmc_kcg_form_info(dkmc_gpubuf *buf, long long *info );
int dkmc_kcg_form_words(dkmc_gpubuf *buf, long long *info );
int dkmc_debug_kbw_halfword_pos(int width, int entry);
void dkmc_debug_kbw_segment_cap(int cap);
int dkmc_get_pair_sum_info(long long *info , double *ms );
void dkmc_debug_heat_chain(int on, int budget);
void dkmc_debug_set_cluster_round_cap(int cap);
int dkmc_debug_get_cluster_times(double *ms2);
void dkmc_debug_set_gap_cell_skip(int on);
void dkmc_debug_set_path_round_cap(int cap);
int dkmc_debug_get_path_times(double *ms2);
void dkmc_debug_set_track_hash(int mode);
int dkmc_debug_get_track_times(double *ms2);
void dkmc_debug_set_cut_round_cap(int cap);
int dkmc_debug_get_cut_times(double *ms2);
void dkmc_debug_set_flow_round_cap(int cap);
int dkmc_debug_get_flow_times(double *ms3);
int dkmc_debug_get_event_times(double *ms2);
int dkmc_debug_event_loop(int N, int nn, const int *d_neigh_idx, const double *d_ev_prob_in, int *d_site_element, int *d_site_charge, const double *d_freq,
                          const double *h_uniform, int n_uniform, int resume,
                          int *n_events_out, int *exhausted_out, int *h_event_log, double *event_time_out);

#ifdef __cplusplus
}
#endif
#endif
```

Before: 5.276.

## Fold row partials via per-column occupied-tile lists and skip rowpart zeroing

Result: faster. 5.584 (median of 6 runs) (+5.8%).

```diff
diff --git a/devicekmc_amd/csrc/common.h b/devicekmc_amd/csrc/common.h
--- a/devicekmc_amd/csrc/common.h
+++ b/devicekmc_amd/csrc/common.h
@@ -193,6 +193,8 @@
     int x_static_nM = -1;
     int x_static_verify = 0;
     int x_tile_f32_fail_once = 0;
+    int x_fold_form = 1;
+    int x_fold_poison = 0;
     int x_nmul_form = 1;
     int x_nmul_lane_bytes = 16;
     int x_nmul_window = 2;
@@ -211,7 +213,7 @@
     int err_code = 0;
     double E_gen[DKMC_MAX_LAYERS] = {0}, E_rec[DKMC_MAX_LAYERS] = {0}, E_Vdiff[DKMC_MAX_LAYERS] = {0}, E_Odiff[DKMC_MAX_LAYERS] = {0};
     int num_layers = 0;
-    static const int NBUF = 184;
+    static const int NBUF = 192;
     void *buf[NBUF] = {nullptr};
     size_t bufsz[NBUF] = {0};
 };
@@ -252,6 +254,7 @@
     S_XTB_EMU_Y, S_XTB_EMU_CTRL, S_XTB_YPANEL, S_XTB_PRE_V, S_XTB_PRE_W1, S_XTB_PRE_W2, S_XTB_PRE_Z, S_XTB_PRE_U,
     S_XTB_NPACK_CNT, S_XTB_NPACK_OFF, S_XTB_NPACK_COL, S_XTB_NPACK_W,
     S_XTL_CELLS, S_XTL_TFLAG, S_XTL_TVAL32, S_XTL_TILES, S_XTL_WRANGE, S_XTL_NITEMW, S_XTL_ITEMS, S_XTL_SPLIT,
+    S_XT_WLIST, S_XTL_WLIST,
     S_KS_TAB, S_KS_OWNER, S_KS_LISTS, S_KS_FLAG, S_KS_BOX, S_KS_RLISTS, S_KS_XA, S_KS_XB, S_KS_SEND, S_KS_RECV, S_KS_YBUF, S_KS_EMU,
     S_XTB_TEST_RP, S_XTB_TEST_CI, S_XTB_TEST_VAL, S_XTB_TEST_SC, S_XTB_TEST_NSR, S_XTB_TEST_LIST, S_XTB_TEST_IN, S_XTB_TEST_ADD, S_XTB_TEST_OUT,
     S_XTB_TEST_W1, S_XTB_TEST_W2, S_XTB_TEST_QS, S_XTB_TEST_CTRL, S_XTB_TEST_NPCNT, S_XTB_TEST_NPOFF, S_XTB_TEST_NPCOL, S_XTB_TEST_NPW,
diff --git a/devicekmc_amd/csrc/engine.hip b/devicekmc_amd/csrc/engine.hip
--- a/devicekmc_amd/csrc/engine.hip
+++ b/devicekmc_amd/csrc/engine.hip
@@ -92,6 +92,9 @@
 void dkmc_set_x_tile_drop_auto_subblocks(long long gate) { eng().x_tile_drop_gate = gate > 0 ? gate : 0; }
 double dkmc_get_x_tile_drop_used(void) { return eng().x_tile_drop_used; }
 void dkmc_debug_fail_true_residual_once(void) { eng().x_tile_f32_fail_once = 1; }
+void dkmc_set_x_fold_form(int form) { eng().x_fold_form = form == 0 ? 0 : 1; }
+int dkmc_get_x_fold_form(void) { return eng().x_fold_form; }
+void dkmc_debug_poison_fold_cells(int on) { eng().x_fold_poison = on ? 1 : 0; }
 void dkmc_set_x_static_tiles(int mode) { eng().x_static_tiles = (mode == 0 || mode == 1) ? mode : 2; }
 int dkmc_get_x_static_tiles(void) { return eng().x_static_tiles; }
 int dkmc_debug_x_static_verify(int on) { const int was = eng().x_static_verify; eng().x_static_verify = on ? 1 : 0; return was; }
diff --git a/devicekmc_amd/csrc/xt.hip b/devicekmc_amd/csrc/xt.hip
--- a/devicekmc_amd/csrc/xt.hip
+++ b/devicekmc_amd/csrc/xt.hip
@@ -93,13 +93,15 @@
     const long long i = (long long)blockIdx.x * blockDim.x + threadIdx.x;
     if (i < ncell && cmask[i]) { XTile t; t.k = (int)(i % nK); t.w = (int)(i / nK); t.mask = cmask[i]; t.soff = soff[i]; tiles[toff[i]] = t; }
 }
-__global__ void k_xt_wrange(int nK, int nW, const unsigned *__restrict__ cmask, int2 *__restrict__ wrange)
+__global__ void k_xt_wrange(int nK, int nW, const unsigned *__restrict__ cmask, int2 *__restrict__ wrange, int *__restrict__ wlist)
 {
     const int i = blockIdx.x * blockDim.x + threadIdx.x;
     if (i < nK) {
-        int b = nW, e = 0;
-        for (int w = 0; w < nW; ++w) if (cmask[(long long)w * nK + i]) { b = min(b, w); e = w + 1; }
+        int b = nW, e = 0, n = 0;
+        int *wl = wlist + (size_t)i * (nW + 1);
+        for (int w = 0; w < nW; ++w) if (cmask[(long long)w * nK + i]) { b = min(b, w); e = w + 1; wl[++n] = w; }
         wrange[i] = make_int2(b, e);
+        wl[0] = n;
     }
 }
 #define XT_MAXRANKS 64
@@ -933,7 +935,7 @@
     xrp_t *rp = nullptr, *dpos = nullptr;
     double *val = nullptr, *sd = nullptr, *tval = nullptr, *rowpart = nullptr, *colpart = nullptr, *sc = nullptr, *r = nullptr, *p = nullptr, *t = nullptr,
            *q = nullptr, *vS = nullptr, *part = nullptr, *qS = nullptr, *sS = nullptr, *xS = nullptr, *part_pt = nullptr, *part_rr = nullptr;
-    XTile *tiles = nullptr; int2 *wrange = nullptr; XItem *items = nullptr; unsigned long long *d_cnt = nullptr; XCtrl *ctrl = nullptr;
+    XTile *tiles = nullptr; int2 *wrange = nullptr; int *wlist = nullptr; XItem *items = nullptr; unsigned long long *d_cnt = nullptr; XCtrl *ctrl = nullptr;
     float *tval32 = nullptr;
     SNodes SN{};
     double *xbuf = nullptr;
@@ -1032,10 +1034,11 @@
         if (e.x_block > 1 && ntiles <= 2048 * nr) X.kc = std::max(1, std::min(XT_MAXKC, (ntiles + 1024 * nr - 1) / (1024 * nr)));
         tiles = (XTile *)scratch(S_XT_TILES, (size_t)(ntiles + 1) * sizeof(XTile));
         wrange = (int2 *)scratch(S_XT_WRANGE, (size_t)(nK + 4) * sizeof(int2));
-        if (!tiles || !wrange) return e.err_code;
+        wlist = (int *)scratch(S_XT_WLIST, ((size_t)nK * (nW + 1) + 4) * sizeof(int));
+        if (!tiles || !wrange || !wlist) return e.err_code;
         if (ncell > 0) {
             hipLaunchKernelGGL(k_xt_tile_list, dim3((unsigned)((ncell + 255) / 256)), dim3(256), 0, st, nK, ncell, (const unsigned *)cmask, (const int *)toff, (const int *)soff, tiles);
-            hipLaunchKernelGGL(k_xt_wrange, dim3((nK + 255) / 256), dim3(256), 0, st, nK, nW, (const unsigned *)cmask, wrange);
+            hipLaunchKernelGGL(k_xt_wrange, dim3((nK + 255) / 256), dim3(256), 0, st, nK, nW, (const unsigned *)cmask, wrange, wlist);
         }
         int h_prefix_differs = 0;
         if (k_cand && t_static > 0) {
@@ -1050,7 +1053,7 @@
         items = sh.items; nitem_w = sh.nitem_w;
         KCHK();
         if (k_cand && t_static > 0) { HIPCHK(hipStreamSynchronize(st)); if (h_prefix_differs) { k_cand = false; xs_reason = XS_PREFIX; } }
-        g_xb.tiles = tiles; g_xb.items = items; g_xb.wrange = wrange; g_xb.nitem_w = nitem_w; g_xb.cmask = cmask; g_xb.toff = toff;
+        g_xb.tiles = tiles; g_xb.items = items; g_xb.wrange = wrange; g_xb.wlist = wlist; g_xb.nitem_w = nitem_w; g_xb.cmask = cmask; g_xb.toff = toff;
 
         X.item_lo = sh.item_lo; X.item_n = sh.item_n; X.tile_lo = sh.tile_lo; X.tile_n = sh.tile_n; X.sub_base = sh.sub_base; X.sub_n = sh.sub_n;
         X.w_lo = sh.w_lo; X.w_hi = sh.w_hi;
@@ -1216,7 +1219,7 @@
         XtbArgs B{};
         B.m = m; B.ns = ns; B.ns_pad = ns_pad; B.nK = nK; B.nW = nW; B.s = e.x_block;
         B.items = (const XItem *)items + X.item_lo; B.item_n = X.item_n; B.tiles = tiles; B.sub_base = (int)X.sub_base; B.tval = tval; B.tval32 = tval32;
-        B.wrange = wrange; B.nitem_w = nitem_w; B.nrecords = X.nitems >> X.rec_shift;
+        B.wrange = wrange; B.wlist = wlist; B.nitem_w = nitem_w; B.nrecords = X.nitems >> X.rec_shift;
         B.srow = srow; B.sS = sS; B.nsrank = nsrank; B.rp = rp; B.ci = col; B.val = val; B.sc = sc; B.ax = buf->atom_x; B.ay = buf->atom_y; B.az = buf->atom_z; B.b = rhs; B.y = y;
         B.yaux = yaux; B.yaux_valid = yaux_valid;
         B.ctrl = ctrl; B.tol2 = tol2; B.nt_loads = nt_loads; B.sharded = sharded; B.w_lo = X.w_lo; B.w_hi = X.w_hi;
@@ -1529,7 +1532,7 @@
     XtbArgs B{};
     B.m = m; B.ns = ns; B.ns_pad = X.ns_pad; B.nK = X.nK; B.nW = X.nW; B.s = s;
     B.items = (const XItem *)g_xb.items + X.item_lo; B.item_n = X.item_n; B.tiles = g_xb.tiles; B.sub_base = (int)X.sub_base; B.tval = g_xb.tval;
-    B.wrange = g_xb.wrange; B.nitem_w = g_xb.nitem_w; B.nrecords = X.nitems >> X.rec_shift;
+    B.wrange = g_xb.wrange; B.wlist = g_xb.wlist; B.nitem_w = g_xb.nitem_w; B.nrecords = X.nitems >> X.rec_shift;
     B.srow = g_xb.srow; B.sS = sS; B.nsrank = g_xb.nsrank; B.rp = g_xb.rp; B.ci = g_xb.ci; B.val = g_xb.val; B.sc = sc;
     B.ax = g_xb.ax; B.ay = g_xb.ay; B.az = g_xb.az; B.b = rhs; B.ctrl = ctrl; B.tol2 = tol * tol;
     B.nt_loads = (size_t)X.sub_n * XT_SUB * 8 > ((size_t)200 << 20); B.sharded = false; B.w_lo = X.w_lo; B.w_hi = X.w_hi;
diff --git a/devicekmc_amd/csrc/xt_live.h b/devicekmc_amd/csrc/xt_live.h
--- a/devicekmc_amd/csrc/xt_live.h
+++ b/devicekmc_amd/csrc/xt_live.h
@@ -180,11 +180,12 @@
     if (!c32) { lv->state = -1; return 0; }
     XTile *ltiles = (XTile *)scratch(S_XTL_TILES, (size_t)(nlive + 1) * sizeof(XTile));
     int2 *lwrange = (int2 *)scratch(S_XTL_WRANGE, (size_t)(nK + 4) * sizeof(int2));
-    if (!ltiles || !lwrange) return e.err_code;
+    int *lwlist = (int *)scratch(S_XTL_WLIST, ((size_t)nK * (nW + 1) + 4) * sizeof(int));
+    if (!ltiles || !lwrange || !lwlist) return e.err_code;
     hipLaunchKernelGGL(k_xtl_compact, dim3(X.ntiles), dim3(XT_NT), 0, st, nK, (const XTile *)g_xb.tiles, (int)X.sub_base, (const unsigned *)lcmask, (const int *)lsoff,
                        reinterpret_cast<const float4 *>(g_xb.tval32), reinterpret_cast<float4 *>(c32));
     hipLaunchKernelGGL(k_xt_tile_list, dim3((unsigned)((ncell + 255) / 256)), dim3(256), 0, st, nK, ncell, (const unsigned *)lcmask, (const int *)ltoff, (const int *)lsoff, ltiles);
-    hipLaunchKernelGGL(k_xt_wrange, dim3((nK + 255) / 256), dim3(256), 0, st, nK, nW, (const unsigned *)lcmask, lwrange);
+    hipLaunchKernelGGL(k_xt_wrange, dim3((nK + 255) / 256), dim3(256), 0, st, nK, nW, (const unsigned *)lcmask, lwrange, lwlist);
     KCHK();
     XShare sh{};
     if (int rc = xt_build_items(nK, nW, X.kc, nlive, nsub_live, ltoff, ltiles, 1, 0, S_XTL_NITEMW, S_XTL_ITEMS, S_XTL_SPLIT, &sh, 2)) return rc;
@@ -196,7 +197,7 @@
         HIPCHK(hipEventElapsedTime(&ms, g_xl_ev[0], g_xl_ev[1])); lv->ms[0] = ms;
         HIPCHK(hipEventElapsedTime(&ms, g_xl_ev[1], g_xl_ev[2])); lv->ms[1] = ms;
     }
-    lv->tiles = ltiles; lv->items = sh.items ? sh.items + sh.item_lo : nullptr; lv->item_n = sh.item_n; lv->wrange = lwrange; lv->nitem_w = sh.nitem_w;
+    lv->tiles = ltiles; lv->items = sh.items ? sh.items + sh.item_lo : nullptr; lv->item_n = sh.item_n; lv->wrange = lwrange; lv->wlist = lwlist; lv->nitem_w = sh.nitem_w;
     lv->nrecords = sh.nitems >> sh.rec_shift; lv->nitems = sh.nitems; lv->tval32 = c32;
     lv->info[6] = (long long)bytes;
     lv->state = 1;
@@ -215,6 +216,17 @@
 {
     if (info8) { for (int c = 0; c < 8; ++c) info8[c] = g_xlive.info[c]; info8[0] = g_xlive.state; }
     if (ms2 && eng().profiling) { ms2[0] = g_xlive.ms[0]; ms2[1] = g_xlive.ms[1]; }
+    return 0;
+}
+extern "C" int dkmc_xt_get_fold_lists(int live, int *nK_out, int *nW_out, int *rows)
+{
+    Engine &e = eng(); const XTState &X = g_xt;
+    if (!X.valid || comm_attached() || X.tile_n != X.ntiles || !g_xb.wlist) return dkmc_fail(13, "xt_get_fold_lists: needs the X of a single-GPU solve", __FILE__, __LINE__);
+    if (live && (g_xlive.state != 1 || !g_xlive.wlist)) return dkmc_fail(13, "xt_get_fold_lists: the last solve had no live view", __FILE__, __LINE__);
+    HIPCHK(hipStreamSynchronize(e.stream));
+    if (nK_out) *nK_out = X.nK;
+    if (nW_out) *nW_out = X.nW;
+    if (rows && X.nK > 0) HIPCHK(hipMemcpy(rows, live ? g_xlive.wlist : (const int *)g_xb.wlist, (size_t)X.nK * (X.nW + 1) * sizeof(int), hipMemcpyDeviceToHost));
     return 0;
 }
 static const double *xt_live_sS()
diff --git a/devicekmc_amd/csrc/xtb.hip b/devicekmc_amd/csrc/xtb.hip
--- a/devicekmc_amd/csrc/xtb.hip
+++ b/devicekmc_amd/csrc/xtb.hip
@@ -489,6 +489,33 @@
     const double got = xor_lane<1>(odd ? sx : sy);
     sa = odd ? got : sx; sb = odd ? sy : got;
 }
+__device__ __forceinline__ void xtb_wlist_sum2(const double *__restrict__ p, size_t stride, size_t off, const int *__restrict__ wl, int n, int v, double &sa, double &sb)
+{
+    const bool odd = (v & 1) != 0;
+    const dbl2 *__restrict__ q = reinterpret_cast<const dbl2 *>(odd ? p - 1 + off : p);
+    const size_t st2 = stride >> 1;
+    double a0 = 0.0, a1 = 0.0, a2 = 0.0, a3 = 0.0, b0 = 0.0, b1 = 0.0, b2 = 0.0, b3 = 0.0;
+    const int w0 = n > 0 ? wl[0] : 0;
+    for (int c = 0; c < n; c += 16) {
+        dbl2 x[16]; int sel[16];
+#pragma unroll
+        for (int u = 0; u < 16; ++u) {
+            const int cu = c + u, w = cu < n ? wl[cu] : w0;
+            sel[u] = cu < n ? (w - w0) & 3 : 4;
+            x[u] = cu < n ? __builtin_nontemporal_load(q + (size_t)w * st2) : (dbl2)(0.0);
+        }
+#pragma unroll
+        for (int u = 0; u < 16; ++u) {
+            if (sel[u] == 0) { a0 += x[u].x; b0 += x[u].y; }
+            else if (sel[u] == 1) { a1 += x[u].x; b1 += x[u].y; }
+            else if (sel[u] == 2) { a2 += x[u].x; b2 += x[u].y; }
+            else if (sel[u] == 3) { a3 += x[u].x; b3 += x[u].y; }
+        }
+    }
+    const double sx = (a0 + a1) + (a2 + a3), sy = (b0 + b1) + (b2 + b3);
+    const double got = xor_lane<1>(odd ? sx : sy);
+    sa = odd ? got : sx; sb = odd ? sy : got;
+}
 __global__ __launch_bounds__(XT_NT) void k_xtb_fold_local(int ns, int nK, int nW, int so, const int2 *__restrict__ wrange, const int *__restrict__ nitem_w,
                                                           const double *__restrict__ rowpartB, const double *__restrict__ colpartB, double *__restrict__ xbuf,
                                                           const XCtrl *ctrl, int flag_rank0, int w_lo, int w_hi, const long long *__restrict__ sdst = nullptr)
@@ -642,7 +669,7 @@
         }
     }
 }
-__global__ __launch_bounds__(XT_NT) void k_xtb_fold_rows(int ns, int nK, int nW, int so, const int2 *__restrict__ wrange, const int *__restrict__ nitem_w,
+__global__ __launch_bounds__(XT_NT) void k_xtb_fold_rows(int ns, int nK, int nW, int so, const int2 *__restrict__ wrange, const int *__restrict__ wlist, const int *__restrict__ nitem_w,
                                                          const double *__restrict__ rowpartB, const double *__restrict__ colpartB, const int *__restrict__ srow,
                                                          const double *__restrict__ sS, const double *__restrict__ sc, const double *__restrict__ drvpart,
                                                          double *__restrict__ T, const XCtrl *ctrl)
@@ -658,7 +685,8 @@
         T[(size_t)row * XB_SP + v] = sc[row] * sd;
     }
     for (int k = blockIdx.x; k < nK; k += gridDim.x) {
-        const int2 wr = wrange[k];
+        const int *wl = wlist ? wlist + (size_t)k * (nW + 1) : nullptr;
+        const int2 wr = wl ? make_int2(0, 0) : wrange[k];
         const int wk = k / (XT_C / XT_R);
         const int nc = nitem_w[wk] >> rec_shift, cbase = nitem_w[nW + 2 + wk] >> rec_shift;
         double tA = 0.0, tB = 0.0;
@@ -669,7 +697,8 @@
             const size_t rs = (size_t)XT_R * so, cs = (size_t)XT_C * so;
             double cA, cB, rA_, rB_;
             xtb_list_sum2(cpp, cs, (size_t)16 * so, 0, nc, v, cA, cB);
-            xtb_list_sum2(rpp, rs, (size_t)16 * so, wr.x, wr.y, v, rA_, rB_);
+            if (wl) xtb_wlist_sum2(rpp, rs, (size_t)16 * so, wl + 1, wl[0], v, rA_, rB_);
+            else xtb_list_sum2(rpp, rs, (size_t)16 * so, wr.x, wr.y, v, rA_, rB_);
             tA = cA + rA_; tB = cB + rB_;
         }
         if (sA < ns) { const size_t o = (size_t)srow[sA] * XB_SP + v; T[o] = sS[sA] * (T[o] + tA); }
@@ -1258,7 +1287,10 @@
     if (one) xtb_poly1_coeffs(pn, pc, &qmin); else xtb_poly_coeffs(pd, pc);
     const double tol2_loop = one ? A.tol2 * qmin : (pd > 0 ? A.tol2 / 2.25 : A.tol2);
     HIPCHK(hipMemsetAsync(QS, 0, (size_t)A.ns_pad * XB_SP * 8, st));
-    HIPCHK(hipMemsetAsync(rowpartB, 0, (size_t)(ncell + 1) * XT_R * so * 8, st));
+    const bool listf = e.x_fold_form == 1 && pd > 0 && !A.sharded && A.wlist != nullptr && (!lv || lv->wlist != nullptr);
+    const int so1 = listf ? 4 : so;
+    if (!listf) HIPCHK(hipMemsetAsync(rowpartB, 0, (size_t)(ncell + 1) * XT_R * so * 8, st));
+    else if (e.x_fold_poison) HIPCHK(hipMemsetAsync(rowpartB, 0xff, (size_t)(ncell + 1) * XT_R * so * 8, st));
     HIPCHK(hipMemsetAsync(colpartB, 0, (size_t)(nrec + 1) * XT_C * so * 8, st));
     HIPCHK(hipMemsetAsync(A.ctrl, 0, sizeof(XCtrl), st));
     const bool sharded = A.sharded;
@@ -1280,9 +1312,9 @@
     int local_fail = 0;
     hipLaunchKernelGGL(k_xtb_init, dim3((unsigned)((pan + 255) / 256)), dim3(256), 0, st, m, (const double *)A.y, A.sc, A.nsrank, y0, P, QS,
                        (const double *)((keep_aux && A.yaux_valid) ? A.yaux : nullptr), hs, s, Ypanel);
-    struct XbView { const XItem *items; int item_n; const XTile *tiles; const int2 *wrange; const int *nitem_w; };
-    const XbView full{A.items, A.item_n, A.tiles, A.wrange, A.nitem_w};
-    const XbView live = lv ? XbView{lv->items, lv->item_n, lv->tiles, lv->wrange, lv->nitem_w} : full;
+    struct XbView { const XItem *items; int item_n; const XTile *tiles; const int2 *wrange; const int *nitem_w; const int *wlist; };
+    const XbView full{A.items, A.item_n, A.tiles, A.wrange, A.nitem_w, listf ? A.wlist : nullptr};
+    const XbView live = lv ? XbView{lv->items, lv->item_n, lv->tiles, lv->wrange, lv->nitem_w, listf ? lv->wlist : nullptr} : full;
     const XbView *vw = &full;
     const int ntb = (A.item_n + 3) / 4;
     const int nnb = 2 * XB_DSPLIT + (std::max(m - 2, 1) + 15) / 16;
@@ -1291,7 +1323,7 @@
     if (prof) if (int prc = g_loop_events.begin(EventSampler::LONG | EventSampler::SHORT)) return prc;
     const bool side = sharded && m > 20000 && ntb > 0 && side_stream_init(g_xb_side) == 0;
     const float *t32 = nullptr;
-    auto product = [&](hipEvent_t e0, hipEvent_t e1) {
+    auto product = [&](hipEvent_t e0, hipEvent_t e1, int sw) {
         int sl = 0;
         if (side) {
             SideStream &S = g_xb_side; sl = (int)(S.seq++ % SideStream::RING);
@@ -1300,7 +1332,7 @@
             hipLaunchKernelGGL(k_xtb_neigh, dim3(nnb), dim3(XT_NT), 0, S.st, m, A.rp, A.ci, A.val, (const double *)P, A.sc, A.nsrank, (const XCtrl *)A.ctrl, T, drvpart);
             (void)hipEventRecord(S.b[sl], S.st);
         }
-        if (vw->item_n > 0) xtb_apply({vw->item_n, vw->items, vw->tiles, A.sub_base, A.tval, QS, A.nW, rowpartB, colpartB, A.ctrl, t32}, A.nt_loads, so, 0, st, e0, e1);
+        if (vw->item_n > 0) xtb_apply({vw->item_n, vw->items, vw->tiles, A.sub_base, A.tval, QS, A.nW, rowpartB, colpartB, A.ctrl, t32}, A.nt_loads, sw, 0, st, e0, e1);
         if (side) (void)hipStreamWaitEvent(st, g_xb_side.b[sl], 0);
         else hipLaunchKernelGGL(k_xtb_neigh, dim3(nnb), dim3(XT_NT), 0, st, m, A.rp, A.ci, A.val, (const double *)P, A.sc, A.nsrank, (const XCtrl *)A.ctrl, T, drvpart);
     };
@@ -1308,8 +1340,8 @@
     auto applyL = [&](double *src, double *dst, bool qs) {
         xtb_applyL(st, A, pn, pc, src, dst, W1, W2, qs, [](int, double *) { return 0; }, [&](bool, auto f) { f(nk, [](double *p) { return p; }); return 0; });
     };
-    auto fold_rows = [&](double *Tt) {
-        hipLaunchKernelGGL(k_xtb_fold_rows, dim3(std::max(ng, 1)), dim3(XT_NT), 0, st, A.ns, A.nK, A.nW, so, vw->wrange, vw->nitem_w, (const double *)rowpartB, (const double *)colpartB,
+    auto fold_rows = [&](double *Tt, int sw) {
+        hipLaunchKernelGGL(k_xtb_fold_rows, dim3(std::max(ng, 1)), dim3(XT_NT), 0, st, A.ns, A.nK, A.nW, sw, vw->wrange, vw->wlist, vw->nitem_w, (const double *)rowpartB, (const double *)colpartB,
                            A.srow, A.sS, A.sc, (const double *)drvpart, Tt, (const XCtrl *)A.ctrl);
     };
     auto product_pre = [&](hipEvent_t e0, hipEvent_t e1) {
@@ -1317,19 +1349,19 @@
         double *Pk = P, *Tk = T; P = Vp; T = Zp;
         t32 = f32 ? A.tval32 : nullptr;
         if (lv) { vw = &live; t32 = lv->tval32; }
-        product(e0, e1);
+        product(e0, e1, so);
         t32 = nullptr;
         P = Pk; T = Tk;
-        fold_rows(Zp);
+        fold_rows(Zp, so);
         vw = &full;
         applyL(Zp, T, false);
     };
     auto product_one = [&](hipEvent_t e0, hipEvent_t e1) {
         t32 = f32 ? A.tval32 : nullptr;
         if (lv) { vw = &live; t32 = lv->tval32; }
-        product(e0, e1);
+        product(e0, e1, so);
         t32 = nullptr;
-        fold_rows(T);
+        fold_rows(T, so);
         vw = &full;
         applyL(T, Up, false);
     };
@@ -1364,16 +1396,16 @@
         else xtb_rows_launch<0, 0>(init, ng, st, e2, e3, XB_ROWS_ARGS(itn));
         return 0;
     };
-    product(nullptr, nullptr);
+    product(nullptr, nullptr, so1);
     if (one) {
-        fold_rows(T);
-        if (lv) xt_live_zero_dead(*lv, rowpartB, so);
+        fold_rows(T, so1);
+        if (lv && !listf) xt_live_zero_dead(*lv, rowpartB, so);
         if (int rcx = rows(true, -1, nullptr, nullptr)) return rcx;
         applyL(R, Zp, false);
         gram_one(nullptr, nullptr);
     } else if (pd > 0) {
-        fold_rows(T);
-        if (lv) xt_live_zero_dead(*lv, rowpartB, so);
+        fold_rows(T, so1);
+        if (lv && !listf) xt_live_zero_dead(*lv, rowpartB, so);
         hipLaunchKernelGGL(k_xtb_pre_resid, dim3((unsigned)((pan + 255) / 256)), dim3(256), 0, st, m, (const double *)T, A.b, Zp);
         applyL(Zp, T, false);
         bsel = bz;
@@ -1392,7 +1424,7 @@
             if (one) { product_one(ev[0], ev[1]); gram_one(ev[2], ev[3]); }
             else {
                 if (pd > 0) product_pre(ev[0], ev[1]);
-                else product(ev[0], ev[1]);
+                else product(ev[0], ev[1], so);
                 if (int rcx = rows(false, it, ev[2], ev[3])) return rcx;
             }
             hipLaunchKernelGGL(k_xtb_gred, dim3(XB_NG * 16), dim3(XT_NT), 0, st, ng, (const double *)gpart, gfin, (const XCtrl *)A.ctrl);
@@ -1418,8 +1450,8 @@
         if (!h.pad[0]) {
             hipLaunchKernelGGL(k_xtb_pre_col0, dim3((unsigned)((pan + 255) / 256)), dim3(256), 0, st, m, (const double *)A.y, P);
             hipLaunchKernelGGL(k_xtb_qs_from, dim3((unsigned)((pan + 255) / 256)), dim3(256), 0, st, m, (const double *)P, A.sc, A.nsrank, QS, (const XCtrl *)A.ctrl);
-            product(nullptr, nullptr);
-            fold_rows(T);
+            product(nullptr, nullptr, so1);
+            fold_rows(T, so1);
             const int nrp = std::min(XB_RR_MAXPART, (m + 1023) / 1024);
             hipLaunchKernelGGL(k_xtb_pre_rr_part, dim3(nrp), dim3(256), 0, st, m, (const double *)T, A.b, gpart);
             hipLaunchKernelGGL(k_xtb_pre_rr, dim3(1), dim3(256), 0, st, nrp, (const double *)gpart, bz + m);
diff --git a/devicekmc_amd/csrc/xtiles.h b/devicekmc_amd/csrc/xtiles.h
--- a/devicekmc_amd/csrc/xtiles.h
+++ b/devicekmc_amd/csrc/xtiles.h
@@ -32,6 +32,7 @@
 
 struct XTBuffers {
     SNodes S; int *srow; XTile *tiles; XItem *items; int2 *wrange; int *nitem_w; double *tval, *rowpart, *colpart;
+    int *wlist;
     float *tval32;
     xrp_t *rp, *dpos; int *ci; double *val; int *nsrank;
     unsigned *cmask; int *toff;
@@ -44,6 +45,7 @@
 struct XLive {
     int state = 0;
     const XTile *tiles = nullptr; const XItem *items = nullptr; int item_n = 0; const int2 *wrange = nullptr; const int *nitem_w = nullptr; int nrecords = 0;
+    const int *wlist = nullptr;
     int nitems = 0;
     const float *tval32 = nullptr;
     const int *tflag = nullptr;
@@ -64,6 +66,7 @@
     const XTile *tiles; int sub_base; const double *tval;
     const float *tval32;
     const int2 *wrange; const int *nitem_w; int nrecords;
+    const int *wlist;
     const int *srow; const double *sS; const int *nsrank;
     const xrp_t *rp; const int *ci; const double *val;
     const double *sc;
diff --git a/devicekmc_amd/lib.py b/devicekmc_amd/lib.py
--- a/devicekmc_amd/lib.py
+++ b/devicekmc_amd/lib.py
@@ -86,6 +86,10 @@
     "dkmc_xt_get_live": (_I, [_D, vp, vp]),
     "dkmc_xt_get_live_masks": (_I, [_D, vp]),
     "dkmc_debug_fail_true_residual_once": (None, []),
+    "dkmc_set_x_fold_form": (None, [_I]),
+    "dkmc_get_x_fold_form": (_I, []),
+    "dkmc_debug_poison_fold_cells": (None, [_I]),
+    "dkmc_xt_get_fold_lists": (_I, [_I, c_int_p, c_int_p, vp]),
     "dkmc_set_x_static_tiles": (None, [_I]),
     "dkmc_get_x_static_tiles": (_I, []),
     "dkmc_get_x_static_info": (_I, [C.POINTER(C.c_longlong)]),
diff --git a/include/devicekmc_hip_debug.h b/include/devicekmc_hip_debug.h
--- a/include/devicekmc_hip_debug.h
+++ b/include/devicekmc_hip_debug.h
@@ -41,6 +41,10 @@
 void dkmc_set_x_tile_drop_auto_subblocks(long long gate);
 int dkmc_xt_get_live(double theta, int *live_per_tile, double *sS_out);
 int dkmc_xt_get_live_masks(double theta, int *mask_per_tile);
+void dkmc_set_x_fold_form(int form);
+int dkmc_get_x_fold_form(void);
+void dkmc_debug_poison_fold_cells(int on);
+int dkmc_xt_get_fold_lists(int live, int *nK, int *nW, int *rows);
 int dkmc_debug_x_static_verify(int on);
 int dkmc_debug_get_x_static_verify(long long *v4);
 int dkmc_x_static_strips(int n_metals);
```
